# gevaertlab/RNA-GAN

Measured on AMD Instinct MI355X. Metric: training imgs/sec (G+D WGAN-GP step, 256x256), higher is better.
Workload: dtype bf16; 1 GPU; RNA-GAN lung (betaVAE-conditioned wganvae path) 256x256, DCGAN enc2048/step64, per-GPU batch 64, one iteration = G-loss + D-loss + GP steps; global_batch=64, parallelism=dp1, ranks=1, rna_features=19198, hip_graphs=True, dp_statistics=rank-local (DDP)

## Files before the change

include/rnagan_hip.h:

```cpp
#ifndef RNAGAN_HIP_H
#define RNAGAN_HIP_H

#include <stddef.h>
#include <stdint.h>

#ifdef __cplusplus
extern "C" {
#endif

#define RG_OK 0
#define RG_EINVAL (-1)
#define RG_EUNSUPPORTED (-2)
#define RG_EWORKSPACE (-3)
#define RG_EHIP (-4)

#define RG_F32 0
#define RG_BF16 1
#define RG_U8 3
#define RG_F16 2

#define RG_ALGO_AUTO 0
#define RG_ALGO_GENERIC 1
#define RG_ALGO_MFMA 2

int rg_version(void);
const char* rg_last_error(void);
int rg_set_option(const char* name, int value);


int rg_pack_conv_weight(const float* w, void* wdn, void* wup, int O, int I, int dtype, void* stream);
int rg_pack_conv_wup_from_bf16(const void* w_bf16, void* wup, int O, int I, void* stream);
int rg_pack_conv_wup_from_bf16_multi(int n, const void* const* w_bf16, void* const* wup, const int* O, const int* I, void* stream);
int rg_pack_g0_weight_from_bf16(const void* w_bf16, void* wp, int E, int C, void* stream);

int rg_conv_stats_rows(int up, int N, int Hlow, int Wlow, int O, int I, int dtype, int algo);
int rg_conv_down(const void* x, const float* w, const void* wdn, void* y, int N, int Hi, int Wi, int I,
                 int O, float* stats_partial, int dtype, int algo, void* ws, size_t ws_bytes, void* stream);
size_t rg_conv_workspace_bytes(int up, int N, int Hlow, int Wlow, int O, int I, int dtype, int algo);

int rg_conv_up(const void* x, const float* w, const void* wup, void* y, int N, int Ho, int Wo, int O, int I,
               const void* mask_act, float mask_slope, float* stats_partial, int dtype, int algo, void* ws,
               size_t ws_bytes, void* stream);

size_t rg_conv_wgrad_workspace_bytes(int N, int Ho, int Wo, int O, int I, int dtype, int algo);
int rg_conv_wgrad(const void* low, const void* high, float* dw, int N, int Ho, int Wo, int O, int I, int dtype,
                  int accumulate, int algo, void* ws, size_t ws_bytes, void* stream);
int rg_conv_wgrad2(const void* low0, const void* high0, const void* low1, const void* high1, float* dw, int N,
                   int Ho, int Wo, int O, int I, int dtype, int accumulate, int algo, void* ws, size_t ws_bytes,
                   void* stream);
int rg_conv_wgrad_slabs(const void* low0, const void* high0, const void* low1, const void* high1, float* dw, int N, int Ho,
                        int Wo, int O, int I, int dtype, int algo, void* slab, size_t slab_bytes, int* nsplit_out,
                        int* slab_dtype_out, void* stream);
int rg_conv_wgrad_adam_supported(int N, int Ho, int Wo, int O, int I, int two, int dtype, int algo);
int rg_conv_wgrad_adam(const void* low0, const void* high0, const void* low1, const void* high1, float* p, float* m, float* v,
                       const float* hyper, void* shadow_bf16, int N, int Ho, int Wo, int O, int I, int dtype, int algo,
                       void* stream);

int rg_first_down(const float* x_nchw, const float* w, const float* bias, void* y, int N, int H, int W, int I,
                  int O, float slope, int dtype, void* stream);
int rg_last_up(const void* x, const float* w, const float* bias, float* y_nchw, int N, int Ho, int Wo, int O,
               int I, int apply_tanh, int dtype, void* stream);
int rg_first_down_bits(const float* x_nchw, const float* w, const float* bias, void* y, void* bits, int N, int H, int W,
                       int I, int O, float slope, int dtype, void* stream);
int rg_sign_pack(const void* a, void* bits, long long npix, int C, int dtype, void* stream);
int rg_first_down_masked_supported(int H, int W, int I, int O, int dtype);
int rg_first_down_masked(const float* x_nchw, const float* w, void* y, const void* mask_bits, float mask_slope, int N,
                         int H, int W, int I, int O, int dtype, void* stream);
int rg_conv_up_maskbits_supported(int N, int Ho, int Wo, int O, int I, int dtype, int algo);
int rg_conv_up_maskbits(const void* x, const void* wup, void* y, int N, int Ho, int Wo, int O, int I,
                        const void* mask_bits, float mask_slope, int dtype, int algo, void* ws, size_t ws_bytes,
                        void* stream);
int rg_last_up_post_blocks(int N, int Ho, int Wo, int O, int I, int dtype);
int rg_last_up_post(const void* x, const float* w, float* y_nchw, int N, int Ho, int Wo, int O, int I, int dtype,
                    const float* tanh_img, float* part, void* stream);
int rg_last_up_part_chan_sum(const float* part, int nblocks, float* out3, int accumulate, void* stream);
int rg_gp_coef_parts(const float* part, int nblocks, float* sq, float* loss, float* coef, float lambd, void* stream);
int rg_gp_coef_parts_scaled(const float* part, int nblocks, float* sq, float* loss, float* coef, float lambd, float in_scale,
                            float out_scale, void* stream);
int rg_gp_coef_parts_scaled_dev(const float* part, int nblocks, float* sq, float* loss, float* coef, float lambd,
                                const int* amp_state, int slot, void* stream);
int rg_last_up_pre_supported(int Wo, int O, int I, int dtype);
int rg_last_up_pre(const void* z, const float* w, const float* bias, float* y_nchw, const float* mean, const float* invstd,
                   const float* gamma, const float* beta, float slope, int N, int Ho, int Wo, int O, int I, int apply_tanh,
                   int dtype, void* stream);
size_t rg_skinny_wgrad_workspace_bytes(int N, int Ho, int Wo, int O, int I);
int rg_skinny_wgrad(const void* low, const float* high_nchw, float* dw, int N, int Ho, int Wo, int O, int I,
                    int dtype, int accumulate, void* ws, size_t ws_bytes, void* stream);
int rg_skinny_wgrad_slabs(const void* low, const float* high_nchw, int N, int Ho, int Wo, int O, int I, int dtype, void* slab,
                          size_t slab_bytes, int* nslab_out, float* bias_slab, int* bias_done_out, void* stream);
int rg_skinny_wgrad_bias(const void* low, const float* high_nchw, float* dw, float* dbias, int N, int Ho, int Wo, int O, int I,
                         int dtype, int accumulate, int bias_accumulate, void* ws, size_t ws_bytes, int* bias_done_out,
                         void* stream);


int rg_pack_g0_weight(const float* w, void* wp, int E, int C, int dtype, void* stream);
int rg_g0_fwd(const float* z, const float* w, const void* wp, void* y, int N, int E, int C, int dtype, int algo,
              void* ws, size_t ws_bytes, void* stream);
size_t rg_g0_workspace_bytes(int N, int E, int C, int dtype, int algo);
int rg_g0_wgrad(const float* z, const void* gy, float* dw, int N, int E, int C, int dtype, int accumulate,
                int algo, void* ws, size_t ws_bytes, void* stream);

int rg_head_fwd(const void* a, const float* w, float* h, float* out, int N, int C, float slope, int dtype,
                void* stream);
int rg_head_fwd_bias(const void* a, const float* w, const float* bias, float* h, float* out, int N, int C, float slope,
                     int dtype, void* stream);
int rg_vec_sum(const float* x, int n, float* out, int accumulate, void* stream);
int rg_head_grad(const float* h, float* gh, int N, float coef, float slope, void* stream);
int rg_head_grad_dev(const float* h, float* gh, int N, float coef, const int* amp_state, int slot, int part, float slope,
                     void* stream);
int rg_head_bwd_data(const float* gh, const float* w, void* ga, int N, int C, int dtype, void* stream);
int rg_head_wgrad(const float* gh, const void* a, float* dw, int N, int C, int dtype, int accumulate,
                  void* stream);

int rg_pack_linear_weight(const float* w, void* wp, int Nout, int K, int Nout_pad, int K_pad, void* stream);
size_t rg_linear_workspace_bytes(int M, int K, int Nout, int algo);
int rg_linear_affine_act(const float* x, int ldx, const float* w, const void* wp, const float* scale,
                         const float* shift, float* y, int ldy, int M, int K, int Nout, float slope, int algo,
                         void* ws, size_t ws_bytes, void* stream);

size_t rg_colreduce_workspace_bytes(int M, int C, int nq);

int rg_bn_stats(const void* z, float* sum, float* sumsq, int M, int C, int dtype, void* ws, size_t ws_bytes,
                void* stream);
int rg_bn_finalize(const float* sum, const float* sumsq, int M, int C, float eps, float momentum, float* mean,
                   float* invstd, float* running_mean, float* running_var, int64_t* num_batches_tracked,
                   void* stream);
int rg_bn_forward(const void* z, int M, int C, float eps, float momentum, const float* gamma, const float* beta,
                  float slope, float* mean, float* invstd, float* running_mean, float* running_var,
                  int64_t* num_batches_tracked, void* a, int dtype, void* ws, size_t ws_bytes, void* stream);
int rg_bn_forward_partials(const float* partial, int G, const void* z, int M, int C, float eps, float momentum,
                           const float* gamma, const float* beta, float slope, float* mean, float* invstd,
                           float* running_mean, float* running_var, int64_t* num_batches_tracked, void* a, int dtype,
                           void* ws, size_t ws_bytes, void* stream);
int rg_bn_stats_finalize(const void* z, int M, int C, float eps, float momentum, float* mean, float* invstd,
                         float* running_mean, float* running_var, int64_t* num_batches_tracked, int dtype, void* ws,
                         size_t ws_bytes, void* stream);
int rg_bn_act(const void* z, const float* mean, const float* invstd, const float* gamma, const float* beta,
              void* a, int M, int C, float slope, int dtype, void* stream);
int rg_bn_act_bwd(const void* z, const void* ga, const float* mean, const float* invstd, const float* gamma,
                  const float* beta, void* gz, float* s_gy, float* s_gyxh, float* dgamma, float* dbeta,
                  int accumulate, int M, int C, float slope, int dtype, void* ws, size_t ws_bytes, void* stream);
int rg_bn_finalize_partials(const float* partial, int G, int M, int C, float eps, float momentum, float* mean,
                            float* invstd, float* running_mean, float* running_var, int64_t* num_batches_tracked, void* ws,
                            size_t ws_bytes, void* stream);
int rg_g0_wgrad_adam_supported(int N, int E, int C, int dtype);
int rg_g0_wgrad_adam(const float* z, const void* gz0, float* p, float* m, float* v, const float* hyper, void* shadow_bf16,
                     int N, int E, int C, int dtype, void* stream);

int rg_linear_wgrad_adam(const void* gT, const void* xT, int ldn, int N, float* p, float* m, float* v, const float* hyper, int O,
                         int I, void* wpack_bf16, int Kp, void* stream);

int rg_im2col_nhwc(const float* x, int ldx, float* cols, int N, int H, int W, int C, int kh, int kw, int sh, int sw, int ph,
                   int pw, void* stream);
int rg_pool2d_nhwc(const float* x, int ldx, float* y, int ldy, int N, int H, int W, int C, int k, int stride, int pad, int mode,
                   void* stream);
int rg_nchw_to_nhwc_affine(const float* x_nchw, float* y_nhwc, int N, int C, int H, int W, const float* scale, const float* shift,
                           void* stream);
int rg_spatial_mean_nhwc(const float* x, float* y, int N, int HW, int C, void* stream);

int rg_resize_bilinear01(const void* src, int src_dtype, int64_t sn, int64_t sc, int64_t sh, int64_t sw, float mul, float add,
                         float* dst_nchw, int N, int C, int H, int W, int Ho, int Wo, void* stream);
int rg_moments_update(const float* x, int ldx, int n, int F, double* s1, double* s2, void* stream);

int rg_conv_split(int up, int N, int Hlow, int Wlow, int O, int I, int dtype, int algo);
int rg_conv_slab_dtype(int up, int N, int Hlow, int Wlow, int O, int I, int dtype, int algo);
int rg_conv_down_partial(const void* x, const void* wdn, int N, int Hi, int Wi, int I, int O, int dtype, int algo,
                         void* ws, size_t ws_bytes, void* stream);
int rg_conv_up_partial(const void* x, const void* wup, int N, int Ho, int Wo, int O, int I, int dtype, int algo,
                       void* ws, size_t ws_bytes, void* stream);
int rg_slab_bn_supported(long long M, int C, int groups, int nsplit);
size_t rg_slab_bn_scratch_bytes(long long M, int C, int groups);
size_t rg_slab_bn_sync_words(void);
int rg_bn_forward_slabs(const void* slab, int nsplit, size_t slab_stride, int slab_dtype, void* z, void* a, long long M, int C, int groups,
                        float eps, float momentum, const float* gamma, const float* beta, float slope, float* mean,
                        float* invstd, float* running_mean, float* running_var, long long* num_batches_tracked,
                        void* scratch, size_t scratch_bytes, void* sync, void* stream);
int rg_bn_tangent_slabs(const void* slab, int nsplit, size_t slab_stride, int slab_dtype, const void* z, void* zt_out, void* at, long long M,
                        int C, const float* mean, const float* invstd, const float* gamma, const float* beta, float slope,
                        float* s_zt, float* s_xhzt, void* scratch, size_t scratch_bytes, void* sync, void* stream);
int rg_bn_act_bwd_slabs(const void* slab, int nsplit, size_t slab_stride, int slab_dtype, const void* z, void* ga_out, void* gz, long long M,
                        int C, int groups, const float* mean, const float* invstd, const float* gamma, const float* beta,
                        float slope, float* s_gy, float* s_gyxh, float* dgamma, float* dbeta, int accumulate, void* scratch,
                        size_t scratch_bytes, void* sync, void* stream);

int rg_bn_finalize_partials_g2(const float* partial, int G, int nblk, int M, int C, float eps, float momentum, float* mean,
                               float* invstd, float* running_mean, float* running_var, int64_t* num_batches_tracked,
                               void* ws, size_t ws_bytes, void* stream);
int rg_bn_forward_g2(const float* partial, int G, int nblk, const void* z, int M, int C, float eps, float momentum,
                     const float* gamma, const float* beta, float slope, float* mean, float* invstd, float* running_mean,
                     float* running_var, int64_t* num_batches_tracked, void* a, int dtype, void* ws, size_t ws_bytes,
                     void* stream);
int rg_bn_act_bwd_g2(const void* z, const void* ga, const float* mean, const float* invstd, const float* gamma,
                     const float* beta, void* gz, float* s_gy, float* s_gyxh, float* dgamma, float* dbeta, int accumulate,
                     int M, int C, float slope, int dtype, void* ws, size_t ws_bytes, void* stream);
int rg_bn_tangent(const void* z, const void* zt, const float* mean, const float* invstd, const float* gamma,
                  const float* beta, void* at, float* s_zt, float* s_xhzt, int M, int C, float slope, int dtype,
                  void* ws, size_t ws_bytes, void* stream);
int rg_bn_double_bwd(const void* z, const void* qa, const void* zt, const void* ga1, const float* mean,
                     const float* invstd, const float* gamma, const float* beta, const float* s_gy,
                     const float* s_gyxh, const float* s_zt, const float* s_xhzt, void* pz, float* dgamma,
                     float* dbeta, int accumulate, int M, int C, float slope, int dtype, void* ws,
                     size_t ws_bytes, void* stream);

int rg_slab_finish_rows(long long M, int C);
int rg_slab_bias_act(const void* slab, int nsplit, size_t stride, int slab_dtype, const float* bias, void* y, long long M, int C,
                     float slope, void* stream);
int rg_slab_mask(const void* slab, int nsplit, size_t stride, int slab_dtype, const void* mask_act, float mask_slope, void* y,
                 float* col_parts, long long M, int C, void* stream);
int rg_parts_col_sum(const float* parts, int rows, int C, float* out, int accumulate, void* stream);
int rg_bias_act(const void* z, const float* bias, void* y, long long M, int C, float slope, int dtype, void* stream);
int rg_conv_down_epi_supported(int N, int Hi, int Wi, int I, int O, int dtype, int algo);
int rg_conv_down_epi(const void* x, const void* wdn, void* y, int N, int Hi, int Wi, int I, int O, const float* shift, float slope,
                     const void* mask_act, float mask_slope, int dtype, int algo, void* ws, size_t ws_bytes, void* stream);

int rg_lrelu_bwd(const void* g, const void* a, void* out, size_t n, float slope, int dtype, void* stream);
int rg_col_sum(const void* g, float* out, int M, int C, int dtype, int accumulate, void* ws, size_t ws_bytes,
               void* stream);

int rg_tanh_bwd(const float* gy, const float* y, float* gz, size_t n, void* stream);
int rg_nchw_chan_sum(const float* g, float* out, int N, int C, int HW, int accumulate, void* ws, size_t ws_bytes,
                     void* stream);
int rg_interp(const float* real, const float* fake, float* out, size_t n, float eps, void* stream);
int rg_interp_dev(const float* real, const float* fake, float* out, size_t n, const float* eps, void* stream);
size_t rg_reduce_workspace_bytes(size_t n);
int rg_sqnorm(const float* x, float* out, size_t n, void* ws, size_t ws_bytes, void* stream);
int rg_gp_coef(const float* sq, float* loss, float* coef, float lambd, void* stream);
int rg_gp_coef_scaled(const float* sq, float* loss, float* coef, float lambd, float in_scale, float out_scale, void* stream);
int rg_gp_coef_scaled_dev(const float* sq, float* loss, float* coef, float lambd, const int* amp_state, int slot, void* stream);
int rg_scale_by(const float* x, const float* coef, float* out, size_t n, void* stream);
int rg_mean_diff(const float* a, const float* b, float* out, int n, float sign, void* stream);
// ... 130 lines not shown
```

rna_gan_amd/_abi.py:

```python
from __future__ import annotations

import ctypes as C
import os

_HERE = os.path.dirname(os.path.abspath(__file__))
LIB_PATH = os.path.join(_HERE, "librnagan_hip.so")

RG_F32, RG_BF16, RG_F16 = 0, 1, 2
RG_U8 = 3
ALGO_AUTO, ALGO_GENERIC, ALGO_MFMA = 0, 1, 2

_p = C.c_void_p
_i = C.c_int
_f = C.c_float
_d = C.c_double
_z = C.c_size_t
_l = C.c_int64

PROTOTYPES = {
    "rg_version": (_i, []),
    "rg_last_error": (C.c_char_p, []),
    "rg_set_option": (_i, [C.c_char_p, _i]),
    "rg_pack_conv_weight": (_i, [_p, _p, _p, _i, _i, _i, _p]),
    "rg_conv_stats_rows": (_i, [_i, _i, _i, _i, _i, _i, _i, _i]),
    "rg_conv_down": (_i, [_p, _p, _p, _p, _i, _i, _i, _i, _i, _p, _i, _i, _p, _z, _p]),
    "rg_conv_up": (_i, [_p, _p, _p, _p, _i, _i, _i, _i, _i, _p, _f, _p, _i, _i, _p, _z, _p]),
    "rg_conv_workspace_bytes": (_z, [_i, _i, _i, _i, _i, _i, _i, _i]),
    "rg_conv_wgrad_workspace_bytes": (_z, [_i, _i, _i, _i, _i, _i, _i]),
    "rg_conv_wgrad": (_i, [_p, _p, _p, _i, _i, _i, _i, _i, _i, _i, _i, _p, _z, _p]),
    "rg_conv_wgrad2": (_i, [_p, _p, _p, _p, _p, _i, _i, _i, _i, _i, _i, _i, _i, _p, _z, _p]),
    "rg_conv_wgrad_slabs": (_i, [_p, _p, _p, _p, _p, _i, _i, _i, _i, _i, _i, _i, _p, _z, _p, _p, _p]),
    "rg_grad_to_wire": (_i, [_p, _p, _z, _i, _p, _p, _p, _p, _p, _p]),
    "rg_conv_wgrad_wire": (_i, [_p, _p, _p, _p, _p, _i, _i, _i, _i, _i, _i, _i, _p]),
    "rg_conv_wgrad_adam_supported": (_i, [_i, _i, _i, _i, _i, _i, _i, _i]),
    "rg_conv_wgrad_adam": (_i, [_p, _p, _p, _p, _p, _p, _p, _p, _p, _i, _i, _i, _i, _i, _i, _i, _p]),
    "rg_first_down": (_i, [_p, _p, _p, _p, _i, _i, _i, _i, _i, _f, _i, _p]),
    "rg_first_down_bits": (_i, [_p, _p, _p, _p, _p, _i, _i, _i, _i, _i, _f, _i, _p]),
    "rg_sign_pack": (_i, [_p, _p, C.c_longlong, _i, _i, _p]),
    "rg_first_down_masked_supported": (_i, [_i, _i, _i, _i, _i]),
    "rg_first_down_masked": (_i, [_p, _p, _p, _p, _f, _i, _i, _i, _i, _i, _i, _p]),
    "rg_conv_up_maskbits_supported": (_i, [_i, _i, _i, _i, _i, _i, _i]),
    "rg_conv_up_maskbits": (_i, [_p, _p, _p, _i, _i, _i, _i, _i, _p, _f, _i, _i, _p, _z, _p]),
    "rg_last_up": (_i, [_p, _p, _p, _p, _i, _i, _i, _i, _i, _i, _i, _p]),
    "rg_skinny_wgrad_workspace_bytes": (_z, [_i, _i, _i, _i, _i]),
    "rg_skinny_wgrad": (_i, [_p, _p, _p, _i, _i, _i, _i, _i, _i, _i, _p, _z, _p]),
    "rg_skinny_wgrad_slabs": (_i, [_p, _p, _i, _i, _i, _i, _i, _i, _p, _z, _p, _p, _p, _p]),
    "rg_skinny_wgrad_bias": (_i, [_p, _p, _p, _p, _i, _i, _i, _i, _i, _i, _i, _i, _p, _z, _p, _p]),
    "rg_pack_g0_weight": (_i, [_p, _p, _i, _i, _i, _p]),
    "rg_pack_conv_wup_from_bf16": (_i, [_p, _p, _i, _i, _p]),
    "rg_pack_conv_wup_from_bf16_multi": (_i, [_i, _p, _p, _p, _p, _p]),
    "rg_pack_g0_weight_from_bf16": (_i, [_p, _p, _i, _i, _p]),
    "rg_g0_fwd": (_i, [_p, _p, _p, _p, _i, _i, _i, _i, _i, _p, _z, _p]),
    "rg_g0_workspace_bytes": (_z, [_i, _i, _i, _i, _i]),
    "rg_g0_wgrad": (_i, [_p, _p, _p, _i, _i, _i, _i, _i, _i, _p, _z, _p]),
    "rg_head_fwd": (_i, [_p, _p, _p, _p, _i, _i, _f, _i, _p]),
    "rg_head_grad": (_i, [_p, _p, _i, _f, _f, _p]),
    "rg_head_grad_dev": (_i, [_p, _p, _i, _f, _p, _i, _i, _f, _p]),
    "rg_adam_hyper_dev3": (_i, [_p, _d, _d, _d, _d, _d, _p, _i, _p, _p]),
    "rg_nonfinite_probe": (_i, [_i, _p, _p, _p, _p, _p]),
    "rg_amp_update": (_i, [_p, _i, _i, _i, _i, _p]),
    "rg_amp_latch": (_i, [_p, _i, _p]),
    "rg_gp_coef_scaled_dev": (_i, [_p, _p, _p, _f, _p, _i, _p]),
    "rg_gp_coef_parts_scaled_dev": (_i, [_p, _i, _p, _p, _p, _f, _p, _i, _p]),
    "rg_head_bwd_data": (_i, [_p, _p, _p, _i, _i, _i, _p]),
    "rg_head_wgrad": (_i, [_p, _p, _p, _i, _i, _i, _i, _p]),
    "rg_pack_linear_weight": (_i, [_p, _p, _i, _i, _i, _i, _p]),
    "rg_linear_workspace_bytes": (_z, [_i, _i, _i, _i]),
    "rg_linear_affine_act": (_i, [_p, _i, _p, _p, _p, _p, _p, _i, _i, _i, _i, _f, _i, _p, _z, _p]),
    "rg_colreduce_workspace_bytes": (_z, [_i, _i, _i]),
    "rg_bn_stats": (_i, [_p, _p, _p, _i, _i, _i, _p, _z, _p]),
    "rg_bn_finalize": (_i, [_p, _p, _i, _i, _f, _f, _p, _p, _p, _p, _p, _p]),
    "rg_bn_forward": (_i, [_p, _i, _i, _f, _f, _p, _p, _f, _p, _p, _p, _p, _p, _p, _i, _p, _z, _p]),
    "rg_bn_forward_partials": (_i, [_p, _i, _p, _i, _i, _f, _f, _p, _p, _f, _p, _p, _p, _p, _p, _p, _i, _p, _z, _p]),
    "rg_bn_stats_finalize": (_i, [_p, _i, _i, _f, _f, _p, _p, _p, _p, _p, _i, _p, _z, _p]),
    "rg_bn_act": (_i, [_p, _p, _p, _p, _p, _p, _i, _i, _f, _i, _p]),
    "rg_bn_act_bwd": (_i, [_p, _p, _p, _p, _p, _p, _p, _p, _p, _p, _p, _i, _i, _i, _f, _i, _p, _z, _p]),
    "rg_bn_act_bwd_g2": (_i, [_p, _p, _p, _p, _p, _p, _p, _p, _p, _p, _p, _i, _i, _i, _f, _i, _p, _z, _p]),
    "rg_bn_finalize_partials": (_i, [_p, _i, _i, _i, _f, _f, _p, _p, _p, _p, _p, _p, _z, _p]),
    "rg_linear_wgrad_adam": (_i, [_p, _p, _i, _i, _p, _p, _p, _p, _i, _i, _p, _i, _p]),
    "rg_last_up_post_blocks": (_i, [_i, _i, _i, _i, _i, _i]),
    "rg_last_up_post": (_i, [_p, _p, _p, _i, _i, _i, _i, _i, _i, _p, _p, _p]),
    "rg_last_up_part_chan_sum": (_i, [_p, _i, _p, _i, _p]),
    "rg_gp_coef_parts": (_i, [_p, _i, _p, _p, _p, _f, _p]),
    "rg_last_up_pre_supported": (_i, [_i, _i, _i, _i]),
    "rg_last_up_pre": (_i, [_p, _p, _p, _p, _p, _p, _p, _p, _f, _i, _i, _i, _i, _i, _i, _i, _p]),
    "rg_bn_forward_g2": (_i, [_p, _i, _i, _p, _i, _i, _f, _f, _p, _p, _f, _p, _p, _p, _p, _p, _p, _i, _p, _z, _p]),
    "rg_bn_finalize_partials_g2": (_i, [_p, _i, _i, _i, _i, _f, _f, _p, _p, _p, _p, _p, _p, _z, _p]),
    "rg_bn_tangent": (_i, [_p, _p, _p, _p, _p, _p, _p, _p, _p, _i, _i, _f, _i, _p, _z, _p]),
    "rg_bn_double_bwd": (_i, [_p, _p, _p, _p, _p, _p, _p, _p, _p, _p, _p, _p, _p, _p, _p, _i, _i, _i, _f, _i,
                              _p, _z, _p]),
    "rg_lrelu_bwd": (_i, [_p, _p, _p, _z, _f, _i, _p]),
    "rg_col_sum": (_i, [_p, _p, _i, _i, _i, _i, _p, _z, _p]),
    "rg_tanh_bwd": (_i, [_p, _p, _p, _z, _p]),
    "rg_nchw_chan_sum": (_i, [_p, _p, _i, _i, _i, _i, _p, _z, _p]),
    "rg_interp": (_i, [_p, _p, _p, _z, _f, _p]),
    "rg_reduce_workspace_bytes": (_z, [_z]),
    "rg_sqnorm": (_i, [_p, _p, _z, _p, _z, _p]),
    "rg_gp_coef": (_i, [_p, _p, _p, _f, _p]),
    "rg_scale_by": (_i, [_p, _p, _p, _z, _p]),
    "rg_mean_diff": (_i, [_p, _p, _p, _i, _f, _p]),
    "rg_latent_prep": (_i, [_p, _p, _p, _i, _i, _p]),
    "rg_adam_step": (_i, [_p, _p, _p, _p, _z, _i, _d, _d, _d, _d, _p]),
    "rg_clamp": (_i, [_p, _z, _f, _f, _p]),
    "rg_upconv3_workspace_bytes": (_z, [_i, _i, _i, _i, _i]),
    "rg_upconv3_fwd": (_i, [_p, _p, _p, _p, _i, _i, _i, _i, _i, _i, _i, _i, _p, _z, _p]),
    "rg_upconv3_bwd_data": (_i, [_p, _i, _p, _p, _i, _i, _i, _i, _i, _i, _i, _p, _z, _p]),
    "rg_upconv3_wgrad": (_i, [_p, _i, _p, _p, _i, _i, _i, _i, _i, _i, _i, _i, _p, _z, _p]),
    "rg_export_images_nhwc": (_i, [_p, _p, _i, _i, _i, _i, _p]),
    "rg_bn_bwd_sums": (_i, [_p, _p, _p, _p, _p, _p, _p, _p, _i, _i, _f, _i, _p, _z, _p]),
    "rg_bn_bwd_apply": (_i, [_p, _p, _p, _p, _p, _p, _p, _p, _p, _i, _i, _i, _f, _i, _p]),
    "rg_bn_tangent_sums": (_i, [_p, _p, _p, _p, _p, _p, _p, _p, _i, _i, _f, _i, _p, _z, _p]),
    "rg_bn_tangent_apply": (_i, [_p, _p, _p, _p, _p, _p, _p, _p, _p, _i, _i, _i, _f, _i, _p]),
    "rg_bn_dbl_sums": (_i, [_p, _p, _p, _p, _p, _p, _p, _p, _p, _i, _i, _f, _i, _p, _z, _p]),
    "rg_bn_dbl_apply": (_i, [_p] * 17 + [_i, _i, _i, _i, _f, _i, _p, _z, _p]),
    "rg_latent_stats": (_i, [_p, _p, _p, _p, _i, _i, _p]),
    "rg_latent_apply": (_i, [_p, _p, _p, _p, _p, _i, _i, _i, _p]),
    "rg_adam_step_dev": (_i, [_p, _p, _p, _p, _z, _p, _p, _p, _p]),
    "rg_adam_step_slabs": (_i, [_p, _p, _p, _p, _z, _p, _p, _i, _p, _p, _p, _p, _p, _p]),
    "rg_ema_update": (_i, [_p, _p, _z, _f, _p, _p, _p]),
    "rg_interp_dev": (_i, [_p, _p, _p, _z, _p, _p]),
    "rg_adam_hyper_dev": (_i, [_p, _d, _d, _d, _d, _d, _p, _p]),
    "rg_adam_hyper_dev2": (_i, [_p, _d, _d, _d, _d, _d, _d, _p, _p]),
    "rg_storage_dtype": (_i, []),
    "rg_gp_coef_scaled": (_i, [_p, _p, _p, _f, _f, _f, _p]),
    "rg_gp_coef_parts_scaled": (_i, [_p, _i, _p, _p, _p, _f, _f, _f, _p]),
    "rg_transpose_f32": (_i, [_p, _p, _i, _i, _p]),
    "rg_transpose_pack_bf16": (_i, [_p, _p, _i, _i, _i, _i, _p]),
    "rg_gemm_nt_bf16_workspace_bytes": (_z, [_i, _i, _i]),
    "rg_gemm_nt_bf16": (_i, [_p, _p, _p, _p, _p, _i, _i, _i, _i, _f, _p, _z, _p]),
    "rg_vae_dropout": (_i, [_p, _p, _p, _i, _i, _i, _f, _p]),
    "rg_vae_reparam": (_i, [_p, _p, _p, _p, _z, _p]),
    "rg_vae_reparam_bwd": (_i, [_p, _p, _p, _p, _p, _p, _p, _z, _p]),
    "rg_tanh_inplace": (_i, [_p, _z, _p]),
    "rg_add_inplace": (_i, [_p, _p, _z, _p]),
    "rg_vae_loss_workspace_bytes": (_z, []),
    "rg_vae_loss": (_i, [_p, _p, _i, _i, _i, _p, _p, _i, _f, _i, _p, _p, _p, _p, _p, _z, _p]),
    "rg_widen_bf16": (_i, [_p, _p, _z, _p]),
    "rg_cast_pad": (_i, [_p, _p, _i, _i, _i, _i, _p]),
    "rg_selftest_layouts": (_i, [_p, _p]),
    "rg_u8_to_norm": (_i, [_p, _p, _z, _f, _f, _p]),
    "rg_conv_up_fp8": (_i, [_p, _p, _p, _i, _i, _i, _i, _i, _p, _p, _f, _i, _p]),
    "rg_gemm_fp8": (_i, [_p, _p, _p, _i, _i, _i, _p, _p, _f, _i, _p]),
    "rg_fp8_supported": (_i, [_i, _i, _i, _i]),
    "rg_cast_fp8": (_i, [_p, _p, _z, _f, _p]),
    "rg_selftest_fp8": (_i, [_p, _p]),
    "rg_g0_wgrad_adam_supported": (_i, [_i, _i, _i, _i]),
    "rg_g0_wgrad_adam": (_i, [_p, _p, _p, _p, _p, _p, _p, _i, _i, _i, _i, _p]),
    "rg_im2col_nhwc": (_i, [_p, _i, _p, _i, _i, _i, _i, _i, _i, _i, _i, _i, _i, _p]),
    "rg_pool2d_nhwc": (_i, [_p, _i, _p, _i, _i, _i, _i, _i, _i, _i, _i, _i, _p]),
    "rg_nchw_to_nhwc_affine": (_i, [_p, _p, _i, _i, _i, _i, _p, _p, _p]),
    "rg_spatial_mean_nhwc": (_i, [_p, _p, _i, _i, _i, _p]),
    "rg_resize_bilinear01": (_i, [_p, _i, _l, _l, _l, _l, _f, _f, _p, _i, _i, _i, _i, _i, _i, _p]),
    "rg_moments_update": (_i, [_p, _i, _i, _i, _p, _p, _p]),
    "rg_conv_split": (_i, [_i, _i, _i, _i, _i, _i, _i, _i]),
    "rg_conv_slab_dtype": (_i, [_i, _i, _i, _i, _i, _i, _i, _i]),
    "rg_conv_down_partial": (_i, [_p, _p, _i, _i, _i, _i, _i, _i, _i, _p, _z, _p]),
    "rg_conv_up_partial": (_i, [_p, _p, _i, _i, _i, _i, _i, _i, _i, _p, _z, _p]),
    "rg_slab_bn_supported": (_i, [C.c_longlong, _i, _i, _i]),
    "rg_slab_bn_scratch_bytes": (_z, [C.c_longlong, _i, _i]),
    "rg_slab_bn_sync_words": (_z, []),
    "rg_bn_forward_slabs": (_i, [_p, _i, _z, _i, _p, _p, C.c_longlong, _i, _i, _f, _f, _p, _p, _f, _p, _p, _p, _p, _p, _p, _z, _p, _p]),
    "rg_bn_tangent_slabs": (_i, [_p, _i, _z, _i, _p, _p, _p, C.c_longlong, _i, _p, _p, _p, _p, _f, _p, _p, _p, _z, _p, _p]),
    "rg_bn_act_bwd_slabs": (_i, [_p, _i, _z, _i, _p, _p, _p, C.c_longlong, _i, _i, _p, _p, _p, _p, _f, _p, _p, _p, _p, _i, _p, _z,
                                 _p, _p]),
    "rg_conv_up_affine": (_i, [_p, _p, _p, _i, _i, _i, _i, _i, _p, _p, _f, _p, _z, _p]),
    "rg_g0_fwd_affine": (_i, [_p, _p, _p, _i, _i, _i, _p, _p, _f, _p, _z, _p]),
    "rg_split_planes": (_i, [_p, _p, _z, _p]),
    "rg_f32p_conv_supported": (_i, [_i, _i, _i, _i, _i, _i, _i]),
    "rg_f32p_conv_workspace_bytes": (_z, [_i, _i, _i, _i, _i, _i, _i]),
    "rg_f32p_conv_stats_rows": (_i, [_i, _i, _i, _i, _i, _i, _i]),
    "rg_f32p_conv": (_i, [_i, _p, _p, _p, _i, _i, _i, _i, _i, _i, _p, _p, _f, _p, _z, _p]),
    "rg_f32p_conv_mask_supported": (_i, [_i, _i, _i, _i, _i, _i, _i]),
    "rg_f32p_wgrad_supported": (_i, [_i, _i, _i, _i, _i, _i]),
    "rg_f32p_wgrad_workspace_bytes": (_z, [_i, _i, _i, _i, _i, _i, _i]),
    "rg_f32p_wgrad": (_i, [_p, _p, _p, _p, _p, _i, _i, _i, _i, _i, _i, _i, _p, _z, _p]),
    "rg_slab_finish_rows": (_i, [C.c_longlong, _i]),
    "rg_slab_bias_act": (_i, [_p, _i, _z, _i, _p, _p, C.c_longlong, _i, _f, _p]),
    "rg_slab_mask": (_i, [_p, _i, _z, _i, _p, _f, _p, _p, C.c_longlong, _i, _p]),
    "rg_parts_col_sum": (_i, [_p, _i, _i, _p, _i, _p]),
    "rg_bias_act": (_i, [_p, _p, _p, C.c_longlong, _i, _f, _i, _p]),
    "rg_vec_sum": (_i, [_p, _i, _p, _i, _p]),
    "rg_conv_down_epi_supported": (_i, [_i, _i, _i, _i, _i, _i, _i]),
    "rg_conv_down_epi": (_i, [_p, _p, _p, _i, _i, _i, _i, _i, _p, _f, _p, _f, _i, _i, _p, _z, _p]),
    "rg_head_fwd_bias": (_i, [_p, _p, _p, _p, _p, _i, _i, _f, _i, _p]),
    "rg_probe_mfma_bare": (_i, [_i, _i, _i, _i, _p, _p, _p]),
    "rg_probe_lds_mfma": (_i, [_i, _i, _i, _p, _p, _p, _p, _p]),
    "rg_probe_copy": (_i, [_p, _p, _z, _i, _i, _p]),
    "rg_probe_fill_bf16": (_i, [_p, _z, C.c_uint, _p]),
}

ABI_VERSION = 616

_libs = {}
LIB_PATH_F16 = os.path.join(_HERE, "librnagan_hip_f16.so")
BF16_ONLY_PREFIXES = ("rg_probe_", "rg_split_planes", "rg_f32p_")


def load(half: str = "bf16"):
    if half in _libs:
        return _libs[half]
    if half not in ("bf16", "f16"):
        raise ValueError("half must be 'bf16' or 'f16'")
    path = LIB_PATH if half == "bf16" else LIB_PATH_F16
    if not os.path.exists(path):
        raise RuntimeError(
            "rna_gan_amd: %s not found. Build it with `python -m rna_gan_amd.build` "
            "(hipcc --offload-arch=gfx950). There is no CPU / eager fallback." % path)
    try:
        lib = C.CDLL(path)
    except OSError as e:
        raise RuntimeError("rna_gan_amd: cannot load %s: %s" % (path, e))
    for name, (res, args) in PROTOTYPES.items():
        if half == "f16" and name.startswith(BF16_ONLY_PREFIXES):
            continue
        fn = getattr(lib, name, None)
        if fn is None:
            raise RuntimeError("rna_gan_amd: symbol %s missing from %s: the library is older than this package -- rebuild "
                               "it with `python -m rna_gan_amd.build`" % (name, path))
        fn.restype = res
        fn.argtypes = args
    got = lib.rg_version()
    if got != ABI_VERSION:
        raise RuntimeError("rna_gan_amd: %s reports ABI version %d, this package binds version %d (a stale or swapped "
                           "build): rebuild it with `python -m rna_gan_amd.build`" % (path, got, ABI_VERSION))
    want = RG_BF16 if half == "bf16" else RG_F16
    if lib.rg_storage_dtype() != want:
        raise RuntimeError("rna_gan_amd: %s stores dtype code %d, expected %d (a swapped build)" % (path, lib.rg_storage_dtype(), want))
    _libs[half] = lib
    return lib


_LAST_ERR_LIBS = ("bf16", "f16")


def check(rc: int, what: str):
    if rc != 0:
        msgs = []
        for h in _LAST_ERR_LIBS:
            if h in _libs:
                m = _libs[h].rg_last_error()
                if m:
                    msgs.append(m.decode() if len(_libs) == 1 else "[%s build] %s" % (h, m.decode()))
        raise RuntimeError("rna_gan_amd: %s failed (%d): %s" % (what, rc, " | ".join(msgs) if msgs else "?"))
```

rna_gan_amd/csrc/rg_api.hip:

```cpp
#include "rg_common.h"
#include "rg_internal.h"
#include <stdarg.h>
#include <stdio.h>
#include <stdlib.h>
#include <string.h>
#include <ctype.h>

static thread_local char g_err[512] = "";

void rg_set_error(const char* fmt, ...) {
  va_list ap;
  va_start(ap, fmt);
  vsnprintf(g_err, sizeof(g_err), fmt, ap);
  va_end(ap);
}

extern "C" int rg_version(void) { return 616; }
extern "C" const char* rg_last_error(void) { return g_err; }

static const char* const g_opt_names[] = {"conv8", "conv8_blocks", "conv_tile", "xcd", "class_fast", "wgrad_blocks",
                                          "wgrad8", "conv_v1", "stream_tile", "narrow8", "conv8_mfma", "conv8_epi", "wgrad8_blocks", "korder", "convp", "convp_blocks",
                                          "fp8_mx", "wgrad8n", "f32mma", "convd", "convd_blocks", "skinny128", "slab16", "wslab16", "bn_rev", "wgrad8_mfma", "narrow32", "upimg", "upimg_blocks"};
constexpr int G_NOPT = sizeof(g_opt_names) / sizeof(g_opt_names[0]);
static int g_opt_override[G_NOPT];
static int g_opt_env[G_NOPT];

int rg_option(const char* name, int dflt) {
  for (int i = 0; i < G_NOPT; ++i) {
    if (strcmp(name, g_opt_names[i]) != 0) continue;
    if (g_opt_override[i] > 0) return g_opt_override[i] - 1;
    if (g_opt_env[i] == 0) {
      char var[64] = "RNAGAN_";
      size_t n = strlen(var);
      for (const char* c = name; *c && n + 1 < sizeof(var); ++c) var[n++] = (char)toupper((unsigned char)*c);
      var[n] = 0;
      const char* e = getenv(var);
      g_opt_env[i] = e ? atoi(e) + 1 : -1;
      if (g_opt_env[i] == 0) g_opt_env[i] = -1;
    }
    return g_opt_env[i] > 0 ? g_opt_env[i] - 1 : dflt;
  }
  return dflt;
}

extern "C" int rg_set_option(const char* name, int value) {
  RG_REQUIRE(name, RG_EINVAL, "set_option: null name");
  for (int i = 0; i < G_NOPT; ++i)
    if (strcmp(name, g_opt_names[i]) == 0) { g_opt_override[i] = value < 0 ? 0 : value + 1; return RG_OK; }
  rg_set_error("set_option: unknown option '%s'", name);
  return RG_EINVAL;
}

static bool want_mfma(int algo, int dtype) { return algo != RG_ALGO_GENERIC && dtype == RG_H16; }

extern "C" int rg_pack_conv_weight(const float* w, void* wdn, void* wup, int O, int I, int dtype, void* stream) {
  RG_REQUIRE(w && O > 0 && I > 0, RG_EINVAL, "pack_conv_weight: bad args");
  RG_REQUIRE(dtype == RG_H16, RG_EUNSUPPORTED, "pack_conv_weight: only bf16 packs exist (fp32 kernels read w)");
  return rg_mfma_pack_conv_weight(w, wdn, wup, O, I, rg_stream(stream));
}

extern "C" size_t rg_conv_workspace_bytes(int up, int N, int Hlow, int Wlow, int O, int I, int dtype, int algo) {
  if (!want_mfma(algo, dtype)) return 0;
  if (!rg_mfma_conv_supported(N, Hlow, Wlow, up ? O : I, up ? I : O)) return 0;
  return rg_mfma_conv_ws_bytes(up, N, Hlow, Wlow, O, I);
}

extern "C" int rg_conv_stats_rows(int up, int N, int Hlow, int Wlow, int O, int I, int dtype, int algo) {
  if (N <= 0 || Hlow <= 0 || Wlow <= 0 || O <= 0 || I <= 0 || !want_mfma(algo, dtype)) return 0;
  if (!rg_mfma_conv_supported(N, Hlow, Wlow, up ? O : I, up ? I : O)) return 0;
  return rg_mfma_conv_stats_rows(up, N, Hlow, Wlow, O, I);
}

extern "C" int rg_conv_split(int up, int N, int Hlow, int Wlow, int O, int I, int dtype, int algo) {
  if (N <= 0 || Hlow <= 0 || Wlow <= 0 || O <= 0 || I <= 0 || !want_mfma(algo, dtype)) return 1;
  if (!rg_mfma_conv_supported(N, Hlow, Wlow, up ? O : I, up ? I : O)) return 1;
  return rg_mfma_conv_nsplit(up, N, Hlow, Wlow, O, I);
}

extern "C" int rg_conv_slab_dtype(int up, int N, int Hlow, int Wlow, int O, int I, int dtype, int algo) {
  if (rg_conv_split(up, N, Hlow, Wlow, O, I, dtype, algo) <= 1) return RG_F32;
  return rg_mfma_conv_slab16(up, N, Hlow, Wlow, O, I) ? RG_H16 : RG_F32;
}

extern "C" int rg_conv_down_partial(const void* x, const void* wdn, int N, int Hi, int Wi, int I, int O, int dtype, int algo,
                                    void* ws, size_t ws_bytes, void* stream) {
  RG_REQUIRE(x && wdn && ws && N > 0 && Hi > 0 && Wi > 0 && I > 0 && O > 0 && Hi % 2 == 0 && Wi % 2 == 0, RG_EINVAL,
             "conv_down_partial: bad args");
  RG_REQUIRE(rg_conv_split(0, N, Hi / 2, Wi / 2, O, I, dtype, algo) > 1, RG_EUNSUPPORTED,
             "conv_down_partial: this shape does not run split-K (rg_conv_split)");
  return rg_mfma_conv_down(x, wdn, nullptr, N, Hi, Wi, I, O, nullptr, ws, ws_bytes, rg_stream(stream), 1);
}

extern "C" int rg_conv_up_partial(const void* x, const void* wup, int N, int Ho, int Wo, int O, int I, int dtype, int algo,
                                  void* ws, size_t ws_bytes, void* stream) {
  RG_REQUIRE(x && wup && ws && N > 0 && Ho > 0 && Wo > 0 && I > 0 && O > 0, RG_EINVAL, "conv_up_partial: bad args");
  RG_REQUIRE(rg_conv_split(1, N, Ho, Wo, O, I, dtype, algo) > 1, RG_EUNSUPPORTED,
             "conv_up_partial: this shape does not run split-K (rg_conv_split)");
  return rg_mfma_conv_up(x, wup, nullptr, N, Ho, Wo, O, I, nullptr, 1.f, nullptr, ws, ws_bytes, rg_stream(stream), nullptr,
                         nullptr, 1.f, 0, 1);
}
// ... 159 lines not shown
                              const float* invstd, const float* gamma, const float* beta, float slope, int N, int Ho, int Wo,
                              int O, int I, int apply_tanh, int dtype, void* stream) {
  RG_REQUIRE(z && w && y_nchw && mean && invstd && gamma && beta && N > 0 && Ho > 0 && Wo > 0, RG_EINVAL,
             "last_up_pre: bad args");
  RG_REQUIRE(rg_last_up_pre_supported(Wo, O, I, dtype), RG_EUNSUPPORTED, "last_up_pre: shape");
  return rg_skinny_last_up(z, w, bias, y_nchw, N, Ho, Wo, O, I, apply_tanh, dtype, rg_stream(stream), mean, invstd, gamma,
                           beta, slope);
}

extern "C" int rg_last_up(const void* x, const float* w, const float* bias, float* y_nchw, int N, int Ho, int Wo,
                          int O, int I, int apply_tanh, int dtype, void* stream) {
  RG_REQUIRE(x && w && y_nchw && N > 0 && Ho > 0 && Wo > 0 && I > 0 && O > 0, RG_EINVAL, "last_up: bad args");
  if (rg_skinny_supported(I, O))
    return rg_skinny_last_up(x, w, bias, y_nchw, N, Ho, Wo, O, I, apply_tanh, dtype, rg_stream(stream));
  return rg_generic_last_up(x, w, bias, y_nchw, N, Ho, Wo, O, I, apply_tanh, dtype, rg_stream(stream));
}

extern "C" int rg_last_up_post_blocks(int N, int Ho, int Wo, int O, int I, int dtype) {
  return rg_skinny_supported(I, O) ? rg_skinny_last_up_post_blocks(N, Ho, Wo, O, dtype) : 0;
}
extern "C" int rg_last_up_post(const void* x, const float* w, float* y_nchw, int N, int Ho, int Wo, int O, int I, int dtype,
                               const float* tanh_img, float* part, void* stream) {
  RG_REQUIRE(x && w && y_nchw && N > 0 && Ho > 0 && Wo > 0 && (tanh_img || part), RG_EINVAL, "last_up_post: bad args");
  RG_REQUIRE(rg_last_up_post_blocks(N, Ho, Wo, O, I, dtype) > 0, RG_EUNSUPPORTED, "last_up_post: shape");
  RG_REQUIRE((((uintptr_t)tanh_img | (uintptr_t)part) & 15) == 0, RG_EINVAL, "last_up_post: 16-byte aligned buffers required");
  return rg_skinny_last_up(x, w, nullptr, y_nchw, N, Ho, Wo, O, I, 0, dtype, rg_stream(stream), nullptr, nullptr, nullptr,
                           nullptr, 1.f, tanh_img, part);
}
extern "C" int rg_last_up_part_chan_sum(const float* part, int nblocks, float* out3, int accumulate, void* stream) {
  RG_REQUIRE(part && out3 && nblocks > 0, RG_EINVAL, "last_up_part_chan_sum: bad args");
  return rg_skinny_lu_part_final(part, nblocks, out3, accumulate, 0, nullptr, nullptr, 0.f, rg_stream(stream));
}
extern "C" int rg_gp_coef_parts_scaled(const float* part, int nblocks, float* sq, float* loss, float* coef, float lambd,
                                       float in_scale, float out_scale, void* stream) {
  RG_REQUIRE(part && loss && coef && nblocks > 0 && in_scale > 0.f && out_scale > 0.f, RG_EINVAL, "gp_coef_parts: bad args");
  return rg_skinny_lu_part_final(part, nblocks, sq, 0, 1, loss, coef, lambd, rg_stream(stream), in_scale, out_scale);
}
extern "C" int rg_storage_dtype(void) { return RG_H16; }
extern "C" int rg_gp_coef_parts(const float* part, int nblocks, float* sq, float* loss, float* coef, float lambd,
                                void* stream) {
  RG_REQUIRE(part && loss && coef && nblocks > 0, RG_EINVAL, "gp_coef_parts: bad args");
  return rg_skinny_lu_part_final(part, nblocks, sq, 0, 1, loss, coef, lambd, rg_stream(stream));
}

extern "C" size_t rg_skinny_wgrad_workspace_bytes(int N, int Ho, int Wo, int O, int I) {
  size_t a = rg_generic_wgrad_ws_bytes(N, Ho, Wo, O, I);
  size_t b = rg_skinny_supported(I, O) ? rg_skinny_wgrad_ws_bytes(N, Ho, Wo, O, I) : 0;
  return a > b ? a : b;
}

extern "C" int rg_skinny_wgrad(const void* low, const float* high_nchw, float* dw, int N, int Ho, int Wo, int O, int I,
                               int dtype, int accumulate, void* ws, size_t ws_bytes, void* stream) {
  RG_REQUIRE(low && high_nchw && dw && N > 0 && Ho > 0 && Wo > 0 && I > 0 && O > 0, RG_EINVAL,
             "skinny_wgrad: bad args");
  if (rg_skinny_supported(I, O) && !(dtype == RG_F32 && rg_generic_f32_image_side(N, 2 * Ho, 2 * Wo, I, O)))
    return rg_skinny_wgrad_impl(low, high_nchw, dw, N, Ho, Wo, O, I, dtype, accumulate, ws, ws_bytes,
                                rg_stream(stream));
  return rg_generic_skinny_wgrad(low, high_nchw, dw, N, Ho, Wo, O, I, dtype, accumulate, ws, ws_bytes,
                                 rg_stream(stream));
}

extern "C" int rg_skinny_wgrad_bias(const void* low, const float* high_nchw, float* dw, float* dbias, int N, int Ho, int Wo, int O,
                                    int I, int dtype, int accumulate, int bias_accumulate, void* ws, size_t ws_bytes,
                                    int* bias_done_out, void* stream) {
  RG_REQUIRE(low && high_nchw && dw && bias_done_out && N > 0 && Ho > 0 && Wo > 0 && I > 0 && O > 0, RG_EINVAL,
             "skinny_wgrad_bias: bad args");
  *bias_done_out = 0;
  if (rg_skinny_supported(I, O) && !(dtype == RG_F32 && rg_generic_f32_image_side(N, 2 * Ho, 2 * Wo, I, O)))
    return rg_skinny_wgrad_impl(low, high_nchw, dw, N, Ho, Wo, O, I, dtype, accumulate, ws, ws_bytes, rg_stream(stream),
                                O == 64 ? dbias : nullptr, bias_accumulate, bias_done_out);
  return rg_generic_skinny_wgrad(low, high_nchw, dw, N, Ho, Wo, O, I, dtype, accumulate, ws, ws_bytes, rg_stream(stream));
}

extern "C" int rg_skinny_wgrad_slabs(const void* low, const float* high_nchw, int N, int Ho, int Wo, int O, int I, int dtype,
                                     void* slab, size_t slab_bytes, int* nslab_out, float* bias_slab, int* bias_done_out,
                                     void* stream) {
  RG_REQUIRE(low && high_nchw && slab && nslab_out && N > 0 && Ho > 0 && Wo > 0 && I > 0 && O > 0 &&
                 (bias_slab == nullptr || bias_done_out != nullptr), RG_EINVAL, "skinny_wgrad_slabs: bad args");
  *nslab_out = 0;
  if (bias_done_out) *bias_done_out = 0;
  if (!rg_skinny_supported(I, O)) return RG_OK;
  return rg_skinny_wgrad_slabs_impl(low, high_nchw, N, Ho, Wo, O, I, dtype, slab, slab_bytes, nslab_out, bias_slab, bias_done_out,
                                    rg_stream(stream));
}

extern "C" int rg_pack_conv_wup_from_bf16(const void* w_bf16, void* wup, int O, int I, void* stream) {
  RG_REQUIRE(w_bf16 && wup && O > 0 && I > 0, RG_EINVAL, "pack_conv_wup_from_bf16: bad args");
  return rg_mfma_transpose_bf16(w_bf16, wup, O, 16 * I, 0, rg_stream(stream));
}
extern "C" int rg_pack_conv_wup_from_bf16_multi(int n, const void* const* w_bf16, void* const* wup, const int* O, const int* I,
                                                void* stream) {
  RG_REQUIRE(n >= 1 && n <= 8 && w_bf16 && wup && O && I, RG_EINVAL, "pack_conv_wup_from_bf16_multi: bad args");
  int Cc[8];
  for (int i = 0; i < n; ++i) Cc[i] = 16 * I[i];
  return rg_mfma_transpose_bf16_multi(n, w_bf16, wup, O, Cc, rg_stream(stream));
}
extern "C" int rg_pack_g0_weight_from_bf16(const void* w_bf16, void* wp, int E, int C, void* stream) {
  RG_REQUIRE(w_bf16 && wp && E > 0 && C > 0, RG_EINVAL, "pack_g0_weight_from_bf16: bad args");
  return rg_mfma_transpose_bf16(w_bf16, wp, E, 16 * C, 1, rg_stream(stream));
}
extern "C" int rg_pack_g0_weight(const float* w, void* wp, int E, int C, int dtype, void* stream) {
  RG_REQUIRE(w && wp && E > 0 && C > 0, RG_EINVAL, "pack_g0_weight: bad args");
  RG_REQUIRE(dtype == RG_H16, RG_EUNSUPPORTED, "pack_g0_weight: only bf16 packs exist");
  return rg_mfma_pack_g0_weight(w, wp, E, C, rg_stream(stream));
}

extern "C" size_t rg_g0_workspace_bytes(int N, int E, int C, int dtype, int algo) {
  if (!want_mfma(algo, dtype)) return 0;
  size_t a = (size_t)N * E * 2;
  size_t b = rg_mfma_g0_wgrad_ws_bytes(N, E, C);
  return a > b ? a : b;
}

extern "C" int rg_g0_fwd(const float* z, const float* w, const void* wp, void* y, int N, int E, int C, int dtype,
                         int algo, void* ws, size_t ws_bytes, void* stream) {
  RG_REQUIRE(z && y && N > 0 && E > 0 && C > 0, RG_EINVAL, "g0_fwd: bad args");
  if (want_mfma(algo, dtype) && wp && rg_mfma_plain_supported(N, E, 16 * C)) {
    RG_REQUIRE(ws && ws_bytes >= (size_t)N * E * 2, RG_EWORKSPACE, "g0_fwd: workspace too small");
    int rc = rg_cast_pad(z, ws, N, E, E, RG_H16, stream);
    if (rc) return rc;
    return rg_mfma_gemm_plain(ws, wp, y, N, E, 16 * C, 16 * C, rg_stream(stream));
  }
  RG_REQUIRE(algo != RG_ALGO_MFMA, RG_EUNSUPPORTED, "g0_fwd: shape/dtype not supported by the MFMA kernel");
  RG_REQUIRE(w, RG_EINVAL, "g0_fwd: generic kernel needs the fp32 master weight");
  return rg_generic_g0_fwd(z, w, y, N, E, C, dtype, rg_stream(stream));
}

extern "C" int rg_g0_fwd_affine(const float* z, const void* wp, void* y, int N, int E, int C, const float* scale,
                                const float* shift, float slope, void* ws, size_t ws_bytes, void* stream) {
  RG_REQUIRE(z && wp && y && scale && shift && N > 0 && E > 0 && C > 0, RG_EINVAL, "g0_fwd_affine: bad args");
  RG_REQUIRE(rg_mfma_plain_supported(N, E, 16 * C), RG_EUNSUPPORTED, "g0_fwd_affine: shape not supported by the MFMA kernel");
  RG_REQUIRE(ws && ws_bytes >= (size_t)N * E * 2, RG_EWORKSPACE, "g0_fwd_affine: workspace too small");
  int rc = rg_cast_pad(z, ws, N, E, E, RG_H16, stream);
  if (rc) return rc;
  return rg_mfma_gemm_plain(ws, wp, y, N, E, 16 * C, 16 * C, rg_stream(stream), scale, shift, slope);
}

extern "C" int rg_conv_up_affine(const void* x, const void* wup, void* y, int N, int Ho, int Wo, int O, int I,
                                 const float* scale, const float* shift, float slope, void* ws, size_t ws_bytes,
                                 void* stream) {
  RG_REQUIRE(x && wup && y && scale && shift && N > 0 && Ho > 0 && Wo > 0 && I > 0 && O > 0, RG_EINVAL,
             "conv_up_affine: bad args");
  RG_REQUIRE(rg_mfma_conv_supported(N, Ho, Wo, O, I), RG_EUNSUPPORTED,
             "conv_up_affine: shape not supported by the MFMA kernel");
  return rg_mfma_conv_up(x, wup, y, N, Ho, Wo, O, I, nullptr, 1.f, nullptr, ws, ws_bytes, rg_stream(stream), scale, shift,
                         slope);
}

extern "C" int rg_conv_up_fp8(const void* x8, const void* wup8, void* y, int N, int Ho, int Wo, int O, int I,
                              const float* scale, const float* shift, float slope, int out_fp8, void* stream) {
  RG_REQUIRE(x8 && wup8 && y && scale && shift && N > 0 && Ho > 0 && Wo > 0 && I > 0 && O > 0, RG_EINVAL, "conv_up_fp8: bad args");
  RG_REQUIRE(rg_is_pow2(Ho) && rg_is_pow2(Wo) && rg_mfma_fp8_supported(N * Ho * Wo, 4 * O, I, 4), RG_EUNSUPPORTED,
             "conv_up_fp8: shape not supported (O, I multiples of 128, at least 256 / 512 low-resolution pixels)");
  return rg_mfma_conv_up_fp8(x8, wup8, y, N, Ho, Wo, O, I, scale, shift, slope, out_fp8, rg_stream(stream));
}
extern "C" int rg_gemm_fp8(const void* a8, const void* b8, void* y, int M, int K, int Ncols, const float* scale,
                           const float* shift, float slope, int out_fp8, void* stream) {
  RG_REQUIRE(a8 && b8 && y && scale && shift && M > 0 && K > 0 && Ncols > 0, RG_EINVAL, "gemm_fp8: bad args");
  RG_REQUIRE(rg_mfma_fp8_supported(M, K, Ncols, 1), RG_EUNSUPPORTED, "gemm_fp8: shape not supported");
  return rg_mfma_gemm_fp8(a8, b8, y, M, K, Ncols, scale, shift, slope, out_fp8, rg_stream(stream));
}
extern "C" int rg_fp8_supported(int M, int K, int Ncols, int taps) { return rg_mfma_fp8_supported(M, K, Ncols, taps) ? 1 : 0; }

extern "C" int rg_g0_wgrad(const float* z, const void* gy, float* dw, int N, int E, int C, int dtype, int accumulate,
                           int algo, void* ws, size_t ws_bytes, void* stream) {
  RG_REQUIRE(z && gy && dw && N > 0 && E > 0 && C > 0, RG_EINVAL, "g0_wgrad: bad args");
// ... 91 lines not shown
```

rna_gan_amd/csrc/rg_g0adam.hip:

```cpp
#include "rg_internal.h"
#include <stdlib.h>

namespace {

constexpr int GA_E = 64, GA_J = 256, GA_N = 64;

struct AdamC { float b1, b2, omb1, omb2, eps, step_size, inv_sqrt_bc2, wd, ginv; };
__device__ __forceinline__ void adam_upd(const AdamC& a, float& pp, float gg, float& mm, float& vv) {
  rg_adam_upd(pp, gg * a.ginv, mm, vv, a.b2, a.omb1, a.omb2, a.eps, a.step_size, a.inv_sqrt_bc2, a.wd);
}

typedef rg_h16x8 ga_bf16x8;
typedef __attribute__((ext_vector_type(16))) float ga_f32x16;
constexpr int GA_CP = GA_J + 4;
constexpr int GA_P = 72;

template <typename TG>
__global__ __launch_bounds__(256) void g0_wgrad_adam_kernel(const float* __restrict__ z, const TG* __restrict__ gz0,
                                                            float* __restrict__ p, float* __restrict__ m, float* __restrict__ v,
                                                            const float* __restrict__ hyper, uint16_t* __restrict__ shadow,
                                                            int N, int E, int C, int e_fastest) {
  constexpr int OPS = (GA_E + GA_J) * GA_P * 2;
  static_assert(32 * GA_CP * 4 <= OPS, "accumulator tile must fit into the operand area");
  __shared__ __attribute__((aligned(16))) unsigned char smem[OPS];
  if (hyper[9] != 0.f) return;
  uint16_t* zsT = reinterpret_cast<uint16_t*>(smem);
  uint16_t* gsT = zsT + GA_E * GA_P;
  float* ct = reinterpret_cast<float*>(smem);
  const int t = threadIdx.x, lane = t & 63, wave = t >> 6;
  const int fr = lane & 31, fh = lane >> 5;
  const int e0 = (e_fastest ? blockIdx.x : blockIdx.y) * GA_E, c0 = (e_fastest ? blockIdx.y : blockIdx.x) * 16;
  ga_f32x16 acc[2][2];
#pragma unroll
  for (int i = 0; i < 2; ++i)
#pragma unroll
    for (int j = 0; j < 2; ++j)
#pragma unroll
      for (int r = 0; r < 16; ++r) acc[i][j][r] = 0.f;

  const int ze = t & 63, zq = t >> 6;
  const int gnp = t & 31, gtap = (t >> 5) * 2;
  float zr[8][2];
  uint4 gr[2][2][2];
  auto load_chunk = [&](int n0) {
#pragma unroll
    for (int i = 0; i < 8; ++i) {
      const int n = n0 + 2 * (zq + 4 * i);
      zr[i][0] = n < N ? z[(size_t)n * E + e0 + ze] : 0.f;
      zr[i][1] = n + 1 < N ? z[(size_t)(n + 1) * E + e0 + ze] : 0.f;
    }
#pragma unroll
    for (int a = 0; a < 2; ++a)
#pragma unroll
      for (int k = 0; k < 2; ++k) {
        const int n = n0 + 2 * gnp + k;
        gr[a][k][0] = gr[a][k][1] = make_uint4(0, 0, 0, 0);
        if (n < N) {
          const TG* src = gz0 + ((size_t)n * 16 + gtap + a) * C + c0;
          if constexpr (sizeof(TG) == 2) {
            gr[a][k][0] = *reinterpret_cast<const uint4*>(src);
            gr[a][k][1] = *reinterpret_cast<const uint4*>(src + 8);
          } else {
            float x[16];
            Vec<TG, 8>::ld(src, x);
            Vec<TG, 8>::ld(src + 8, x + 8);
            uint32_t w[8];
#pragma unroll
            for (int c2 = 0; c2 < 8; ++c2) w[c2] = (uint32_t)f32_to_h16(x[2 * c2]) | ((uint32_t)f32_to_h16(x[2 * c2 + 1]) << 16);
            gr[a][k][0] = make_uint4(w[0], w[1], w[2], w[3]);
            gr[a][k][1] = make_uint4(w[4], w[5], w[6], w[7]);
          }
        }
      }
  };
  auto store_chunk = [&]() {
#pragma unroll
    for (int i = 0; i < 8; ++i)
      *reinterpret_cast<uint32_t*>(zsT + ze * GA_P + 2 * (zq + 4 * i)) =
          (uint32_t)f32_to_h16(zr[i][0]) | ((uint32_t)f32_to_h16(zr[i][1]) << 16);
#pragma unroll
    for (int a = 0; a < 2; ++a)
#pragma unroll
      for (int h = 0; h < 2; ++h) {
        const uint32_t lo[4] = {gr[a][0][h].x, gr[a][0][h].y, gr[a][0][h].z, gr[a][0][h].w};
        const uint32_t hi[4] = {gr[a][1][h].x, gr[a][1][h].y, gr[a][1][h].z, gr[a][1][h].w};
#pragma unroll
        for (int c2 = 0; c2 < 4; ++c2) {
          const int cl = 8 * h + 2 * c2;
          *reinterpret_cast<uint32_t*>(gsT + (cl * 16 + gtap + a) * GA_P + 2 * gnp) = (lo[c2] & 0xffffu) | (hi[c2] << 16);
          *reinterpret_cast<uint32_t*>(gsT + ((cl + 1) * 16 + gtap + a) * GA_P + 2 * gnp) = (lo[c2] >> 16) | (hi[c2] & 0xffff0000u);
        }
      }
  };
  load_chunk(0);
  for (int n0 = 0; n0 < N; n0 += GA_N) {
    if (n0) __syncthreads();
    store_chunk();
    __syncthreads();
    if (n0 + GA_N < N) load_chunk(n0 + GA_N);
#pragma unroll
    for (int ks = 0; ks < 4; ++ks) {
      ga_bf16x8 fa[2], fb[2];
#pragma unroll
      for (int i = 0; i < 2; ++i)
        fa[i] = __builtin_bit_cast(ga_bf16x8, *reinterpret_cast<const uint4*>(zsT + (32 * i + fr) * GA_P + 16 * ks + 8 * fh));
#pragma unroll
      for (int j = 0; j < 2; ++j)
        fb[j] = __builtin_bit_cast(ga_bf16x8,
                                   *reinterpret_cast<const uint4*>(gsT + (64 * wave + 32 * j + fr) * GA_P + 16 * ks + 8 * fh));
#pragma unroll
      for (int i = 0; i < 2; ++i)
#pragma unroll
        for (int j = 0; j < 2; ++j) acc[i][j] = rg_mfma_h16_32x32x16(fa[i], fb[j], acc[i][j], 0, 0, 0);
    }
  }

  const AdamC a{hyper[0], hyper[1], hyper[2], hyper[3], hyper[4], hyper[5], hyper[6], hyper[7], hyper[8]};
  const size_t ld = (size_t)C * 16;
  const int tj = t & 63, te = t >> 6;
  const size_t col = (size_t)c0 * 16 + 4 * tj;
#pragma unroll
  for (int i = 0; i < 2; ++i) {
    __syncthreads();
#pragma unroll
    for (int j = 0; j < 2; ++j)
#pragma unroll
      for (int r = 0; r < 16; ++r)
        ct[(8 * (r >> 2) + 4 * fh + (r & 3)) * GA_CP + 64 * wave + 32 * j + fr] = acc[i][j][r];
    __syncthreads();
#pragma unroll
    for (int k0 = 0; k0 < 8; k0 += 4) {
      float4 P[4], M[4], V[4];
#pragma unroll
      for (int k = 0; k < 4; ++k) {
        const size_t idx = (size_t)(e0 + 32 * i + 8 * te + k0 + k) * ld + col;
        P[k] = *reinterpret_cast<const float4*>(p + idx);
        M[k] = *reinterpret_cast<const float4*>(m + idx);
        V[k] = *reinterpret_cast<const float4*>(v + idx);
      }
#pragma unroll
      for (int k = 0; k < 4; ++k) {
        const size_t idx = (size_t)(e0 + 32 * i + 8 * te + k0 + k) * ld + col;
        const float4 g4 = *reinterpret_cast<const float4*>(ct + (8 * te + k0 + k) * GA_CP + 4 * tj);
        adam_upd(a, P[k].x, g4.x, M[k].x, V[k].x);
        adam_upd(a, P[k].y, g4.y, M[k].y, V[k].y);
        adam_upd(a, P[k].z, g4.z, M[k].z, V[k].z);
        adam_upd(a, P[k].w, g4.w, M[k].w, V[k].w);
        *reinterpret_cast<float4*>(p + idx) = P[k];
        *reinterpret_cast<float4*>(m + idx) = M[k];
        *reinterpret_cast<float4*>(v + idx) = V[k];
        if (shadow)
          *reinterpret_cast<uint2*>(shadow + idx) = make_uint2((uint32_t)f32_to_h16(P[k].x) | ((uint32_t)f32_to_h16(P[k].y) << 16),
                                                               (uint32_t)f32_to_h16(P[k].z) | ((uint32_t)f32_to_h16(P[k].w) << 16));
      }
    }
  }
}


template <int VEC>
__global__ __launch_bounds__(256) void lin_wgrad_adam_kernel(const uint16_t* __restrict__ gT, const uint16_t* __restrict__ xT,
                                                             int ldn, int N, float* __restrict__ p, float* __restrict__ m,
                                                             float* __restrict__ v, const float* __restrict__ hyper, int O,
                                                             int I, uint16_t* __restrict__ wpack, int Kp) {
  constexpr int OPS = (GA_E + GA_J) * GA_P * 2;
  __shared__ __attribute__((aligned(16))) unsigned char smem[OPS];
  if (hyper[9] != 0.f) return;
  uint16_t* zsT = reinterpret_cast<uint16_t*>(smem);
  uint16_t* gsT = zsT + GA_E * GA_P;
  float* ct = reinterpret_cast<float*>(smem);
  const int t = threadIdx.x, lane = t & 63, wave = t >> 6;
  const int fr = lane & 31, fh = lane >> 5;
  const int o0 = blockIdx.x * GA_E, i0 = blockIdx.y * GA_J;
  ga_f32x16 acc[2][2];
#pragma unroll
  for (int a = 0; a < 2; ++a)
#pragma unroll
    for (int b = 0; b < 2; ++b)
#pragma unroll
      for (int r = 0; r < 16; ++r) acc[a][b][r] = 0.f;

  for (int n0 = 0; n0 < N; n0 += GA_N) {
    if (n0) __syncthreads();
#pragma unroll
    for (int k = 0; k < 2; ++k) {
      const int idx = t + 256 * k, row = idx >> 3, pc = idx & 7;
      uint4 w = make_uint4(0, 0, 0, 0);
      if (o0 + row < O) w = *reinterpret_cast<const uint4*>(gT + (size_t)(o0 + row) * ldn + n0 + 8 * pc);
      *reinterpret_cast<uint4*>(zsT + row * GA_P + 8 * pc) = w;
    }
#pragma unroll
    for (int k = 0; k < 8; ++k) {
      const int idx = t + 256 * k, row = idx >> 3, pc = idx & 7;
      uint4 w = make_uint4(0, 0, 0, 0);
      if (i0 + row < I) w = *reinterpret_cast<const uint4*>(xT + (size_t)(i0 + row) * ldn + n0 + 8 * pc);
      *reinterpret_cast<uint4*>(gsT + row * GA_P + 8 * pc) = w;
    }
    __syncthreads();
#pragma unroll
    for (int ks = 0; ks < 4; ++ks) {
      ga_bf16x8 fa[2], fb[2];
#pragma unroll
      for (int a = 0; a < 2; ++a)
        fa[a] = __builtin_bit_cast(ga_bf16x8, *reinterpret_cast<const uint4*>(zsT + (32 * a + fr) * GA_P + 16 * ks + 8 * fh));
#pragma unroll
      for (int b = 0; b < 2; ++b)
        fb[b] = __builtin_bit_cast(ga_bf16x8,
                                   *reinterpret_cast<const uint4*>(gsT + (64 * wave + 32 * b + fr) * GA_P + 16 * ks + 8 * fh));
#pragma unroll
      for (int a = 0; a < 2; ++a)
#pragma unroll
        for (int b = 0; b < 2; ++b) acc[a][b] = rg_mfma_h16_32x32x16(fa[a], fb[b], acc[a][b], 0, 0, 0);
    }
  }

  const AdamC hy{hyper[0], hyper[1], hyper[2], hyper[3], hyper[4], hyper[5], hyper[6], hyper[7], hyper[8]};
  const int tj = t & 63, te = t >> 6;
  const int col = i0 + 4 * tj;
#pragma unroll
  for (int a = 0; a < 2; ++a) {
    __syncthreads();
#pragma unroll
    for (int b = 0; b < 2; ++b)
#pragma unroll
      for (int r = 0; r < 16; ++r)
        ct[(8 * (r >> 2) + 4 * fh + (r & 3)) * GA_CP + 64 * wave + 32 * b + fr] = acc[a][b][r];
    __syncthreads();
    constexpr int VPR = 4 / VEC;
#pragma unroll
    for (int k0 = 0; k0 < 8; k0 += 4) {
      float P[4][4], M[4][4], V[4][4];
      bool ok[4][VPR];
#pragma unroll
      for (int k = 0; k < 4; ++k) {
        const int row = o0 + 32 * a + 8 * te + k0 + k;
        const size_t base = (size_t)row * I + col;
#pragma unroll
        for (int q = 0; q < VPR; ++q) {
          ok[k][q] = row < O && col + q * VEC < I;
          if (!ok[k][q]) continue;
          if constexpr (VEC == 4) {
            const float4 a4 = *reinterpret_cast<const float4*>(p + base), b4 = *reinterpret_cast<const float4*>(m + base),
                         c4 = *reinterpret_cast<const float4*>(v + base);
            P[k][0] = a4.x; P[k][1] = a4.y; P[k][2] = a4.z; P[k][3] = a4.w;
            M[k][0] = b4.x; M[k][1] = b4.y; M[k][2] = b4.z; M[k][3] = b4.w;
            V[k][0] = c4.x; V[k][1] = c4.y; V[k][2] = c4.z; V[k][3] = c4.w;
          } else if constexpr (VEC == 2) {
            const float2 a2 = *reinterpret_cast<const float2*>(p + base + 2 * q), b2 = *reinterpret_cast<const float2*>(m + base + 2 * q),
                         c2 = *reinterpret_cast<const float2*>(v + base + 2 * q);
            P[k][2 * q] = a2.x; P[k][2 * q + 1] = a2.y; M[k][2 * q] = b2.x; M[k][2 * q + 1] = b2.y;
            V[k][2 * q] = c2.x; V[k][2 * q + 1] = c2.y;
          } else {
            P[k][q] = p[base + q]; M[k][q] = m[base + q]; V[k][q] = v[base + q];
          }
        }
      }
#pragma unroll
      for (int k = 0; k < 4; ++k) {
        const int row = o0 + 32 * a + 8 * te + k0 + k;
        const size_t base = (size_t)row * I + col;
        const float* gsrc = ct + (8 * te + k0 + k) * GA_CP + 4 * tj;
#pragma unroll
        for (int q = 0; q < VPR; ++q) {
          if (!ok[k][q]) continue;
#pragma unroll
          for (int e = 0; e < VEC; ++e) adam_upd(hy, P[k][q * VEC + e], gsrc[q * VEC + e], M[k][q * VEC + e], V[k][q * VEC + e]);
          if constexpr (VEC == 4) {
            *reinterpret_cast<float4*>(p + base) = make_float4(P[k][0], P[k][1], P[k][2], P[k][3]);
            *reinterpret_cast<float4*>(m + base) = make_float4(M[k][0], M[k][1], M[k][2], M[k][3]);
            *reinterpret_cast<float4*>(v + base) = make_float4(V[k][0], V[k][1], V[k][2], V[k][3]);
            if (wpack)
              *reinterpret_cast<uint2*>(wpack + (size_t)row * Kp + col) =
                  make_uint2((uint32_t)f32_to_h16(P[k][0]) | ((uint32_t)f32_to_h16(P[k][1]) << 16),
                             (uint32_t)f32_to_h16(P[k][2]) | ((uint32_t)f32_to_h16(P[k][3]) << 16));
          } else if constexpr (VEC == 2) {
            *reinterpret_cast<float2*>(p + base + 2 * q) = make_float2(P[k][2 * q], P[k][2 * q + 1]);
            *reinterpret_cast<float2*>(m + base + 2 * q) = make_float2(M[k][2 * q], M[k][2 * q + 1]);
            *reinterpret_cast<float2*>(v + base + 2 * q) = make_float2(V[k][2 * q], V[k][2 * q + 1]);
            if (wpack)
              *reinterpret_cast<uint32_t*>(wpack + (size_t)row * Kp + col + 2 * q) =
                  (uint32_t)f32_to_h16(P[k][2 * q]) | ((uint32_t)f32_to_h16(P[k][2 * q + 1]) << 16);
          } else {
            p[base + q] = P[k][q]; m[base + q] = M[k][q]; v[base + q] = V[k][q];
            if (wpack) wpack[(size_t)row * Kp + col + q] = f32_to_h16(P[k][q]);
          }
        }
      }
    }
  }
}

}

extern "C" int rg_g0_wgrad_adam_supported(int N, int E, int C, int dtype) {
  return N > 0 && E % GA_E == 0 && C % 16 == 0 && (dtype == RG_H16 || dtype == RG_F32) ? 1 : 0;
}

extern "C" int rg_g0_wgrad_adam(const float* z, const void* gz0, float* p, float* m, float* v, const float* hyper,
                                void* shadow_bf16, int N, int E, int C, int dtype, void* stream) {
  RG_REQUIRE(z && gz0 && p && m && v && hyper, RG_EINVAL, "g0_wgrad_adam: null");
  RG_REQUIRE(rg_g0_wgrad_adam_supported(N, E, C, dtype), RG_EUNSUPPORTED, "g0_wgrad_adam: E %% 64 == 0 and C %% 16 == 0 required");
  RG_REQUIRE((((uintptr_t)p | (uintptr_t)m | (uintptr_t)v | (uintptr_t)z | (uintptr_t)gz0) & 15) == 0 &&
                 (((uintptr_t)shadow_bf16) & 7) == 0, RG_EINVAL, "g0_wgrad_adam: 16-byte aligned buffers required");
  static int order = -1;
  if (order < 0) { const char* e = getenv("RNAGAN_G0ADAM_ORDER"); order = e ? atoi(e) : 1; }
  const int e_fastest = order != 0;
  const dim3 grid(e_fastest ? (unsigned)(E / GA_E) : (unsigned)(C / 16), e_fastest ? (unsigned)(C / 16) : (unsigned)(E / GA_E));
  hipStream_t st = rg_stream(stream);
  if (dtype == RG_H16)
    hipLaunchKernelGGL(g0_wgrad_adam_kernel<h16_t>, grid, dim3(256), 0, st, z, (const h16_t*)gz0, p, m, v, hyper,
                       (uint16_t*)shadow_bf16, N, E, C, e_fastest);
  else
    hipLaunchKernelGGL(g0_wgrad_adam_kernel<float>, grid, dim3(256), 0, st, z, (const float*)gz0, p, m, v, hyper,
                       (uint16_t*)shadow_bf16, N, E, C, e_fastest);
  RG_LAUNCH_CHECK("g0_wgrad_adam");
  return RG_OK;
}

extern "C" int rg_linear_wgrad_adam(const void* gT, const void* xT, int ldn, int N, float* p, float* m, float* v,
                                    const float* hyper, int O, int I, void* wpack_bf16, int Kp, void* stream) {
  RG_REQUIRE(gT && xT && p && m && v && hyper && N > 0 && O > 0 && I > 0, RG_EINVAL, "linear_wgrad_adam: bad args");
  RG_REQUIRE(ldn % 64 == 0 && ldn >= N && (((uintptr_t)gT | (uintptr_t)xT) & 15) == 0, RG_EINVAL,
             "linear_wgrad_adam: operands must be sample-contiguous, zero padded to a multiple of 64 samples, 16-byte aligned");
  RG_REQUIRE(!wpack_bf16 || (Kp >= I && Kp % 8 == 0 && ((uintptr_t)wpack_bf16 & 15) == 0), RG_EINVAL,
             "linear_wgrad_adam: packed image needs Kp >= I, Kp %% 8 == 0, 16-byte alignment");
  uint16_t* wpk = (uint16_t*)wpack_bf16;
  const dim3 grid((unsigned)((O + GA_E - 1) / GA_E), (unsigned)((I + GA_J - 1) / GA_J));
  hipStream_t st = rg_stream(stream);
  const uintptr_t al = (uintptr_t)p | (uintptr_t)m | (uintptr_t)v;
  const uint16_t* a = (const uint16_t*)gT;
  const uint16_t* b = (const uint16_t*)xT;
  if (I % 4 == 0 && (al & 15) == 0)
    hipLaunchKernelGGL(lin_wgrad_adam_kernel<4>, grid, dim3(256), 0, st, a, b, ldn, N, p, m, v, hyper, O, I, wpk, Kp);
  else if (I % 2 == 0 && (al & 7) == 0)
    hipLaunchKernelGGL(lin_wgrad_adam_kernel<2>, grid, dim3(256), 0, st, a, b, ldn, N, p, m, v, hyper, O, I, wpk, Kp);
  else
    hipLaunchKernelGGL(lin_wgrad_adam_kernel<1>, grid, dim3(256), 0, st, a, b, ldn, N, p, m, v, hyper, O, I, wpk, Kp);
  RG_LAUNCH_CHECK("linear_wgrad_adam");
  return RG_OK;
}
```

rna_gan_amd/csrc/rg_internal.h:

```cpp
#pragma once
#include "rg_common.h"

int rg_option(const char* name, int dflt);

int rg_reduce_slabs(const float* slab, float* dst, size_t n, int nsplit, int accumulate, int perm_mode, int Q,
                    hipStream_t st);
int rg_generic_conv_down(const void* x, const float* w, void* y, int N, int Hi, int Wi, int I, int O, int dtype,
                         hipStream_t st);
int rg_generic_conv_up(const void* x, const float* w, void* y, int N, int Ho, int Wo, int O, int I, const void* mask,
                       float mslope, int dtype, hipStream_t st);
bool rg_generic_f32_image_side(int N, int H, int W, int I, int O);
int rg_generic_first_down(const float* x, const float* w, const float* bias, void* y, int N, int H, int W, int I,
                          int O, float slope, int dtype, hipStream_t st);
int rg_generic_last_up(const void* x, const float* w, const float* bias, float* y, int N, int Ho, int Wo, int O,
                       int I, int apply_tanh, int dtype, hipStream_t st);
size_t rg_generic_wgrad_ws_bytes(int N, int Ho, int Wo, int O, int I);
int rg_generic_conv_wgrad(const void* low, const void* high, float* dw, int N, int Ho, int Wo, int O, int I,
                          int dtype, int accumulate, void* ws, size_t ws_bytes, hipStream_t st);
int rg_generic_skinny_wgrad(const void* low, const float* high_nchw, float* dw, int N, int Ho, int Wo, int O, int I,
                            int dtype, int accumulate, void* ws, size_t ws_bytes, hipStream_t st);
int rg_generic_g0_fwd(const float* z, const float* w, void* y, int N, int E, int C, int dtype, hipStream_t st);
int rg_generic_g0_wgrad(const float* z, const void* gy, float* dw, int N, int E, int C, int dtype, int accumulate,
                        hipStream_t st);
int rg_generic_linear(const float* x, int ldx, const float* w, const float* scale, const float* shift, float* y,
// ... 63 lines not shown
                           int Cout, int out_nchw, int dtype, hipStream_t st);
int rg_generic_upconv3_bwd_data(const void* gy, int gy_nchw, const float* w, void* gx, int N, int H, int W, int Cin,
                                int Cout, int dtype, void* ws, size_t ws_bytes, hipStream_t st);
int rg_generic_upconv3_wgrad(const void* gy, int gy_nchw, const void* x, float* dw, int N, int H, int W, int Cin,
                             int Cout, int dtype, int accumulate, void* ws, size_t ws_bytes, hipStream_t st);
int rg_mfma_transpose_bf16(const void* src, void* dst, int R, int Cc, int permute, hipStream_t st);
int rg_mfma_transpose_bf16_multi(int n, const void* const* src, void* const* dst, const int* R, const int* Cc, hipStream_t st);
size_t rg_mfma_g0_wgrad_ws_bytes(int N, int E, int C);
bool rg_mfma_g0_wgrad_supported(int N, int E, int C);
int rg_mfma_g0_wgrad(const float* z, const void* gy, float* dw, int N, int E, int C, void* ws, size_t ws_bytes,
                     hipStream_t st);
int rg_mfma_gemm_plain(const void* a, const void* bt, void* c, int M, int K, int Ncols, int ldc, hipStream_t st,
                       const float* scale = nullptr, const float* shift = nullptr, float slope = 1.f);
int rg_mfma_linear(const void* a, const void* bt, const float* scale, const float* shift, float* y, int ldy, int M,
                   int Kpad, int Nout, float slope, void* ws, size_t ws_bytes, hipStream_t st);
size_t rg_mfma_linear_ws_bytes(int M, int Kpad, int Nout);
int rg_mfma_conv_wgrad(const void* low, const void* high, float* dw, int N, int Ho, int Wo, int O, int I,
                       int accumulate, void* ws, size_t ws_bytes, hipStream_t st);

int rg_mfma_conv_wgrad2(const void* low0, const void* high0, const void* low1, const void* high1, float* dw, int N,
                        int Ho, int Wo, int O, int I, int accumulate, void* ws, size_t ws_bytes, hipStream_t st,
                        int* nsplit_out = nullptr, int* slab_dtype_out = nullptr);
size_t rg_mfma_wgrad2_ws_bytes(int N, int Ho, int Wo, int O, int I);

bool rg_mfma_conv_up_planes64_supported(int N, int Ho, int Wo, int O, int I, int products);
int rg_mfma_conv_up_planes64(const void* xp, const void* wp, float* y, int N, int Ho, int Wo, int O, int I, int products,
                             hipStream_t st, const float* maskf = nullptr, float mslope = 1.f);
bool rg_mfma_fp8_supported(int M, int K, int Ncols, int taps);
int rg_mfma_conv_up_fp8(const void* x8, const void* wup8, void* y, int N, int Ho, int Wo, int O, int I, const float* scale,
                        const float* shift, float slope, int out_fp8, hipStream_t st);
int rg_mfma_gemm_fp8(const void* a8, const void* b8, void* y, int M, int K, int Ncols, const float* scale, const float* shift,
                     float slope, int out_fp8, hipStream_t st);

int rg_conv8_launch(int mode, const void* args, int bm, unsigned gx, unsigned gy, unsigned gz, hipStream_t st);
int rg_conv8n_launch(const void* args, unsigned tiles_m, hipStream_t st);
bool rg_convp_supported(int M, int Ncols, int Cin, int Hs, int Ws);
constexpr int RG_CONVP_DEFAULT = 1;
bool rg_convd_supported(int M, int Ncols, int Cin, int Hs, int Ws);
int rg_convd_stats_rows(int M);
int rg_convd_launch(const void* args, hipStream_t st);
int rg_convp_tiles(int M);
int rg_convp_launch(const void* args, hipStream_t st);

bool rg_wgrad8_supported(int K, int O, int I);
int rg_wgrad8_split(int K, int O, int I, int* kt_per_split);
bool rg_wgrad8n_supported(int K, int O, int I);
int rg_wgrad8n_split(int K, int O, int I, int* kt_per_split);
int rg_wgrad8n_launch(const void* low0, const void* high0, const void* low1, const void* high1, float* out, int Kseg,
                      int two, int O, int I, int Ho, int Wo, int nsplit, int kt_per_split, int accumulate, hipStream_t st,
                      int slab16 = 0);
int rg_wgrad8_launch(const void* low0, const void* high0, const void* low1, const void* high1, float* out, int Kseg,
                     int two, int O, int I, int Ho, int Wo, int nsplit, int kt_per_split, int accumulate, hipStream_t st,
                     int slab16 = 0);
int rg_wgrad8_wire_launch(const void* low0, const void* high0, const void* low1, const void* high1, uint16_t* out16, int Kseg,
                          int two, int O, int I, int Ho, int Wo, int kt_per_split, hipStream_t st);
int rg_mfma_conv_wgrad_wire(const void* low0, const void* high0, const void* low1, const void* high1, int N, int Ho, int Wo,
                            int O, int I, uint16_t* out16, hipStream_t st);
int rg_wgrad8_adam_launch(const void* low0, const void* high0, const void* low1, const void* high1, int Kseg, int two, int O,
                          int I, int Ho, int Wo, int kt_per_split, float* p, float* m, float* v, uint16_t* shadow,
                          const float* hyper, hipStream_t st);
bool rg_mfma_conv_wgrad_adam_supported(int N, int Ho, int Wo, int O, int I, bool two);
int rg_mfma_conv_wgrad_adam(const void* low0, const void* high0, const void* low1, const void* high1, int N, int Ho, int Wo,
                            int O, int I, float* p, float* m, float* v, uint16_t* shadow, const float* hyper, hipStream_t st);

bool rg_skinny_supported(int I, int O);
int rg_skinny_first_down(const float* x, const float* w, const float* bias, void* y, void* bits, int N, int H, int W, int I,
                         int O, float slope, int dtype, hipStream_t st);
int rg_skinny_sign_pack(const void* a, void* bits, long long npix, int C, int dtype, hipStream_t st);
bool rg_skinny_first_down_masked_supported(int H, int W, int I, int O, int dtype);
int rg_skinny_first_down_masked(const float* x, const float* w, void* y, const void* mask_bits, float mslope, int N, int H,
                                int W, int I, int O, int dtype, hipStream_t st);
int rg_skinny_last_up(const void* x, const float* w, const float* bias, float* y, int N, int Ho, int Wo, int O, int I,
                      int apply_tanh, int dtype, hipStream_t st, const float* pre_mean = nullptr,
                      const float* pre_invstd = nullptr, const float* pre_gamma = nullptr, const float* pre_beta = nullptr,
                      float pre_slope = 1.f, const float* post_tb_img = nullptr, float* post_part = nullptr);
bool rg_skinny_last_up_pre_supported(int Wo, int O, int dtype);
int rg_skinny_last_up_post_blocks(int N, int Ho, int Wo, int O, int dtype);
int rg_skinny_lu_part_final(const float* part, int nb, float* out, int accumulate, int mode, float* loss, float* coef,
                            float lambd, hipStream_t st, float in_scale = 1.f, float out_scale = 1.f,
                            const int* scale_exp = nullptr);
size_t rg_skinny_wgrad_ws_bytes(int N, int Ho, int Wo, int O, int I);
int rg_skinny_wgrad_slabs_impl(const void* low, const float* high_nchw, int N, int Ho, int Wo, int O, int I, int dtype,
                               void* slab, size_t slab_bytes, int* nslab_out, float* bias_slab, int* bias_done_out,
                               hipStream_t st);
int rg_skinny_wgrad_impl(const void* low, const float* high_nchw, float* dw, int N, int Ho, int Wo, int O, int I,
                         int dtype, int accumulate, void* ws, size_t ws_bytes, hipStream_t st, float* dbias = nullptr,
                         int bias_accumulate = 0, int* bias_done_out = nullptr);
```

rna_gan_amd/csrc/rg_skinny.hip:

```cpp
#include "rg_internal.h"
#include <stdlib.h>

namespace {

constexpr int SK_I = 3;
constexpr int SK_K = SK_I * 16;


template <typename T, int OC>
__global__ __launch_bounds__(256) void first_down_kernel(const float* __restrict__ x, const float* __restrict__ wq,
                                                         const float* __restrict__ bias, T* __restrict__ y, int N,
                                                         int H, int W, int O, float slope) {
  const int Ho = H >> 1, Wo = W >> 1;
  const long long npix = (long long)N * Ho * Wo;
  const long long p = (long long)blockIdx.x * 256 + threadIdx.x;
  if (p >= npix) return;
  const int wo = (int)(p % Wo);
  const long long tq = p / Wo;
  const int ho = (int)(tq % Ho), n = (int)(tq / Ho);
  float patch[SK_K];
#pragma unroll
  for (int ci = 0; ci < SK_I; ++ci)
#pragma unroll
    for (int kh = 0; kh < 4; ++kh)
// ... 907 lines not shown
        const uint16_t* s1 = ring + ((k - 1) % 3) * SLOT;
        const uint16_t* s2 = slot;
#pragma unroll
        for (int sj = 0; sj < 2; ++sj) {
          const int st = wave + 4 * sj;
          sk_f32x4 acc = {0.f, 0.f, 0.f, 0.f};
          const int aoff = (16 * st + lp) * LU_PXS + 8 * lq;
#pragma unroll
          for (int dw = 0; dw < 3; ++dw)
#pragma unroll
            for (int c = 0; c < 2; ++c) {
              const int o = aoff + dw * LU_PXS + 32 * c;
              sk_bf16x8 a0 = __builtin_bit_cast(sk_bf16x8, *reinterpret_cast<const uint4*>(s0 + o));
              sk_bf16x8 a1 = __builtin_bit_cast(sk_bf16x8, *reinterpret_cast<const uint4*>(s1 + o));
              sk_bf16x8 a2 = __builtin_bit_cast(sk_bf16x8, *reinterpret_cast<const uint4*>(s2 + o));
              acc = rg_mfma_h16_16x16x32(a0, wf[0][dw][c], acc, 0, 0, 0);
              acc = rg_mfma_h16_16x16x32(a1, wf[1][dw][c], acc, 0, 0, 0);
              acc = rg_mfma_h16_16x16x32(a2, wf[2][dw][c], acc, 0, 0, 0);
            }
          if (ni < SK_I) {
            float* orow = outt + (ni * 2 + nph) * LU_OS + 2 * (16 * st + 4 * lq) + npw;
#pragma unroll
            for (int r = 0; r < 4; ++r) {
              float v = acc[r] + bv;
              if (apply_tanh) v = sk_fast_tanh(v);
              orow[2 * r] = v;
            }
          }
        }
        __syncthreads();
        float4 v4 = *reinterpret_cast<const float4*>(outt + rid4 * LU_OS + 4 * m4);
        float2 v2 = *reinterpret_cast<const float2*>(outt + rid2 * LU_OS + 2 * m2);
        if (TB) {
          v4 = make_float4(v4.x * (1.f - im4.x * im4.x), v4.y * (1.f - im4.y * im4.y), v4.z * (1.f - im4.z * im4.z),
                           v4.w * (1.f - im4.w * im4.w));
          v2 = make_float2(v2.x * (1.f - im2.x * im2.x), v2.y * (1.f - im2.y * im2.y));
        }
        *reinterpret_cast<float4*>(y + oi4) = v4;
        *reinterpret_cast<float2*>(y + oi2) = v2;
        if (PART) {
          const float s4 = (v4.x + v4.y) + (v4.z + v4.w), s2 = v2.x + v2.y;
          const int i4 = rid4 >> 1;
          pc0 += i4 == 0 ? s4 : 0.f; pc1 += i4 == 1 ? s4 : 0.f; pc2 += s2;
          pq += ((v4.x * v4.x + v4.y * v4.y) + (v4.z * v4.z + v4.w * v4.w)) + (v2.x * v2.x + v2.y * v2.y);
        }
      }
    };
    step(0, ra, false);
    step(1, rb, false);
    step(2, ra, true);
    step(3, rb, true);
#pragma unroll 1
    for (int k = 4; k < STRIP + 2; k += 2) {
      step(k, ra, true);
      step(k + 1, rb, true);
    }
  }
  if (PART) {
    float vals[4] = {pc0, pc1, pc2, pq};
#pragma unroll
    for (int k = 0; k < 4; ++k)
#pragma unroll
      for (int o = 32; o > 0; o >>= 1) vals[k] += __shfl_xor(vals[k], o, 64);
    __syncthreads();
    if (lane == 0) {
#pragma unroll
      for (int k = 0; k < 4; ++k) outt[wave * 4 + k] = vals[k];
    }
    __syncthreads();
    if (t < 4) post.part[(size_t)blockIdx.x * 4 + t] = (outt[t] + outt[4 + t]) + (outt[8 + t] + outt[12 + t]);
  }
}

typedef __attribute__((ext_vector_type(4))) unsigned sk_u32x4;
struct Sw128Low { sk_u32x4 v0, v1, v2, v3; };
__device__ __forceinline__ void sw128_load_low(Sw128Low& r, const uint16_t* __restrict__ low, int u, int t) {
  const uint16_t* src = low + (size_t)u * R128_WO * 64 + (size_t)t * 8;
  r.v0 = *reinterpret_cast<const sk_u32x4*>(src);
  r.v1 = *reinterpret_cast<const sk_u32x4*>(src + 2048);
  r.v2 = *reinterpret_cast<const sk_u32x4*>(src + 4096);
  r.v3 = *reinterpret_cast<const sk_u32x4*>(src + 6144);
}

__global__ __launch_bounds__(256, 2) void skinny_wgrad_rows128_kernel(const uint16_t* __restrict__ low,
                                                                      const float* __restrict__ x, float* __restrict__ slab,
                                                                      int nunits, float* __restrict__ bias_slab) {
  __shared__ __attribute__((aligned(16))) uint16_t pt2[2][(SK_K + 1) * SW_PTS];
  __shared__ __attribute__((aligned(16))) uint16_t lt2[2][128 * 64];
  uint16_t* const lt = lt2[0];
  const int t = threadIdx.x, lane = t & 63, wave = t >> 6;
  const int r = lane & 31, h = lane >> 5;
  sk_f32x16 acc[2][2];
#pragma unroll
  for (int i = 0; i < 2; ++i)
#pragma unroll
    for (int j = 0; j < 2; ++j)
#pragma unroll
      for (int e = 0; e < 16; ++e) acc[i][j][e] = 0.f;
  const int grp16 = lane >> 4, idx = lane & 15, q4 = idx >> 2, p4 = idx & 3, fh = grp16 >> 1, cb = grp16 & 1;
  const int per = (nunits + gridDim.x - 1) / gridDim.x;
  const int u0 = blockIdx.x * per, u1 = min(nunits, u0 + per);
  if (u0 < u1) {
    fd128_zero_edges<SW_PTS>(pt2[0], t);
    fd128_zero_edges<SW_PTS>(pt2[1], t);
    if (t < SW_PTS) { pt2[0][SK_K * SW_PTS + t] = RG_H16_ONE; pt2[1][SK_K * SW_PTS + t] = RG_H16_ONE; }
    Fd128Rows ra, rb;
    Sw128Low la, lb;
    fd128_load(ra, x, u0, wave, lane);
    sw128_load_low(la, low, u0, t);
    fd128_load(rb, x, min(u0 + 1, u1 - 1), wave, lane);
    sw128_load_low(lb, low, min(u0 + 1, u1 - 1), t);
    auto step = [&](int u, Fd128Rows& cur, Sw128Low& lcur, uint16_t* ptu, uint16_t* ltu) __attribute__((always_inline)) {
      fd128_scatter<SW_PTS>(ptu, cur, fd128_row_ok(u, wave), wave, lane);
      {
        const int px = t >> 3, c = t & 7;
        uint16_t* d = ltu + px * 64 + ((c ^ (((px >> 1) & 1) << 2)) << 3);
        *reinterpret_cast<sk_u32x4*>(d) = lcur.v0;
        *reinterpret_cast<sk_u32x4*>(d + 32 * 64) = lcur.v1;
        *reinterpret_cast<sk_u32x4*>(d + 64 * 64) = lcur.v2;
        *reinterpret_cast<sk_u32x4*>(d + 96 * 64) = lcur.v3;
      }
      __syncthreads();
      fd128_load(cur, x, min(u + 2, u1 - 1), wave, lane);
      sw128_load_low(lcur, low, min(u + 2, u1 - 1), t);
#pragma unroll
      for (int ks = 0; ks < 2; ++ks) {
        const int prow = wave * 32 + ks * 16 + 8 * fh + q4;
        const int sw = ((prow >> 1) & 1) << 2;
        sk_bf16x8 fa[2], fb[2];
#pragma unroll
        for (int i = 0; i < 2; ++i) {
          const int c = 4 * i + 2 * cb + (p4 >> 1);
          const uint16_t* ap = ltu + prow * 64 + ((c ^ sw) << 3) + (p4 & 1) * 4;
          sk_s16x4 lo = sk_tr_read(ap), hi = sk_tr_read(ap + 4 * 64);
          fa[i] = __builtin_bit_cast(sk_bf16x8, __builtin_shufflevector(lo, hi, 0, 1, 2, 3, 4, 5, 6, 7));
          const int k = 32 * i + r;
          fb[i] = __builtin_bit_cast(sk_bf16x8, *reinterpret_cast<const uint4*>(ptu + (k <= SK_K ? k : 0) * SW_PTS +
                                                                                wave * 32 + ks * 16 + 8 * h));
        }
#pragma unroll
        for (int i = 0; i < 2; ++i)
#pragma unroll
          for (int j = 0; j < 2; ++j) acc[i][j] = rg_mfma_h16_32x32x16(fa[i], fb[j], acc[i][j], 0, 0, 0);
      }
    };
    int u = u0;
    if (u + 1 < u1) {
      step(u, ra, la, pt2[0], lt2[0]);
      step(u + 1, rb, lb, pt2[1], lt2[1]);
      u += 2;
#pragma unroll 1
      for (; u + 1 < u1; u += 2) {
        step(u, ra, la, pt2[0], lt2[0]);
        step(u + 1, rb, lb, pt2[1], lt2[1]);
      }
    }
    if (u < u1) step(u, ra, la, pt2[0], lt2[0]);
  }
  __syncthreads();
  float* red = reinterpret_cast<float*>(lt);
  for (int i = t; i < 64 * SK_K + 64; i += 256) red[i] = 0.f;
  __syncthreads();
  for (int wv = 0; wv < 4; ++wv) {
    if (wave == wv) {
#pragma unroll
      for (int i = 0; i < 2; ++i)
#pragma unroll
        for (int j = 0; j < 2; ++j) {
          const int k = 32 * j + r;
          if (k < SK_K) {
#pragma unroll
            for (int e = 0; e < 16; ++e) red[(32 * i + (e & 3) + 8 * (e >> 2) + 4 * h) * SK_K + k] += acc[i][j][e];
          } else if (k == SK_K) {
#pragma unroll
            for (int e = 0; e < 16; ++e) red[64 * SK_K + 32 * i + (e & 3) + 8 * (e >> 2) + 4 * h] += acc[i][j][e];
          }
        }
    }
    __syncthreads();
  }
  float* sl = slab + (size_t)blockIdx.x * 64 * SK_K;
  for (int i = t; i < 64 * SK_K; i += 256) sl[i] = red[i];
  if (bias_slab && t < 64) bias_slab[(size_t)blockIdx.x * 64 + t] = red[64 * SK_K + t];
}

constexpr int SK_ROWS_BLOCKS = 768;
bool sk_rows128(int H, int W) { return H == R128_H && W == R128_W && rg_option("skinny128", 1) != 0; }
bool sk_rows_chunk(int Wo, int* chunk) {
  if (Wo >= 128 && Wo % 128 == 0) { *chunk = 128; return true; }
  if (Wo == 32 || Wo == 64) { *chunk = Wo; return true; }
  return false;
}

int skinny_wgrad_blocks(long long npix, int* ppb) {
  long long want = 512;
  long long per = (npix + want - 1) / want;
  per = (per + 63) / 64 * 64;
  if (per < 64) per = 64;
  *ppb = (int)per;
  return (int)((npix + per - 1) / per);
}

}
// ... 112 lines not shown
                            float lambd, hipStream_t st, float in_scale, float out_scale, const int* scale_exp) {
  hipLaunchKernelGGL(lu_part_final_kernel, dim3(1), dim3(256), 0, st, part, nb, out, accumulate, mode, loss, coef, lambd,
                     1.f / in_scale, out_scale, scale_exp);
  RG_LAUNCH_CHECK("last_up_post_final");
  return RG_OK;
}
int rg_skinny_last_up(const void* x, const float* w, const float* bias, float* y, int N, int Ho, int Wo, int O, int I,
                      int apply_tanh, int dtype, hipStream_t st, const float* pre_mean, const float* pre_invstd,
                      const float* pre_gamma, const float* pre_beta, float pre_slope, const float* post_tb_img,
                      float* post_part) {
  const LuPre pre{pre_mean, pre_invstd, pre_gamma, pre_beta, pre_slope};
  const LuPost post{post_tb_img, post_part};
  RG_REQUIRE(!(post_tb_img || post_part) || rg_skinny_last_up_post_blocks(N, Ho, Wo, O, dtype) > 0, RG_EUNSUPPORTED,
             "last_up: fused output epilogue");
  RG_REQUIRE(!pre_mean || rg_skinny_last_up_pre_supported(Wo, O, dtype), RG_EUNSUPPORTED, "last_up: fused BatchNorm input");
  (void)I;
  static int lu_valu = -1;
  if (lu_valu < 0) { const char* e = getenv("RNAGAN_SKINNY_VALU"); lu_valu = (e && e[0] == '1') ? 1 : 0; }
  int chunk;
  if (dtype == RG_H16 && O == 64 && sk_rows_chunk(Wo, &chunk) && !lu_valu) {
    int strip = Ho < 16 ? Ho : 16;
    while (Ho % strip) --strip;
    long long nstrips = (long long)N * (Ho / strip) * (Wo / chunk);
    int blocks = nstrips < 512 ? (int)nstrips : 512;
    if (sk_rows128(2 * Ho, 2 * Wo)) {
#define LU128(PRE_, TB_, PART_)                                                                                          \
  hipLaunchKernelGGL((last_up_rows128_kernel<PRE_, TB_, PART_>), dim3(blocks), dim3(256), 0, st, (const uint16_t*)x, w, bias, \
                     y, apply_tanh, (int)nstrips, pre, post)
      if (pre_mean) {
        RG_REQUIRE(!post_tb_img && !post_part, RG_EUNSUPPORTED, "last_up: fused input and output passes together");
        LU128(true, false, false);
      } else if (post_tb_img) {
        if (post_part) LU128(false, true, true); else LU128(false, true, false);
      } else {
        if (post_part) LU128(false, false, true); else LU128(false, false, false);
      }
#undef LU128
      RG_LAUNCH_CHECK("last_up(128)");
      return RG_OK;
    }
    hipLaunchKernelGGL(last_up_rows_kernel, dim3(blocks), dim3(256), 0, st, (const uint16_t*)x, w, bias, y, N, Ho, Wo,
                       apply_tanh, chunk, strip, (int)nstrips, pre, post);
    RG_LAUNCH_CHECK("last_up(mfma)");
    return RG_OK;
  }
  if (dtype == RG_H16) {
    constexpr int TH = 8;
    int tiles = ((Wo + LU_TW - 1) / LU_TW) * ((Ho + TH - 1) / TH);
    size_t sh = (size_t)(TH + 2) * (LU_TW + 2) * (O * 2 + 8);
    hipLaunchKernelGGL((last_up_kernel<h16_t, TH>), dim3((unsigned)((long long)N * tiles)), dim3(TH * 32), sh, st,
                       (const h16_t*)x, w, bias, y, N, Ho, Wo, O, apply_tanh);
  } else if (dtype == RG_F32) {
    if (O % 16 == 0 && !getenv("RNAGAN_LASTUP_WHOLE")) {
      constexpr int TH = 4, CCH = 16;
      int tiles = ((Wo + LU_TW - 1) / LU_TW) * ((Ho + TH - 1) / TH);
      size_t sh = (size_t)(TH + 2) * (LU_TW + 2) * (CCH * 4 + 8);
      hipLaunchKernelGGL((last_up_kernel<float, TH, CCH>), dim3((unsigned)((long long)N * tiles)), dim3(TH * 32), sh, st,
                         (const float*)x, w, bias, y, N, Ho, Wo, O, apply_tanh);
    } else {
      constexpr int TH = 2;
      int tiles = ((Wo + LU_TW - 1) / LU_TW) * ((Ho + TH - 1) / TH);
      size_t sh = (size_t)(TH + 2) * (LU_TW + 2) * (O * 4 + 8);
      hipLaunchKernelGGL((last_up_kernel<float, TH>), dim3((unsigned)((long long)N * tiles)), dim3(TH * 32), sh, st,
                         (const float*)x, w, bias, y, N, Ho, Wo, O, apply_tanh);
    }
  } else {
    rg_set_error("bad dtype %d", dtype);
    return RG_EINVAL;
  }
  RG_LAUNCH_CHECK("last_up");
  return RG_OK;
}

constexpr int SKW_BLOCKS = SK_ROWS_BLOCKS;

size_t rg_skinny_wgrad_ws_bytes(int N, int Ho, int Wo, int O, int I) {
  (void)I;
  int ppb;
  int nb = skinny_wgrad_blocks((long long)N * Ho * Wo, &ppb);
  if (nb < SKW_BLOCKS) nb = SKW_BLOCKS;
  return (size_t)nb * (O * SK_K + 64) * sizeof(float);
}

int rg_skinny_wgrad_slabs_impl(const void* low, const float* high_nchw, int N, int Ho, int Wo, int O, int I, int dtype,
                               void* slab, size_t slab_bytes, int* nslab_out, float* bias_slab, int* bias_done_out,
                               hipStream_t st) {
  (void)I;
  *nslab_out = 0;
  if (bias_done_out) *bias_done_out = 0;
  const size_t elems = (size_t)O * SK_K;
  const long long npix = (long long)N * Ho * Wo;
  int chunk;
  if (!(dtype == RG_H16 && O == 64 && sk_rows_chunk(Wo, &chunk) && npix / chunk < 0x7fffffff)) return RG_OK;
  const int nunits = (int)(npix / chunk);
  int nbm = nunits < SK_ROWS_BLOCKS ? nunits : SK_ROWS_BLOCKS;
  if (sk_rows128(2 * Ho, 2 * Wo)) {
    if (nbm > 512) nbm = 512;
    RG_REQUIRE(slab && slab_bytes >= (size_t)nbm * elems * sizeof(float), RG_EWORKSPACE, "skinny_wgrad_slabs: buffer too small");
    hipLaunchKernelGGL(skinny_wgrad_rows128_kernel, dim3(nbm), dim3(256), 0, st, (const uint16_t*)low, high_nchw, (float*)slab,
                       nunits, bias_slab);
    if (bias_done_out) *bias_done_out = bias_slab ? 1 : 0;
  } else {
    RG_REQUIRE(slab && slab_bytes >= (size_t)nbm * elems * sizeof(float), RG_EWORKSPACE, "skinny_wgrad_slabs: buffer too small");
    hipLaunchKernelGGL(skinny_wgrad_rows_kernel, dim3(nbm), dim3(256), 0, st, (const uint16_t*)low, high_nchw, (float*)slab, N,
                       2 * Ho, 2 * Wo, chunk, nunits);
  }
  RG_LAUNCH_CHECK("skinny_wgrad_slabs");
  *nslab_out = nbm;
  return RG_OK;
}

int rg_skinny_wgrad_impl(const void* low, const float* high_nchw, float* dw, int N, int Ho, int Wo, int O, int I,
                         int dtype, int accumulate, void* ws, size_t ws_bytes, hipStream_t st, float* dbias, int bias_accumulate,
                         int* bias_done_out) {
  (void)I;
  int bias_done_local = 0;
  if (!bias_done_out) bias_done_out = &bias_done_local;
  *bias_done_out = 0;
  size_t elems = (size_t)O * SK_K;
  long long npix = (long long)N * Ho * Wo;
  static int no_mfma = -1;
  if (no_mfma < 0) { const char* e = getenv("RNAGAN_SKINNY_VALU"); no_mfma = (e && e[0] == '1') ? 1 : 0; }
  int chunk;
  if (dtype == RG_H16 && O == 64 && sk_rows_chunk(Wo, &chunk) && npix / chunk < 0x7fffffff && !no_mfma) {
    int nunits = (int)(npix / chunk);
    int nbm = nunits < SK_ROWS_BLOCKS ? nunits : SK_ROWS_BLOCKS;
    RG_REQUIRE(ws && ws_bytes >= (size_t)nbm * elems * sizeof(float), RG_EWORKSPACE, "skinny_wgrad: workspace too small");
    if (sk_rows128(2 * Ho, 2 * Wo)) {
      if (nbm > 512) nbm = 512;
      float* bpart = (dbias && ws_bytes >= (size_t)nbm * (elems + 64) * sizeof(float)) ? (float*)ws + (size_t)nbm * elems : nullptr;
      hipLaunchKernelGGL(skinny_wgrad_rows128_kernel, dim3(nbm), dim3(256), 0, st, (const uint16_t*)low, high_nchw, (float*)ws,
                         nunits, bpart);
      RG_LAUNCH_CHECK("skinny_wgrad(128)");
      int rc = rg_reduce_slabs((const float*)ws, dw, elems, nbm, accumulate, 0, 0, st);
      if (rc || !bpart) return rc;
      *bias_done_out = 1;
      return rg_reduce_slabs(bpart, dbias, 64, nbm, bias_accumulate, 0, 0, st);
    }
    hipLaunchKernelGGL(skinny_wgrad_rows_kernel, dim3(nbm), dim3(256), 0, st, (const uint16_t*)low, high_nchw, (float*)ws,
                       N, 2 * Ho, 2 * Wo, chunk, nunits);
    RG_LAUNCH_CHECK("skinny_wgrad(mfma)");
    return rg_reduce_slabs((const float*)ws, dw, elems, nbm, accumulate, 0, 0, st);
  }
  int ppb;
  int nb = skinny_wgrad_blocks(npix, &ppb);
  RG_REQUIRE(ws && ws_bytes >= (size_t)nb * elems * sizeof(float), RG_EWORKSPACE, "skinny_wgrad: workspace too small");
  RG_DISPATCH_DTYPE(dtype, T, {
    hipLaunchKernelGGL((skinny_wgrad_kernel<T>), dim3(nb), dim3(256), 0, st, (const T*)low, high_nchw, (float*)ws, N,
                       Ho, Wo, O, ppb);
    RG_LAUNCH_CHECK("skinny_wgrad");
  })
  return rg_reduce_slabs((const float*)ws, dw, elems, nb, accumulate, 0, 0, st);
}
```

rna_gan_amd/engine.py:

```python
from __future__ import annotations

from typing import List, NamedTuple, Optional

import torch


class ConvW:

    __slots__ = ("w", "bias", "dw", "dbias", "packs", "packs_version", "version", "layout", "shadow",
                 "shadow_version", "_fp8", "fuse_step", "pending_wgrad", "factor_stage", "owner", "defer_slabs",
                 "pending_slabs", "_slab_ws", "wire_slot", "pending_bias", "_bias_ws")

    def __init__(self, w, bias=None, dw=None, dbias=None, layout="OIHW"):
        self.w = w
        self.bias = bias
        self.dw = dw
        self.dbias = dbias
        self.packs = None
        self.packs_version = -1
        self.version = 0
        self.layout = layout
        self.shadow = None
        self.shadow_version = -1
        self._fp8 = None
# ... 372 lines not shown
                    ops.col_sum(p, D.conv0.dbias, True)
    gx = None
    if need_input_grad and input_post is not None:
        fused = ops.last_up_post(gz0, D.conv0, input_post.get("tanh_img"))
        if fused is not None:
            gx, ctx.gx_parts = fused
    if need_input_grad and gx is None:
        gx = ops.last_up(gz0, D.conv0, None, False)
    return gx


def _plain_backward_pair(ops, D: PlainDiscNet, ctx_a, coef_a, ctx_b, coef_b):
    _plain_backward(ops, D, ctx_a, coef_a, "defer", False, False)
    _plain_backward(ops, D, ctx_b, coef_b, True, True, False, partner=ctx_a)


def _plain_loss_grads_batched(ops, G, D: PlainDiscNet, real, noise, grad_scale=1.0, next_noise=None):
    n = real.shape[0]
    fake_next = None
    if next_noise is not None and isinstance(G, GenNet):
        img2 = gen_forward_pair(ops, G, torch.cat([noise, next_noise]))
        img, fake_next = img2[:n], img2[n:]
    else:
        img, _ = _gen_fwd(ops, G, noise, keep=False)
        if next_noise is not None:
            fake_next, _ = _gen_fwd(ops, G, next_noise, keep=False)
    xs = (real, img)
    _refresh(ops, [(cw,) for cw in D.blocks])
    H, W = real.shape[2], real.shape[3]
    C0 = D.conv0.w.shape[0]
    a = torch.empty((2 * n, H // 2, W // 2, C0), dtype=ops.act_dtype, device=real.device)
    bits = ops.sign_bits_for(2 * n, H // 2, W // 2, C0, D.blocks[0].O) if D.blocks else None
    for h in range(2):
        ops.first_down(xs[h], D.conv0, D.conv0.bias, D.slope,
                       out=(a[h * n:(h + 1) * n], None if bits is None else bits[h * n:(h + 1) * n]))
    if bits is not None:
        a._rg_sign_bits = bits
    ctx = _Ctx()
    ctx.x, ctx.a = xs, [a]
    for cw in D.blocks:
        a = ops.conv_down_bias_act(a, cw, cw.bias, D.slope)
        ctx.a.append(a)
    ctx.h, out = ops.head_fwd_bias(a, D.head, D.head.bias, D.last_slope)
    loss = ops.mean_diff(out[n:], out[:n], 1.0)
    gh = torch.cat([ops.head_grad(ctx.h[:n], -grad_scale / n, D.last_slope), ops.head_grad(ctx.h[n:], grad_scale / n, D.last_slope)])
    _plain_backward(ops, D, ctx, None, True, False, False, gh=gh)
    return loss if next_noise is None else (loss, fake_next)


def _plain_gp_second(ops, D: PlainDiscNet, ctx, st, accumulate, need_input_grad):
    R = len(D.blocks)
    g, v = st
    at = ops.first_down_tangent(v, D.conv0, ctx.a[0], D.slope)
    ats = [at]
    for l in range(1, R + 1):
        at = ops.conv_down_mask(at, D.blocks[l - 1], ctx.a[l], D.slope)
        ats.append(at)
    ops.head_wgrad(ctx.gh, ats[R], D.head.dw, accumulate)
    for l in range(R, 0, -1):
        ops.conv_wgrad(ctx.gz1[l], ats[l - 1], D.blocks[l - 1], accumulate)
    ops.skinny_wgrad(ctx.gz1[0], v, D.conv0.dw, accumulate)
    if not accumulate:
        for cw in D.convs():
            ops.zero_(cw.dbias)
    gx = ops.zero_(torch.empty_like(ctx.x)) if need_input_grad else None
    return gx


def gen_forward(ops, G: GenNet, noise, update_running=True, keep=True):
    ctx = _Ctx()
    ctx.noise = noise
    _refresh(ops, G.blocks)
    z = ops.g0_fwd(noise, G.g0)
    a, mean, invstd = _bn_forward(ops, z, G.bn0, G.slope, update_running)
    ctx.z, ctx.mean, ctx.invstd, ctx.a = [z], [mean], [invstd], [a]
    for l, (cw, bn) in enumerate(G.blocks):
        fused_last = not keep and l == len(G.blocks) - 1
        z, st = ops.conv_up(a, cw, want_stats=True, defer=0 if fused_last else 1)
        if not keep and l == len(G.blocks) - 1:
            img = ops.last_up_bn(z, st, bn, G.slope, G.last, G.last.bias, True, update_running)
            if img is not None:
                ctx.img = img
                return img, ctx
        a, mean, invstd = _bn_forward(ops, z, bn, G.slope, update_running, st)
        if keep:
            ctx.z.append(z); ctx.mean.append(mean); ctx.invstd.append(invstd); ctx.a.append(a)
    img = ops.last_up(a, G.last, G.last.bias, True)
    ctx.img = img
    return img, ctx


def _class_partials(st, m_half: int):
    if st is None:
        return None
    rows = st.shape[0]
    if rows % 8:
        return None
    per_class = rows // 4
    if (2 * m_half) % per_class or m_half % ((2 * m_half) // per_class):
        return None
    return st


def gen_forward_pair(ops, G: GenNet, noise2, update_running=True):
    def run(bn):
        return (bn.running_mean, bn.running_var, bn.nbt) if update_running else (None, None, None)
    _refresh(ops, G.blocks)
    z = ops.g0_fwd(noise2, G.g0)
    a, _, _ = ops.bn_forward2(z, G.bn0.gamma, G.bn0.beta, G.slope, G.bn0.eps, G.bn0.momentum, *run(G.bn0))
    for l, (cw, bn) in enumerate(G.blocks):
        z, st = ops.conv_up(a, cw, want_stats=True, defer=0 if l == len(G.blocks) - 1 else 2)
        st = _class_partials(st, a.numel() // a.shape[-1] // 2)
        if l == len(G.blocks) - 1:
            img = ops.last_up_bn2(z, st, bn, G.slope, G.last, G.last.bias, True, update_running)
            if img is not None:
                return img
        a, _, _ = ops.bn_forward2(z, bn.gamma, bn.beta, G.slope, bn.eps, bn.momentum, *run(bn), partials=st, nblk=4)
    return ops.last_up(a, G.last, G.last.bias, True)


def upgen_forward(ops, G: UpGenNet, noise, update_running=True, keep=True):
    ctx = _Ctx()
    ctx.noise = noise
    z = ops.g0_fwd(noise, G.g0)
    a, mean, invstd = _bn_forward(ops, z, G.bn0, G.slope, update_running)
    ctx.z, ctx.mean, ctx.invstd, ctx.a = [z], [mean], [invstd], [a]
    for cw, bn in G.blocks:
        z = ops.upconv3(a, cw, cw.bias)
        a, mean, invstd = _bn_forward(ops, z, bn, G.slope, update_running)
        if keep:
            ctx.z.append(z); ctx.mean.append(mean); ctx.invstd.append(invstd); ctx.a.append(a)
    ctx.a_last = a
    img = ops.upconv3(a, G.last, G.last.bias, out_nchw=True)
    ctx.img = img
    return img, ctx


def upgen_backward(ops, G: UpGenNet, ctx, gimg, accumulate: bool, need_input_grad: bool = False):
    R = len(G.blocks)
    ops.upconv3_wgrad(gimg, ctx.a[R], G.last, accumulate, gy_nchw=True)
    ops.nchw_chan_sum(gimg, G.last.dbias, accumulate)
    ga = ops.upconv3_bwd_data(gimg, G.last, gy_nchw=True)
    for l in range(R, 0, -1):
        cw, bn = G.blocks[l - 1]
        gz, _, _ = ops.bn_act_bwd(ctx.z[l], ga, ctx.mean[l], ctx.invstd[l], bn.gamma, bn.beta,
                                  G.slope, bn.dgamma, bn.dbeta, accumulate)
        ops.upconv3_wgrad(gz, ctx.a[l - 1], cw, accumulate)
        ops.col_sum(gz, cw.dbias, accumulate)
        ga = ops.upconv3_bwd_data(gz, cw)
    gz0, _, _ = ops.bn_act_bwd(ctx.z[0], ga, ctx.mean[0], ctx.invstd[0], G.bn0.gamma, G.bn0.beta,
                               G.slope, G.bn0.dgamma, G.bn0.dbeta, accumulate)
    ops.g0_wgrad(ctx.noise, gz0, G.g0.dw, accumulate)
    return ops.g0_bwd_data(gz0, G.g0) if need_input_grad else None


def _gen_fwd(ops, G, noise, **kw):
    return upgen_forward(ops, G, noise, **kw) if isinstance(G, UpGenNet) else gen_forward(ops, G, noise, **kw)


def _gen_bwd(ops, G, ctx, gimg, accumulate, need_input_grad=False):
    if isinstance(G, UpGenNet):
        return upgen_backward(ops, G, ctx, gimg, accumulate, need_input_grad)
    return gen_backward(ops, G, ctx, gimg, accumulate, need_input_grad)


def gen_backward(ops, G: GenNet, ctx, gimg, accumulate: bool, need_input_grad: bool = False, gzl=None, gzl_parts=None):
    R = len(G.blocks)
    if gzl is None:
        gzl = ops.tanh_bwd(gimg, ctx.img)
    ops.skinny_wgrad(ctx.a[R], gzl, G.last.dw, accumulate)
    if gzl_parts is not None:
        ops.parts_chan_sum(gzl_parts, G.last.dbias, accumulate)
    else:
        ops.nchw_chan_sum(gzl, G.last.dbias, accumulate)
    ga = ops.first_down(gzl, G.last, None, 1.0)
    for l in range(R, 0, -1):
        cw, bn = G.blocks[l - 1]
        gz, _, _ = ops.bn_act_bwd(ctx.z[l], ga, ctx.mean[l], ctx.invstd[l], bn.gamma, bn.beta,
                                  G.slope, bn.dgamma, bn.dbeta, accumulate, keep_ga=False)
        ops.conv_wgrad(ctx.a[l - 1], gz, cw, accumulate)
        ga = ops.conv_down(gz, cw, defer=1)
    gz0, _, _ = ops.bn_act_bwd(ctx.z[0], ga, ctx.mean[0], ctx.invstd[0], G.bn0.gamma, G.bn0.beta,
                               G.slope, G.bn0.dgamma, G.bn0.dbeta, accumulate, keep_ga=False)
    if not ops.g0_wgrad_deferred(ctx.noise, gz0, G.g0, accumulate):
        ops.g0_wgrad(ctx.noise, gz0, G.g0.dw, accumulate)
    gin = ops.g0_bwd_data(gz0, G.g0) if need_input_grad else None
    return gin


def gen_loss_prefix(ops, G, noise):
    return _gen_fwd(ops, G, noise)


def gen_loss_rest(ops, G, D: DiscNet, pre, grad_scale: float = 1.0):
    img, gctx = pre
    n = img.shape[0]
    out, dctx = disc_forward(ops, D, img)
    loss = ops.mean_diff(out, None, -1.0)
    fuse = {"tanh_img": gctx.img} if isinstance(G, GenNet) else None
    gimg = disc_backward(ops, D, dctx, -grad_scale / n, wgrad=False, accumulate=False, need_input_grad=True, input_post=fuse)
    if dctx.gx_parts is not None:
        gen_backward(ops, G, gctx, None, accumulate=False, gzl=gimg, gzl_parts=dctx.gx_parts)
    else:
        _gen_bwd(ops, G, gctx, gimg, accumulate=False)
    return loss


def gen_loss_grads(ops, G: GenNet, D: DiscNet, noise, grad_scale: float = 1.0):
    return gen_loss_rest(ops, G, D, gen_loss_prefix(ops, G, noise), grad_scale)


class DiscPrefix(NamedTuple):
    out_r: object
    ctx_r: object
    backward: object


def disc_loss_prefix(ops, D: DiscNet, real, backward=None, grad_scale: float = 1.0):
    out_r, ctx_r = disc_forward(ops, D, real)
    if backward is not None:
        n = out_r.shape[0]
        disc_backward(ops, D, ctx_r, -grad_scale / n, wgrad=True if backward == "all" else "defer", accumulate=False,
                      need_input_grad=False)
    return DiscPrefix(out_r, None if backward == "all" else ctx_r, backward)


def disc_loss_rest(ops, G, D: DiscNet, pre: DiscPrefix, noise, grad_scale: float = 1.0):
    out_r, ctx_r, backward = pre
    n = out_r.shape[0]
    img, _ = _gen_fwd(ops, G, noise, keep=False)
    out_f, ctx_f = disc_forward(ops, D, img)
    loss = ops.mean_diff(out_f, out_r, 1.0)
    if backward is None:
        disc_backward_pair(ops, D, ctx_r, -grad_scale / n, ctx_f, grad_scale / n)
    else:
        disc_backward(ops, D, ctx_f, grad_scale / n, wgrad=True, accumulate=True, need_input_grad=False,
                      partner=ctx_r if backward == "dgrad" else None)
    return loss


def _half_partials(st, m_half: int, m_total: int, h: int):
    if st is None:
        return None
    rows = st.shape[0]
    if rows % 2 or m_total % rows or m_half % (m_total // rows):
        return None
    return st[h * (rows // 2):(h + 1) * (rows // 2)]


def disc_loss_grads_batched(ops, G, D: DiscNet, real, noise, grad_scale: float = 1.0, next_noise=None):
    if isinstance(D, PlainDiscNet):
        return _plain_loss_grads_batched(ops, G, D, real, noise, grad_scale, next_noise)
    n = real.shape[0]
# ... 240 lines not shown
```

rna_gan_amd/graphed.py:

```python
from __future__ import annotations

import math
import os

import torch

ENABLED = os.environ.get("RNAGAN_GRAPHS", "1") != "0"
WARMUP_CALLS = 2
_captured = []
_POOL = None


def _pool():
    global _POOL
    if os.environ.get("RNAGAN_GRAPH_POOL", "1") == "0":
        return None
    if _POOL is None:
        _POOL = torch.cuda.graph_pool_handle()
    return _POOL


def mark_static(t):
    t._rg_static = True
    return t


class StepGraph:

    def __init__(self, fn, example_inputs, modules, optimizers, stepped=()):
        self.fn = fn
        self.static_in = [t if getattr(t, "_rg_static", False) else t.detach().clone() for t in example_inputs]
        self.modules = modules
        self.optimizers = optimizers
        self.stepped = list(stepped)
        self.graph = None
        self.static_out = None
        self.calls = 0
        self.failed = False
        self._out_spec = None
        self.wire_cell = None
        self._rebuilt = {}

    STABLE_NUMEL = 4096

    @staticmethod
    def _flat(out):
        return list(out) if isinstance(out, (tuple, list)) else [out]

    def _note_outputs(self, out):
        self._out_spec = [(tuple(t.shape), t.dtype, t.device) if torch.is_tensor(t) else None for t in self._flat(out)]
        return out

    def _stable(self, out, bufs):
        res = []
        for t, b in zip(self._flat(out), bufs):
            if b is not None:
                b.copy_(t)
                res.append(b)
            else:
                res.append(t)
        return type(out)(res) if isinstance(out, (tuple, list)) else res[0]

    def _run(self):
        return self.fn(*self.static_in)

    def __call__(self, *inputs, allow_capture=True):
        for i, (s, t) in enumerate(zip(self.static_in, inputs)):
            if s.shape != t.shape:
                raise RuntimeError("StepGraph: input shape changed")
            if s is not t:
                if self.graph is None and getattr(t, "_rg_static", False) and t.dtype == s.dtype:
                    self.static_in[i] = t
                else:
                    s.copy_(t, non_blocking=True)
        self.calls += 1
        if self.failed or self.calls <= WARMUP_CALLS or (self.graph is None and not allow_capture):
            return self._note_outputs(self._run())
        if self.graph is None:
            try:
                torch.cuda.synchronize()
                bufs = [torch.empty(sp[0], dtype=sp[1], device=sp[2])
                        if sp is not None and math.prod(sp[0]) <= self.STABLE_NUMEL else None
                        for sp in (self._out_spec or [])]
                before = {id(m): m.pack_versions() for m in self.modules if getattr(m, "precision", None) == "fp32"}
                g = torch.cuda.CUDAGraph()
                with torch.cuda.graph(g, pool=_pool(), capture_error_mode="thread_local"):
                    out = self._run()
                    self.static_out = self._stable(out, bufs) if len(bufs) == len(self._flat(out)) else out
                self.graph = g
                self._rebuilt = {mid: [cw for cw, pv in snap.items() if cw.packs_version != pv] for mid, snap in before.items()}
                if os.environ.get("RNAGAN_GRAPH_DEBUG"):
                    print("rna_gan_amd: captured graph #%d for %s" % (len(_captured), getattr(self.fn, "__name__", "?")),
                          flush=True)
                _captured.append(self)
            except Exception as e:
                self.failed = True
                print("rna_gan_amd: HIP graph capture failed (%s); continuing without graphs" % str(e)[:200])
                torch.cuda.synchronize()
                return self._run()
        self.graph.replay()
        for t in (self.static_out if isinstance(self.static_out, (tuple, list)) else (self.static_out,)):
            if torch.is_tensor(t):
                t._rg_static = True
        for o in self.optimizers:
            o.note_replayed()
        for m in self.modules:
            m.mark_packs_fresh(only=self._rebuilt.get(id(m)))
        for m in self.stepped:
            m.weights_changed(by_optimizer=True)
        return self.static_out
```

rna_gan_amd/models.py:

```python
from __future__ import annotations

from math import ceil, log2
from typing import List

import torch
import torch.nn as nn

from . import dist as D_
from . import engine as E


def _num_repeats(size: int, what: str) -> int:
    if size < 16 or ceil(log2(size)) != log2(size):
        raise Exception("%s must be at least 16*16 and an exact power of 2" % what)
    return size.bit_length() - 4


def _flat_view(buf, off, n, p):
    if E.is_tap_major(p.data):
        O, I = p.shape[0], p.shape[1]
        return buf[off:off + n].view(O, 4, 4, I).permute(0, 3, 1, 2)
    return buf[off:off + n].view(p.shape)


# ... 44 lines not shown
            if p.grad is None or p.grad.data_ptr() != gbase + self.esize * off:
                p.grad = _flat_view(self.grad, off, n, p)
        return True


class _HipModule(nn.Module):

    def __init__(self):
        super().__init__()
        self._rt_ops = None
        self._rt_net = None
        self._rt_flat = None
        self.precision = "bf16"

    def set_precision(self, precision: str):
        if precision not in ("bf16", "fp32", "fp16"):
            raise ValueError("precision must be 'bf16', 'fp32' or 'fp16'")
        if precision != self.precision:
            self.precision = precision
            self._rt_ops = None
            self._rt_net = None
        return self

    def _build_net(self):
        raise NotImplementedError

    def runtime(self):
        p0 = next(self.parameters())
        if p0.device.type != "cuda":
            raise RuntimeError("%s runs on the HIP kernels only: move it to a ROCm GPU (.to('cuda')); "
                               "there is no CPU fallback" % type(self).__name__)
        if self._rt_flat is None or not self._rt_flat.owns(self):
            E.tap_major_(self)
            self._rt_flat = FlatParams(self)
            self._rt_net = None
        if self._rt_ops is None or self._rt_net is None:
            from .ops_hip import HipOps
            dt = {"bf16": torch.bfloat16, "fp16": torch.float16, "fp32": torch.float32}[self.precision]
            self._rt_ops = D_.attach_sync(HipOps(dt, p0.device))
            if getattr(self, "_amp_scaler", None) is not None:
                self._amp_scaler.attach_ops(self._rt_ops)
            self._rt_net = self._build_net()
            for cw in self._rt_net.convs():
                cw.owner = "D" if hasattr(self, "disc") else "G"
            if self.precision in ("bf16", "fp16") and p0.dtype == torch.float32:
                self._attach_shadows()
        return self._rt_ops, self._rt_net

    def _attach_shadows(self):
        flat = self._rt_flat
        shadow = flat.ensure_shadow(self._rt_ops.h16)
        base = flat.data.data_ptr()
        g0 = getattr(self._rt_net, "g0", None)
        for cw in self._rt_net.convs():
            if cw.layout != "OHWI" and cw is not g0:
                continue
            off = (cw.w.data_ptr() - base) // flat.esize
            n = cw.w.numel()
            cw.shadow = shadow[off:off + n].view(cw.O, 16, cw.I) if cw.layout == "OHWI" else shadow[off:off + n]
            cw.shadow_version = -1

    @property
    def flat(self) -> "FlatParams":
        self.runtime()
        return self._rt_flat

    def weights_changed(self, by_optimizer=False):
        if self._rt_net is not None:
            self._rt_net.bump()
            if by_optimizer and self._rt_flat is not None and self._rt_flat.shadow is not None:
                for cw in self._rt_net.convs():
                    if cw.shadow is not None:
                        cw.shadow_version = cw.version

    def packs_stale(self) -> int:
        if self._rt_net is None:
            return 2
        st = 0
        for cw in self._rt_net.convs():
            if cw.packs is None and self.precision == "fp32":
                continue
            if cw.packs_version != cw.version:
                st = max(st, 2 if (cw.shadow is not None and cw.shadow_version != cw.version) else 1)
        return st

    def mark_packs_fresh(self, only=None):
        if self._rt_net is not None:
            for cw in (self._rt_net.convs() if only is None else only):
                cw.packs_version = cw.version
                if cw.shadow is not None:
                    cw.shadow_version = cw.version

    def pack_versions(self):
        return {} if self._rt_net is None else {cw: cw.packs_version for cw in self._rt_net.convs()}

    def load_state_dict(self, *a, **k):
        D_.flush()
        r = super().load_state_dict(*a, **k)
        self.weights_changed()
        return r

    def state_dict(self, *a, **k):
        D_.flush()
        return super().state_dict(*a, **k)

    def _apply(self, fn, *a, **k):
        r = super()._apply(fn, *a, **k)
        flat = self._rt_flat
        if flat is not None and next(self.parameters()).device == flat.data.device and \
                next(self.parameters()).dtype == flat.data.dtype and flat.owns(self):
            return r
        self._rt_ops = None
        self._rt_net = None
        self._rt_flat = None
        return r


class Generator(_HipModule):

    def __init__(self, encoding_dims, label_type="none"):
        super().__init__()
        self.encoding_dims = encoding_dims
        self.label_type = label_type

    def _weight_initializer(self):
        for m in self.modules():
            if isinstance(m, (nn.ConvTranspose2d, nn.Conv2d, nn.Linear)):
                nn.init.kaiming_normal_(m.weight)
                if m.bias is not None:
                    nn.init.constant_(m.bias, 0.0)
            elif isinstance(m, nn.BatchNorm2d):
                nn.init.constant_(m.weight, 1.0)
                nn.init.constant_(m.bias, 0.0)

    def sampler(self, sample_size, device):
        return [torch.randn(sample_size, self.encoding_dims, device=device)]


class Discriminator(_HipModule):

    def __init__(self, input_dims, label_type="none"):
        super().__init__()
        self.input_dims = input_dims
        self.label_type = label_type

    _weight_initializer = Generator._weight_initializer


class _GenForwardFn(torch.autograd.Function):

    @staticmethod
    def forward(ctx, module, x, *params):
        ops, net = module.runtime()
        img, gctx = E._gen_fwd(ops, net, x, update_running=True)
        ctx.module, ctx.gctx = module, gctx
        return img

    @staticmethod
    def backward(ctx, gimg):
        ops, net = ctx.module.runtime()
        gin = E._gen_bwd(ops, net, ctx.gctx, gimg.contiguous().float(), accumulate=True,
                         need_input_grad=ctx.needs_input_grad[1])
        return (None, gin) + (None,) * len(ctx.module._rt_flat.params)


class _DiscForwardFn(torch.autograd.Function):
# ... 150 lines not shown
```

rna_gan_amd/ops_hip.py:

```python
from __future__ import annotations

import ctypes
import os
import weakref

import torch

from . import _abi
from ._abi import RG_BF16, RG_F16, RG_F32, check
from .engine import ConvW


def _ptr(t):
    return 0 if t is None else t.data_ptr()


class SlabRef:

    __slots__ = ("ws", "nsplit", "stride", "groups", "dtype")

    def __init__(self, ws, nsplit, stride, groups, dtype=RG_F32):
        self.ws, self.nsplit, self.stride, self.groups, self.dtype = ws, nsplit, stride, groups, dtype


# ... 20 lines not shown
_HANDOFF_MSG = ("rna_gan_amd: a fused split-K BatchNorm launch timed out waiting for its workgroups%s: the results of that "
                "launch are invalid.  The kernels need all their <= 256 workgroups co-resident; another kernel (a "
                "collective?) held CUs.  Set RNAGAN_SPLIT_BN_DP=0 / RNAGAN_SPLIT_BN=0 to use the separate launches.")


def check_handoffs():
    from . import dist as D_
    flag = _handoff_flag()
    if D_.active():
        if flag is None:
            dev = torch.device("cuda", torch.cuda.current_device()) if torch.cuda.is_available() else torch.device("cpu")
            flag = torch.zeros(1, dtype=torch.int32, device=dev)
        torch.distributed.all_reduce(flag, op=torch.distributed.ReduceOp.MAX)
    if flag is not None and int(flag.item()) != 0:
        _rearm()
        raise RuntimeError(_HANDOFF_MSG % (" on at least one rank" if D_.active() else ""))


def handoffs_poll_start():
    from . import dist as D_
    flag = _handoff_flag()
    if flag is None:
        if not D_.active() or not torch.cuda.is_available():
            return None
        flag = torch.zeros(1, dtype=torch.int32, device=torch.device("cuda", torch.cuda.current_device()))
    if D_.active():
        torch.distributed.all_reduce(flag, op=torch.distributed.ReduceOp.MAX)
    slot = torch.empty(1, dtype=torch.int32, pin_memory=flag.is_cuda)
    slot.copy_(flag, non_blocking=True)
    ev = None
    if flag.is_cuda:
        ev = torch.cuda.Event()
        ev.record(torch.cuda.current_stream(flag.device))
    return slot, ev, flag


def handoffs_poll_finish(handle):
    if handle is None:
        return
    from . import dist as D_
    slot, ev, _flag = handle
    if ev is not None:
        ev.synchronize()
    if int(slot.item()) != 0:
        _rearm()
        raise RuntimeError(_HANDOFF_MSG % (" on at least one rank" if D_.active() else ""))


class HipOps:
    name = "hip"

    def __init__(self, act_dtype=torch.bfloat16, device="cuda:0", algo=_abi.ALGO_AUTO):
        if not torch.cuda.is_available():
            raise RuntimeError("rna_gan_amd.HipOps needs a ROCm GPU (no CPU fallback exists)")
        if act_dtype not in (torch.float32, torch.bfloat16, torch.float16):
            raise ValueError("act_dtype must be torch.float32, torch.bfloat16 or torch.float16")
        self.half = "f16" if act_dtype == torch.float16 else "bf16"
        self.lib = _abi.load(self.half)
        self.device = torch.device(device)
        self.act_dtype = act_dtype
        self.h16 = torch.float16 if self.half == "f16" else torch.bfloat16
        self.H16 = RG_F16 if self.half == "f16" else RG_BF16
        self.dt = RG_F32 if act_dtype == torch.float32 else self.H16
        self.loss_scale = 1.0
        self.gp_seed_scale = 1.0
        self.gp_tangent_scale = 1.0
        self.amp = None
        self.amp_slot = 0
        if self.half == "f16" and os.environ.get("RNAGAN_F16_LOSS_SCALE", "").strip().lower() == "dynamic":
            from .amp import default_scaler
            self.amp = default_scaler(self.device)
        elif self.half == "f16":
            ls = float(os.environ.get("RNAGAN_F16_LOSS_SCALE", "4096"))
            rt = ls ** 0.5
            if ls < 1.0 or rt != int(rt) or (int(rt) & (int(rt) - 1)) != 0:
                raise ValueError("RNAGAN_F16_LOSS_SCALE must be the square of a power of two (1, 4, 16, ..., 4096, 16384, ...)")
            self.loss_scale, self.gp_seed_scale, self.gp_tangent_scale = ls, rt, rt
        self.algo = algo
        self._wsbuf = None
        self.timing = None
        self._ws_retired = []
        self.fuse_input_post = os.environ.get("RNAGAN_INPUT_POST", "1") != "0"
        self.pack_from_shadow = os.environ.get("RNAGAN_PACK_FROM_SHADOW", "1") != "0"
        self.wgrad_in_step = os.environ.get("RNAGAN_WGRAD_ADAM", "1") != "0"
        self._skinny_defer = None
        self.skinny_bias = os.environ.get("RNAGAN_SKINNY_BIAS", "1") != "0"
        self.epilogue_stats = os.environ.get("RNAGAN_EPILOGUE_STATS", "1") != "0"
        self.stat_reduce = None
        self.stat_world = 1
        self.split_bn = os.environ.get("RNAGAN_SPLIT_BN", "1") != "0"
        self._split_bn_dp = None
        self.f32_planes = int(os.environ.get("RNAGAN_F32_PLANES", "6")) if self.dt == RG_F32 else 0
        if self.f32_planes not in (0, 3, 6):
            raise ValueError("RNAGAN_F32_PLANES must be 0, 3 or 6")
        self.plain_paths = {}
        self._slabs_pending = None
        self._sb_sync = None
        self._sb_scratch = None
        self._sb_retired = []
        _LIVE_OPS.add(self)

    @property
    def stream(self):
        return torch.cuda.current_stream(self.device).cuda_stream

    def _ws(self, nbytes: int):
        nbytes = max(int(nbytes), 256)
        if self._slabs_pending is not None:
            raise RuntimeError("rna_gan_amd: a conv launched with defer= left its split-K slabs in the workspace and another "
                               "op asked for the workspace before the BatchNorm op consumed them")
        if self._wsbuf is None or self._wsbuf.numel() < nbytes:
            if self._wsbuf is not None:
                self._ws_retired.append(self._wsbuf)
            self._wsbuf = torch.empty(int(nbytes * 1.25) + 4096, dtype=torch.uint8, device=self.device)
        return self._wsbuf

    def _sb_bufs(self, M, C, groups):
        if self._sb_sync is None:
            self._sb_sync = torch.zeros(int(self.lib.rg_slab_bn_sync_words()), dtype=torch.int32, device=self.device)
        need = int(self.lib.rg_slab_bn_scratch_bytes(int(M), int(C), int(groups)))
        if self._sb_scratch is None or self._sb_scratch.numel() < need:
            if self._sb_scratch is not None:
                self._sb_retired.append(self._sb_scratch)
            self._sb_scratch = torch.empty(max(need, 1 << 20), dtype=torch.uint8, device=self.device)
        return self._sb_scratch, self._sb_sync

    def _defer_split(self, up, N, Hl, Wl, O, I, rows_out, C, groups):
        if not groups or not self.split_bn or self.dt == RG_F32 or self.stat_reduce is not None or rows_out % groups:
            return 0
        if self._split_bn_dp is None:
            from . import dist as D_
            dflt = "1" if D_.world_size() <= 1 else "0"
            self._split_bn_dp = (not D_.active()) or os.environ.get("RNAGAN_SPLIT_BN_DP", dflt) != "0"
        if not self._split_bn_dp:
            return 0
        ns = int(self.lib.rg_conv_split(up, N, Hl, Wl, O, I, self.dt, self.algo))
        if ns <= 1 or not self.lib.rg_slab_bn_supported(rows_out // groups, C, groups, ns):
            return 0
        return ns

    def _timed(self, key, flops, thunk, cw=None):
        if self.timing is None:
            return thunk()
        e0, e1 = torch.cuda.Event(enable_timing=True), torch.cuda.Event(enable_timing=True)
        e0.record(torch.cuda.current_stream(self.device))
        r = thunk()
        e1.record(torch.cuda.current_stream(self.device))
        self.timing.append((key, float(flops), e0, e1, getattr(cw, "owner", None)))
        return r

    def _act(self, *shape):
        return torch.empty(shape, dtype=self.act_dtype, device=self.device)

    def _f32(self, *shape):
        return torch.empty(shape, dtype=torch.float32, device=self.device)

    def _planes(self, t):
        c = getattr(t, "_rg_planes", None)
        if c is None or c[0] != t._version:
            assert t.dtype == torch.float32 and t.is_contiguous() and t.numel() % 8 == 0
            p = c[1] if c is not None else torch.empty((3, t.numel()), dtype=torch.bfloat16, device=self.device)
            check(self.lib.rg_split_planes(_ptr(t), _ptr(p), t.numel(), self.stream), "rg_split_planes")
            c = t._rg_planes = (t._version, p)
        return c[1]

    def _plane_packs(self, cw: ConvW):
# ... 458 lines not shown
        assert img_nchw.dtype == torch.float32 and img_nchw.is_contiguous()
        y = self._f32(N, H, W, C)
        check(self.lib.rg_export_images_nhwc(_ptr(img_nchw), _ptr(y), N, C, H, W, self.stream), "rg_export_images_nhwc")
        return y

    def upconv3(self, x, cw: ConvW, bias, out_nchw=False):
        N, H, W, Cin = x.shape
        Cout = cw.w.shape[0]
        assert tuple(cw.w.shape) == (Cout, Cin, 3, 3) and cw.w.is_contiguous() and x.is_contiguous()
        y = self._f32(N, Cout, 2 * H, 2 * W) if out_nchw else self._act(N, 2 * H, 2 * W, Cout)
        ws = self._ws(self.lib.rg_upconv3_workspace_bytes(N, H, W, Cin, Cout))
        check(self.lib.rg_upconv3_fwd(_ptr(x), _ptr(cw.w), _ptr(bias), _ptr(y), N, H, W, Cin, Cout, int(out_nchw),
                                      self.dt, self.algo, _ptr(ws), ws.numel(), self.stream), "rg_upconv3_fwd")
        return y

    def _up_dims(self, gy, cw, gy_nchw):
        Cout, Cin = cw.w.shape[0], cw.w.shape[1]
        if gy_nchw:
            N, C, H2, W2 = gy.shape
            assert gy.dtype == torch.float32
        else:
            N, H2, W2, C = gy.shape
        assert C == Cout and gy.is_contiguous()
        return N, H2 // 2, W2 // 2, Cin, Cout

    def upconv3_bwd_data(self, gy, cw: ConvW, gy_nchw=False):
        N, H, W, Cin, Cout = self._up_dims(gy, cw, gy_nchw)
        gx = self._act(N, H, W, Cin)
        ws = self._ws(self.lib.rg_upconv3_workspace_bytes(N, H, W, Cin, Cout))
        check(self.lib.rg_upconv3_bwd_data(_ptr(gy), int(gy_nchw), _ptr(cw.w), _ptr(gx), N, H, W, Cin, Cout, self.dt,
                                           self.algo, _ptr(ws), ws.numel(), self.stream), "rg_upconv3_bwd_data")
        return gx

    def upconv3_wgrad(self, gy, x, cw: ConvW, accumulate: bool, gy_nchw=False):
        N, H, W, Cin, Cout = self._up_dims(gy, cw, gy_nchw)
        assert tuple(x.shape) == (N, H, W, Cin) and x.is_contiguous() and cw.dw.is_contiguous()
        ws = self._ws(self.lib.rg_upconv3_workspace_bytes(N, H, W, Cin, Cout))
        check(self.lib.rg_upconv3_wgrad(_ptr(gy), int(gy_nchw), _ptr(x), _ptr(cw.dw), N, H, W, Cin, Cout, self.dt,
                                        self.algo, int(accumulate), _ptr(ws), ws.numel(), self.stream), "rg_upconv3_wgrad")

    def first_down(self, x_nchw, cw: ConvW, bias, slope: float, out=None):
        N, I, H, W = x_nchw.shape
        O = cw.w.shape[0]
        assert x_nchw.dtype == torch.float32 and x_nchw.is_contiguous() and cw.w.shape[1] == I
        if out is not None:
            y, bits = out
            assert y.shape == (N, H // 2, W // 2, O) and y.is_contiguous() and y.dtype == self.act_dtype
            if bits is not None:
                check(self.lib.rg_first_down_bits(_ptr(x_nchw), _ptr(cw.w), _ptr(bias), _ptr(y), _ptr(bits), N, H, W, I, O,
                                                  float(slope), self.dt, self.stream), "rg_first_down_bits")
            else:
                check(self.lib.rg_first_down(_ptr(x_nchw), _ptr(cw.w), _ptr(bias), _ptr(y), N, H, W, I, O, float(slope),
                                             self.dt, self.stream), "rg_first_down")
            return y
        y = self._act(N, H // 2, W // 2, O)
        if (self.dt != RG_F32 and O == 64 and slope != 1.0 and H % 4 == 0 and W % 4 == 0 and
                self.lib.rg_conv_up_maskbits_supported(N, H // 4, W // 4, 128, 64, self.dt, self.algo)):
            bits = torch.empty((N, H // 2, W // 2), dtype=torch.int64, device=self.device)
            check(self.lib.rg_first_down_bits(_ptr(x_nchw), _ptr(cw.w), _ptr(bias), _ptr(y), _ptr(bits), N, H, W, I, O,
                                              float(slope), self.dt, self.stream), "rg_first_down_bits")
            y._rg_sign_bits = bits
            return y
        check(self.lib.rg_first_down(_ptr(x_nchw), _ptr(cw.w), _ptr(bias), _ptr(y), N, H, W, I, O, float(slope),
                                     self.dt, self.stream), "rg_first_down")
        return y

    def first_down_tangent(self, v_nchw, cw: ConvW, a0, slope: float):
        N, I, H, W = v_nchw.shape
        O = cw.w.shape[0]
        bits = getattr(a0, "_rg_sign_bits", None)
        if bits is not None and self.lib.rg_first_down_masked_supported(H, W, I, O, self.dt):
            y = self._act(N, H // 2, W // 2, O)
            check(self.lib.rg_first_down_masked(_ptr(v_nchw), _ptr(cw.w), _ptr(y), _ptr(bits), float(slope), N, H, W, I, O,
                                                self.dt, self.stream), "rg_first_down_masked")
            return y
        return self.lrelu_bwd(self.first_down(v_nchw, cw, None, 1.0), a0, slope)

    def sign_pack(self, a):
        assert a.dtype == self.h16 and a.shape[-1] == 64 and a.is_contiguous()
        bits = torch.empty(a.shape[:-1], dtype=torch.int64, device=a.device)
        check(self.lib.rg_sign_pack(_ptr(a), _ptr(bits), a.numel() // 64, 64, self.dt, self.stream), "rg_sign_pack")
        return bits

    def last_up_bn(self, z, partials, bn, slope: float, cw: ConvW, bias, tanh: bool, update_running=True):
        N, Ho, Wo, O = z.shape
        I = cw.w.shape[1]
        if self.stat_reduce is not None or not self.lib.rg_last_up_pre_supported(Wo, O, I, self.dt):
            return None
        M, C = self._mc(z)
        rm, rv, nbt = (bn.running_mean, bn.running_var, bn.nbt) if update_running else (None, None, None)
        if partials is not None:
            mean, invstd = self._f32(C), self._f32(C)
            ws = self._ws(32 * 2 * C * 4)
            check(self.lib.rg_bn_finalize_partials(_ptr(partials), partials.shape[0], M, C, float(bn.eps), float(bn.momentum),
                                                   _ptr(mean), _ptr(invstd), _ptr(rm), _ptr(rv), _ptr(nbt), _ptr(ws),
                                                   ws.numel(), self.stream), "rg_bn_finalize_partials")
        else:
            mean, invstd = self.bn_stats_finalize(z, bn.eps, bn.momentum, rm, rv, nbt)
        y = self._f32(N, I, 2 * Ho, 2 * Wo)
        check(self.lib.rg_last_up_pre(_ptr(z), _ptr(cw.w), _ptr(bias), _ptr(y), _ptr(mean), _ptr(invstd), _ptr(bn.gamma),
                                      _ptr(bn.beta), float(slope), N, Ho, Wo, O, I, int(tanh), self.dt, self.stream),
              "rg_last_up_pre")
        return y

    def last_up_bn2(self, z, partials, bn, slope: float, cw: ConvW, bias, tanh: bool, update_running=True):
        N2, Ho, Wo, O = z.shape
        I = cw.w.shape[1]
        n = N2 // 2
        if self.stat_reduce is not None or N2 % 2 or not self.lib.rg_last_up_pre_supported(Wo, O, I, self.dt):
            return None
        M2, C = self._mc(z)
        M = M2 // 2
        rm, rv, nbt = (bn.running_mean, bn.running_var, bn.nbt) if update_running else (None, None, None)
        if partials is not None:
            mean, invstd = self._f32(2, C), self._f32(2, C)
            ws = self._ws(2 * 32 * 2 * C * 4)
            check(self.lib.rg_bn_finalize_partials_g2(_ptr(partials), partials.shape[0] // 2, 4, M, C, float(bn.eps),
                                                      float(bn.momentum), _ptr(mean), _ptr(invstd), _ptr(rm), _ptr(rv),
                                                      _ptr(nbt), _ptr(ws), ws.numel(), self.stream),
                  "rg_bn_finalize_partials_g2")
        else:
            st = [self.bn_stats_finalize(z[h * n:(h + 1) * n], bn.eps, bn.momentum, rm, rv, nbt) for h in range(2)]
            mean, invstd = torch.stack([st[0][0], st[1][0]]), torch.stack([st[0][1], st[1][1]])
        y = self._f32(N2, I, 2 * Ho, 2 * Wo)
        for h in range(2):
            check(self.lib.rg_last_up_pre(_ptr(z[h * n:(h + 1) * n]), _ptr(cw.w), _ptr(bias), _ptr(y[h * n:(h + 1) * n]),
                                          _ptr(mean[h]), _ptr(invstd[h]), _ptr(bn.gamma), _ptr(bn.beta), float(slope), n, Ho, Wo,
                                          O, I, int(tanh), self.dt, self.stream), "rg_last_up_pre")
        return y

    def last_up(self, x, cw: ConvW, bias, tanh: bool):
        N, Ho, Wo, O = x.shape
        I = cw.w.shape[1]
        assert cw.w.shape[0] == O and x.is_contiguous()
        y = self._f32(N, I, 2 * Ho, 2 * Wo)
        check(self.lib.rg_last_up(_ptr(x), _ptr(cw.w), _ptr(bias), _ptr(y), N, Ho, Wo, O, I, int(tanh), self.dt,
                                  self.stream), "rg_last_up")
        return y

    def last_up_post(self, x, cw: ConvW, tanh_img=None):
        N, Ho, Wo, O = x.shape
        I = cw.w.shape[1]
        if not self.fuse_input_post:
            return None
        nb = self.lib.rg_last_up_post_blocks(N, Ho, Wo, O, I, self.dt)
        if nb <= 0:
            return None
        assert cw.w.shape[0] == O and x.is_contiguous()
        assert tanh_img is None or (tanh_img.shape == (N, I, 2 * Ho, 2 * Wo) and tanh_img.is_contiguous()
                                    and tanh_img.dtype == torch.float32)
        y = self._f32(N, I, 2 * Ho, 2 * Wo)
        parts = self._f32(nb, 4)
        check(self.lib.rg_last_up_post(_ptr(x), _ptr(cw.w), _ptr(y), N, Ho, Wo, O, I, self.dt, _ptr(tanh_img), _ptr(parts),
                                       self.stream), "rg_last_up_post")
        return y, parts

    def parts_chan_sum(self, parts, out, accumulate: bool):
        check(self.lib.rg_last_up_part_chan_sum(_ptr(parts), parts.shape[0], _ptr(out), int(accumulate), self.stream),
              "rg_last_up_part_chan_sum")

    def gp_coef_parts(self, parts, lambd: float):
        loss, coef = self._f32(1), self._f32(1)
        if self.amp is not None:
            check(self.lib.rg_gp_coef_parts_scaled_dev(_ptr(parts), parts.shape[0], None, _ptr(loss), _ptr(coef), float(lambd),
                                                       _ptr(self.amp.state), self.amp_slot, self.stream),
                  "rg_gp_coef_parts_scaled_dev")
            return loss, coef
        check(self.lib.rg_gp_coef_parts_scaled(_ptr(parts), parts.shape[0], None, _ptr(loss), _ptr(coef), float(lambd),
                                               float(self.gp_seed_scale), float(self.gp_tangent_scale), self.stream),
              "rg_gp_coef_parts_scaled")
        return loss, coef

    def skinny_wgrad(self, low, high_nchw, dw, accumulate: bool, dbias=None, dbias_accumulate=False):
        N, Ho, Wo, O = low.shape
        I = high_nchw.shape[1]
        assert high_nchw.dtype == torch.float32 and high_nchw.is_contiguous() and low.is_contiguous()
        if not self.skinny_bias:
            dbias = None
        nb = self.lib.rg_skinny_wgrad_workspace_bytes(N, Ho, Wo, O, I)
        cw = self._skinny_defer.get(dw.data_ptr()) if self._skinny_defer else None
        if cw is not None and cw.pending_slabs is None and accumulate:
            cw = None
        if cw is not None and self.dt != RG_F32 and self.stat_reduce is None:
            prev = cw.pending_slabs
            if (prev is None) == bool(accumulate):
                raise RuntimeError("rna_gan_amd: deferred image-side weight gradient: contributions out of order")
            have = 0 if prev is None else prev[1]
            if cw._slab_ws is None or cw._slab_ws.numel() < 2 * nb + 4096:
                if prev is not None:
                    raise RuntimeError("rna_gan_amd: deferred image-side weight gradient: the slab buffer grew between two contributions")
                self._ws_retired.extend(b for b in (cw._slab_ws, cw._bias_ws) if b is not None)
                cw._slab_ws = torch.empty(2 * nb + 4096, dtype=torch.uint8, device=self.device)
                cw._bias_ws = torch.empty(2 * 1024 * O, dtype=torch.float32, device=self.device)
            want_bias = (dbias is not None and cw.bias is not None and cw.dbias is not None and
                         dbias.data_ptr() == cw.dbias.data_ptr() and O == 64)
            bprev = cw.pending_bias
            if want_bias and (bprev is None) == bool(dbias_accumulate):
                want_bias = False
            bhave = 0 if bprev is None else bprev[1]
            off = have * O * 48 * 4
            ns, bdone = ctypes.c_int(0), ctypes.c_int(0)
            check(self.lib.rg_skinny_wgrad_slabs(_ptr(low), _ptr(high_nchw), N, Ho, Wo, O, I, self.dt, cw._slab_ws.data_ptr() + off,
                                                 cw._slab_ws.numel() - off, ctypes.addressof(ns),
                                                 cw._bias_ws.data_ptr() + bhave * O * 4 if want_bias else 0,
                                                 ctypes.addressof(bdone), self.stream), "rg_skinny_wgrad_slabs")
            if ns.value > 0:
                cw.pending_slabs = (cw._slab_ws, have + int(ns.value), RG_F32)
                if want_bias and bdone.value:
                    if bhave + ns.value > 2 * 1024:
                        raise RuntimeError("rna_gan_amd: deferred bias-gradient partials exceed their buffer")
                    cw.pending_bias = (cw._bias_ws, bhave + int(ns.value))
                    return True
                return False
            if prev is not None:
                raise RuntimeError("rna_gan_amd: deferred image-side weight gradient: the second contribution has no slab form")
        ws = self._ws(nb)
        bdone = ctypes.c_int(0)
        check(self.lib.rg_skinny_wgrad_bias(_ptr(low), _ptr(high_nchw), _ptr(dw), _ptr(dbias), N, Ho, Wo, O, I, self.dt,
                                            int(accumulate), int(dbias_accumulate), _ptr(ws), ws.numel(), ctypes.addressof(bdone),
                                            self.stream), "rg_skinny_wgrad_bias")
        return bool(bdone.value)

    def g0_pack(self, cw: ConvW):
        E, C = cw.w.shape[0], cw.w.shape[1]
        if True:
            if cw.packs is None or cw.packs_version != cw.version:
                if cw.packs is None:
                    cw.packs = (torch.empty((16 * C, E), dtype=self.h16, device=self.device),)
                if cw.shadow is not None and cw.shadow_version == cw.version and self.pack_from_shadow:
                    check(self.lib.rg_pack_g0_weight_from_bf16(_ptr(cw.shadow), _ptr(cw.packs[0]), E, C, self.stream),
                          "rg_pack_g0_weight_from_bf16")
                else:
                    check(self.lib.rg_pack_g0_weight(_ptr(cw.w), _ptr(cw.packs[0]), E, C, self.H16, self.stream),
                          "rg_pack_g0_weight")
                cw.packs_version = cw.version
                if cw.shadow is not None:
                    cw.shadow_version = cw.version

    def g0_fwd(self, z, cw: ConvW):
        N, E = z.shape
        C = cw.w.shape[1]
        assert z.dtype == torch.float32 and z.is_contiguous() and cw.w.shape[0] == E
        wp = None
        if self.dt != RG_F32:
            self.g0_pack(cw)
            wp = cw.packs[0]
        y = self._act(N, 4, 4, C)
        ws = self._ws(self.lib.rg_g0_workspace_bytes(N, E, C, self.dt, self.algo))
        check(self.lib.rg_g0_fwd(_ptr(z), _ptr(cw.w), _ptr(wp), _ptr(y), N, E, C, self.dt, self.algo, _ptr(ws),
                                 ws.numel(), self.stream), "rg_g0_fwd")
        return y

    def g0_wgrad_deferred(self, z, gy, cw: ConvW, accumulate: bool):
        if not cw.fuse_step or accumulate or self.stat_reduce is not None:
            return False
        N, E = z.shape
        C = gy.shape[3]
        if not self.lib.rg_g0_wgrad_adam_supported(N, E, C, self.dt) or not z.is_contiguous() or not gy.is_contiguous():
            if cw.factor_stage is not None:
                raise RuntimeError("g0_wgrad_deferred: the data-parallel runner announced gathered factors for a shape the "
                                   "fused kernel does not take")
            return False
        if cw.factor_stage is not None:
            zs, gs = cw.factor_stage
            zs.copy_(z)
            gs.copy_(gy.reshape(gs.shape))
            cw.pending_wgrad = "staged"
            return True
        cw.pending_wgrad = (z, gy, self.dt)
        return True

    def g0_wgrad(self, z, gy, dw, accumulate: bool):
        N, E = z.shape
        C = gy.shape[3]
        ws = self._ws(self.lib.rg_g0_workspace_bytes(N, E, C, self.dt, self.algo))
        check(self.lib.rg_g0_wgrad(_ptr(z), _ptr(gy), _ptr(dw), N, E, C, self.dt, int(accumulate), self.algo,
                                   _ptr(ws), ws.numel(), self.stream), "rg_g0_wgrad")

    def g0_bwd_data(self, gz0, cw: ConvW):
        N, C = gz0.shape[0], gz0.shape[3]
        E = cw.w.shape[0]
        assert tuple(cw.w.shape) == (E, C, 4, 4) and cw.w.is_contiguous()
        x = gz0.float().reshape(N, 16, C).permute(0, 2, 1).contiguous().reshape(N, C * 16)
        return self.linear_affine_act(x, cw.w.reshape(E, C * 16), None, None, 1.0)

    def head_fwd(self, a, cw: ConvW, slope: float):
        N, C = a.shape[0], a.shape[3]
        assert a.shape[1] == 4 and a.shape[2] == 4 and a.is_contiguous()
        h, out = self._f32(N), self._f32(N)
        check(self.lib.rg_head_fwd(_ptr(a), _ptr(cw.w), _ptr(h), _ptr(out), N, C, float(slope), self.dt,
                                   self.stream), "rg_head_fwd")
        return h, out

    def head_grad(self, h, coef: float, slope: float, part: int = 0):
        gh = torch.empty_like(h)
        if self.amp is not None:
            check(self.lib.rg_head_grad_dev(_ptr(h), _ptr(gh), h.numel(), float(coef), _ptr(self.amp.state), self.amp_slot,
                                            int(part), float(slope), self.stream), "rg_head_grad_dev")
            return gh
        check(self.lib.rg_head_grad(_ptr(h), _ptr(gh), h.numel(), float(coef), float(slope), self.stream),
# ... 358 lines not shown
```

rna_gan_amd/optim.py:

```python
from __future__ import annotations

import torch

from .models import _flat_view

from . import _abi
from ._abi import check


class Adam(torch.optim.Adam):
    def __init__(self, params, lr=1e-3, betas=(0.9, 0.999), eps=1e-8, weight_decay=0, amsgrad=False, **kw):
        if amsgrad:
            raise NotImplementedError("rna_gan_amd.optim.Adam: amsgrad is not on the RNA-GAN path")
        super().__init__(params, lr=lr, betas=betas, eps=eps, weight_decay=weight_decay, amsgrad=False,
                         foreach=False, fused=False)
        self._module = None
        self._m = None
        self._v = None
        self._flat_id = None
        self._step_dev = None
        self._hyper = None
        self._host_steps = 0
        self.buf_gen = 0
        self.grad_wire = None
        self._ema = None

    def bind(self, module, fuse_linear_wgrad=False):
        mine = {id(p) for g in self.param_groups for p in g["params"]}
        theirs = list(module.parameters())
        if len(self.param_groups) != 1 or mine != {id(p) for p in theirs}:
            raise ValueError("rna_gan_amd.optim.Adam: one param group holding exactly module.parameters() is required "
                             "(the fused kernel steps the module's whole flat buffer)")
        if not all(p.requires_grad for p in theirs):
            raise ValueError("rna_gan_amd.optim.Adam: frozen parameters (requires_grad=False) are not supported")
        self._module = module
        if fuse_linear_wgrad:
            module._fuse_linear_wgrad = True
            if hasattr(module, "_trt"):
                module._trt = None
        return self

    def attach_ema(self, ema):
        if self._module is None or ema.source is not self._module:
            raise ValueError("rna_gan_amd.optim.Adam: attach_ema needs an optimizer bound to the module the ParamEMA averages")
        if self._ema is not None and self._ema is not ema:
            raise RuntimeError("rna_gan_amd.optim.Adam: another ParamEMA is attached (detach_ema() first)")
        from . import dist as D_
        D_.flush()
        ema._attach(self)
        self._ema = ema
        self.buf_gen += 1
        return ema

    def detach_ema(self):
        ema, self._ema = self._ema, None
        if ema is not None:
            from . import dist as D_
            D_.flush()
            ema._detach()
            self.buf_gen += 1
        return ema

    def _ensure(self):
        if self._module is None:
            raise RuntimeError("rna_gan_amd.optim.Adam must be bound to its module (Adam(...).bind(module))")
        flat = self._module.flat
        if self._flat_id is not flat:
            old = {p: self.state.get(p) for p in flat.params}
            self._m = torch.zeros_like(flat.data)
            self._v = torch.zeros_like(flat.data)
            step0 = 0
            for p, (off, n) in zip(flat.params, flat.offsets):
                st = old.get(p) or {}
                m = _flat_view(self._m, off, n, p)
                v = _flat_view(self._v, off, n, p)
                if "exp_avg" in st:
                    m.copy_(st["exp_avg"]); v.copy_(st["exp_avg_sq"])
                step0 = max(step0, int(float(st.get("step", 0))))
                self.state[p] = {"step": torch.tensor(float(step0)), "exp_avg": m, "exp_avg_sq": v}
            self._host_steps = step0
            self._step_dev = torch.tensor([step0], dtype=torch.int32, device=flat.data.device)
            self._hyper = torch.zeros(12, dtype=torch.float32, device=flat.data.device)
            self._flat_id = flat
            self.buf_gen += 1
        if self._ema is not None and not torch.cuda.is_current_stream_capturing() and self._ema._rehomed():
            self.buf_gen += 1
        return flat

    def _sync_step_state(self):
        for p in (self._flat_id.params if self._flat_id is not None else []):
            self.state[p]["step"] = torch.tensor(float(self._host_steps))

    def _amp(self):
        return getattr(getattr(self._module, "_rt_ops", None), "amp", None) if self._module is not None else None

    def state_dict(self):
        from . import dist as D_
        D_.flush()
        if self._amp() is not None and self._step_dev is not None:
            self._host_steps = int(self._step_dev.item())
        self._sync_step_state()
        return super().state_dict()

    def load_state_dict(self, state_dict):
        from . import dist as D_
        D_.flush()
        super().load_state_dict(state_dict)
        flat = self._flat_id
        if flat is None or self._module is None or self._module._rt_flat is not flat:
            self._flat_id = None
            return
        step0 = 0
        with torch.no_grad():
            for p, (off, n) in zip(flat.params, flat.offsets):
                st = self.state.get(p) or {}
                m, v = _flat_view(self._m, off, n, p), _flat_view(self._v, off, n, p)
                if "exp_avg" in st:
                    m.copy_(st["exp_avg"]); v.copy_(st["exp_avg_sq"])
                else:
                    m.zero_(); v.zero_()
                step0 = max(step0, int(float(st.get("step", 0))))
                self.state[p] = {"step": torch.tensor(float(step0)), "exp_avg": m, "exp_avg_sq": v}
            self._step_dev.fill_(step0)
        self._host_steps = step0

    def zero_grad(self, set_to_none: bool = False):
        if self._module is not None and not set_to_none:
            from . import dist as D_
            D_.flush()
            self._module.flat.grad.zero_()

    def note_replayed(self):
        self._host_steps += 1
        if self._ema is not None:
            self._ema.module.weights_changed()

    @torch.no_grad()
    def step(self, closure=None):
        flat = self._ensure()
        g = self.param_groups[0]
        mops = getattr(self._module, "_rt_ops", None)
        lib = mops.lib if mops is not None else _abi.load()
        ginv = 1.0 / float(getattr(mops, "loss_scale", 1.0)) if mops is not None else 1.0
        stream = torch.cuda.current_stream(flat.data.device).cuda_stream
        amp = getattr(mops, "amp", None) if mops is not None else None
        launches, probes = [], []
        if amp is None:
            check(lib.rg_adam_hyper_dev2(self._step_dev.data_ptr(), float(g["lr"]), float(g["betas"][0]),
                                         float(g["betas"][1]), float(g["eps"]), float(g.get("weight_decay", 0.0)), ginv,
                                         self._hyper.data_ptr(), stream),
                  "rg_adam_hyper_dev2")
        H16 = getattr(mops, "H16", _abi.RG_BF16)

        def seg(t, n=None, dt=None):
            if torch.is_tensor(t):
                return (t.data_ptr(), t.numel() if n is None else n, _abi.RG_F32 if t.dtype == torch.float32 else H16)
            return (t, n, dt)
        shadow = flat.shadow
        lo = 0
        g0 = getattr(getattr(self._module, "_rt_net", None), "g0", None)
        pend = None if g0 is None else g0.pending_wgrad
        if pend is not None:
            g0.pending_wgrad = None
            z, gy, dt = pend
            off = (g0.w.data_ptr() - flat.data.data_ptr()) // 4
            n0 = g0.w.numel()
            if off != 0:
                raise RuntimeError("rna_gan_amd.optim.Adam: the deferred G.0 weight gradient expects that tensor at the head "
                                   "of the flat buffer")
            E, C = g0.w.shape[0], g0.w.shape[1]
            launches.append(lambda z=z, gy=gy, E=E, C=C, dt=dt: check(lib.rg_g0_wgrad_adam(
                z.data_ptr(), gy.data_ptr(), flat.data.data_ptr(), self._m.data_ptr(), self._v.data_ptr(),
                self._hyper.data_ptr(), 0 if shadow is None else shadow.data_ptr(), z.shape[0], E, C, dt, stream),
                "rg_g0_wgrad_adam"))
            probes += [seg(z), seg(gy)]
            lo = n0
        segs = []
        pend_lin = getattr(self._module, "_rg_pending_linear", None)
        if pend_lin:
            self._module._rg_pending_linear = []
            if shadow is not None or self.grad_wire is not None:
                raise RuntimeError("rna_gan_amd.optim.Adam: fused linear weight gradients expect an fp32-only, single-process step")
            for w, gT, xT, nsamp, pack in pend_lin:
                off = (w.data_ptr() - flat.data.data_ptr()) // 4
                O_, I_ = w.shape
                if not w.is_contiguous() or off < 0 or off + O_ * I_ > flat.data.numel():
                    raise RuntimeError("rna_gan_amd.optim.Adam: a pending linear weight is not a dense view of the flat buffer")
                img = None if pack is None else pack["image"]
                launches.append(lambda gT=gT, xT=xT, nsamp=nsamp, off=off, O_=O_, I_=I_, img=img: check(lib.rg_linear_wgrad_adam(
                    gT.data_ptr(), xT.data_ptr(), gT.shape[1], nsamp, flat.data.data_ptr() + 4 * off,
                    self._m.data_ptr() + 4 * off, self._v.data_ptr() + 4 * off, self._hyper.data_ptr(), O_, I_,
                    0 if img is None else img.data_ptr(), 0 if img is None else img.shape[1], stream), "rg_linear_wgrad_adam"))
                probes += [seg(gT), seg(xT)]
                if pack is not None:
                    pack["version"] = w._version
                segs.append((off, off + O_ * I_))
            segs.sort()
        slab_segs = []
        net = getattr(self._module, "_rt_net", None)
        for cw in (net.convs() if net is not None and hasattr(net, "convs") else []):
            ps = getattr(cw, "pending_slabs", None)
            if ps is not None:
                cw.pending_slabs = None
                slab_segs.append(((cw.w.data_ptr() - flat.data.data_ptr()) // 4, cw.w.numel(), ps[0], ps[1], ps[2]))
            pb = getattr(cw, "pending_bias", None)
            if pb is not None:
                cw.pending_bias = None
                slab_segs.append(((cw.bias.data_ptr() - flat.data.data_ptr()) // 4, cw.bias.numel(), pb[0], pb[1], 0))
            pw = getattr(cw, "pending_wgrad", None)
            if isinstance(pw, tuple) and isinstance(pw[0], str) and pw[0] == "conv":
                cw.pending_wgrad = None
                _, low0, high0, low1, high1, (N_, Ho_, Wo_, O_, I_), dt, algo, flops = pw
                off = (cw.w.data_ptr() - flat.data.data_ptr()) // 4
                if shadow is None or off % 4 or off < lo:
                    raise RuntimeError("rna_gan_amd.optim.Adam: a deferred single-launch weight gradient expects a bf16 step and "
                                       "a 16-byte aligned tensor inside the flat buffer")
                ops = getattr(self._module, "_rt_ops", None)
                call = lambda low0=low0, high0=high0, low1=low1, high1=high1, off=off, N_=N_, Ho_=Ho_, Wo_=Wo_, O_=O_, I_=I_, \
                    dt=dt, algo=algo: check(lib.rg_conv_wgrad_adam(
                    low0.data_ptr(), high0.data_ptr(), 0 if low1 is None else low1.data_ptr(),
                    0 if high1 is None else high1.data_ptr(), flat.data.data_ptr() + 4 * off, self._m.data_ptr() + 4 * off,
                    self._v.data_ptr() + 4 * off, self._hyper.data_ptr(), shadow.data_ptr() + 2 * off, N_, Ho_, Wo_, O_, I_, dt,
                    algo, stream), "rg_conv_wgrad_adam")
                if ops is not None and hasattr(ops, "_timed"):
                    launches.append(lambda call=call, flops=flops, cw=cw, ops=ops: ops._timed("conv_wgrad_adam", flops, call, cw=cw))
                else:
                    launches.append(call)
                probes += [seg(t) for t in (low0, high0, low1, high1) if t is not None]
                slab_segs.append((off, cw.w.numel(), None, -1, 0))
        if slab_segs:
            if segs or self.grad_wire is not None:
                raise RuntimeError("rna_gan_amd.optim.Adam: deferred split-K slabs expect a single-process step without fused "
                                   "linear weight gradients")
            import ctypes as C
            slab_segs.sort(key=lambda t: t[0])
            total = flat.data.numel()
            table, pos = [], lo
            for off, n, buf, ns, sdt in slab_segs:
                if off < pos or off % 4 or n % 4 or off + n > total:
                    raise RuntimeError("rna_gan_amd.optim.Adam: a deferred weight gradient does not sit 16-byte aligned inside "
                                       "the part of the flat buffer this launch steps")
                if off > pos:
                    table.append((pos - lo, off - pos, 0, 0, 0))
                table.append((off - lo, n, 0 if buf is None else buf.data_ptr(), ns, sdt))
                pos = off + n
            if total > pos:
                table.append((pos - lo, total - pos, 0, 0, 0))
            k = len(table)
            offs = (C.c_ulonglong * k)(*[t[0] for t in table])
            lens = (C.c_ulonglong * k)(*[t[1] for t in table])
            slabs = (C.c_void_p * k)(*[t[2] or None for t in table])
            nsp = (C.c_int * k)(*[t[3] for t in table])
            sdts = (C.c_int * k)(*[t[4] for t in table])
            launches.append(lambda k=k, offs=offs, lens=lens, slabs=slabs, nsp=nsp, sdts=sdts: check(lib.rg_adam_step_slabs(
                flat.data.data_ptr() + 4 * lo, flat.grad.data_ptr() + 4 * lo, self._m.data_ptr() + 4 * lo,
                self._v.data_ptr() + 4 * lo, total - lo, self._hyper.data_ptr(),
                0 if shadow is None else shadow.data_ptr() + 2 * lo, k, C.addressof(offs), C.addressof(lens),
                C.addressof(slabs), C.addressof(nsp), C.addressof(sdts), stream), "rg_adam_step_slabs"))
            for off, n, sp, ns, sdt in table:
                if sp:
                    probes.append(seg(sp, ns * n, _abi.RG_F32 if sdt == _abi.RG_F32 else H16))
                elif ns == 0:
                    probes.append(seg(flat.grad.data_ptr() + 4 * (lo + off), n, _abi.RG_F32))
            segs = [(lo, total)]
        pos = lo
        wire = self.grad_wire
        for a, b in segs + [(flat.data.numel(), flat.data.numel())]:
            if a > pos:
                launches.append(lambda pos=pos, a=a: check(lib.rg_adam_step_dev(
                    flat.data.data_ptr() + 4 * pos, flat.grad.data_ptr() + 4 * pos, self._m.data_ptr() + 4 * pos,
                    self._v.data_ptr() + 4 * pos, a - pos, self._hyper.data_ptr(),
                    0 if shadow is None else shadow.data_ptr() + 2 * pos, 0 if wire is None else wire.data_ptr() + 2 * pos,
                    stream), "rg_adam_step_dev"))
                probes.append(seg(flat.grad.data_ptr() + 4 * pos, a - pos, _abi.RG_F32) if wire is None else
                              seg(wire.data_ptr() + 2 * pos, a - pos, H16))
            pos = max(pos, b)
        if amp is not None:
            amp.probe(lib, self._module, probes, stream)
            amp.hyper(lib, self._module, self._step_dev, g, self._hyper, stream)
        for fn in launches:
            fn()
        if self._ema is not None:
            self._ema._launch(lib, self._hyper, self._step_dev, stream)
        if amp is not None:
            amp.update(lib, self._module, stream)
        if not torch.cuda.is_current_stream_capturing():
            self._host_steps += 1
        self._module.weights_changed(by_optimizer=True)
        return None
```

Before: 6020 imgs/sec.

## Fuse G0 weight packing into Adam step and BN-activation into skinny wgrad

The G0 weight-gradient Adam kernel gains a PACK variant. It restages the updated 16-bit weights through shared memory and writes the packed forward-weight layout directly, so a separate pack pass after the optimizer is no longer needed. Separately, the skinny wgrad kernels gain a PRE mode that applies BN normalization and leaky-ReLU to the stored pre-activation z on the fly. This lets the last up-block skip materializing its activation. Both add template variants and extra register and shared-memory work inside already heavy kernels.

```diff
diff --git a/include/rnagan_hip.h b/include/rnagan_hip.h
--- a/include/rnagan_hip.h
+++ b/include/rnagan_hip.h
@@ -83,6 +83,14 @@
 int rg_last_up_pre(const void* z, const float* w, const float* bias, float* y_nchw, const float* mean, const float* invstd,
                    const float* gamma, const float* beta, float slope, int N, int Ho, int Wo, int O, int I, int apply_tanh,
                    int dtype, void* stream);
+int rg_skinny_wgrad_pre_supported(int N, int Ho, int Wo, int O, int I, int dtype);
+int rg_skinny_wgrad_bias_pre(const void* z, const float* high_nchw, float* dw, float* dbias, const float* mean,
+                             const float* invstd, const float* gamma, const float* beta, float slope, int N, int Ho, int Wo,
+                             int O, int I, int dtype, int accumulate, int bias_accumulate, void* ws, size_t ws_bytes,
+                             int* bias_done_out, void* stream);
+int rg_skinny_wgrad_slabs_pre(const void* z, const float* high_nchw, const float* mean, const float* invstd, const float* gamma,
+                              const float* beta, float slope, int N, int Ho, int Wo, int O, int I, int dtype, void* slab,
+                              size_t slab_bytes, int* nslab_out, float* bias_slab, int* bias_done_out, void* stream);
 size_t rg_skinny_wgrad_workspace_bytes(int N, int Ho, int Wo, int O, int I);
 int rg_skinny_wgrad(const void* low, const float* high_nchw, float* dw, int N, int Ho, int Wo, int O, int I,
                     int dtype, int accumulate, void* ws, size_t ws_bytes, void* stream);
@@ -146,6 +154,8 @@
 int rg_g0_wgrad_adam_supported(int N, int E, int C, int dtype);
 int rg_g0_wgrad_adam(const float* z, const void* gz0, float* p, float* m, float* v, const float* hyper, void* shadow_bf16,
                      int N, int E, int C, int dtype, void* stream);
+int rg_g0_wgrad_adam_pack(const float* z, const void* gz0, float* p, float* m, float* v, const float* hyper, void* shadow_bf16,
+                          void* wp, int N, int E, int C, int dtype, void* stream);
 
 int rg_linear_wgrad_adam(const void* gT, const void* xT, int ldn, int N, float* p, float* m, float* v, const float* hyper, int O,
                          int I, void* wpack_bf16, int Kp, void* stream);
diff --git a/rna_gan_amd/_abi.py b/rna_gan_amd/_abi.py
--- a/rna_gan_amd/_abi.py
+++ b/rna_gan_amd/_abi.py
@@ -46,6 +46,9 @@
     "rg_skinny_wgrad": (_i, [_p, _p, _p, _i, _i, _i, _i, _i, _i, _i, _p, _z, _p]),
     "rg_skinny_wgrad_slabs": (_i, [_p, _p, _i, _i, _i, _i, _i, _i, _p, _z, _p, _p, _p, _p]),
     "rg_skinny_wgrad_bias": (_i, [_p, _p, _p, _p, _i, _i, _i, _i, _i, _i, _i, _i, _p, _z, _p, _p]),
+    "rg_skinny_wgrad_pre_supported": (_i, [_i, _i, _i, _i, _i, _i]),
+    "rg_skinny_wgrad_bias_pre": (_i, [_p, _p, _p, _p, _p, _p, _p, _p, _f, _i, _i, _i, _i, _i, _i, _i, _i, _p, _z, _p, _p]),
+    "rg_skinny_wgrad_slabs_pre": (_i, [_p, _p, _p, _p, _p, _p, _f, _i, _i, _i, _i, _i, _i, _p, _z, _p, _p, _p, _p]),
     "rg_pack_g0_weight": (_i, [_p, _p, _i, _i, _i, _p]),
     "rg_pack_conv_wup_from_bf16": (_i, [_p, _p, _i, _i, _p]),
     "rg_pack_conv_wup_from_bf16_multi": (_i, [_i, _p, _p, _p, _p, _p]),
@@ -146,6 +149,7 @@
     "rg_selftest_fp8": (_i, [_p, _p]),
     "rg_g0_wgrad_adam_supported": (_i, [_i, _i, _i, _i]),
     "rg_g0_wgrad_adam": (_i, [_p, _p, _p, _p, _p, _p, _p, _i, _i, _i, _i, _p]),
+    "rg_g0_wgrad_adam_pack": (_i, [_p, _p, _p, _p, _p, _p, _p, _p, _i, _i, _i, _i, _p]),
     "rg_im2col_nhwc": (_i, [_p, _i, _p, _i, _i, _i, _i, _i, _i, _i, _i, _i, _i, _p]),
     "rg_pool2d_nhwc": (_i, [_p, _i, _p, _i, _i, _i, _i, _i, _i, _i, _i, _i, _p]),
     "rg_nchw_to_nhwc_affine": (_i, [_p, _p, _i, _i, _i, _i, _p, _p, _p]),
@@ -189,7 +193,7 @@
     "rg_probe_fill_bf16": (_i, [_p, _z, C.c_uint, _p]),
 }
 
-ABI_VERSION = 616
+ABI_VERSION = 617
 
 _libs = {}
 LIB_PATH_F16 = os.path.join(_HERE, "librnagan_hip_f16.so")
diff --git a/rna_gan_amd/csrc/rg_api.hip b/rna_gan_amd/csrc/rg_api.hip
--- a/rna_gan_amd/csrc/rg_api.hip
+++ b/rna_gan_amd/csrc/rg_api.hip
@@ -15,7 +15,7 @@
   va_end(ap);
 }
 
-extern "C" int rg_version(void) { return 616; }
+extern "C" int rg_version(void) { return 617; }
 extern "C" const char* rg_last_error(void) { return g_err; }
 
 static const char* const g_opt_names[] = {"conv8", "conv8_blocks", "conv_tile", "xcd", "class_fast", "wgrad_blocks",
@@ -341,6 +341,32 @@
   if (!rg_skinny_supported(I, O)) return RG_OK;
   return rg_skinny_wgrad_slabs_impl(low, high_nchw, N, Ho, Wo, O, I, dtype, slab, slab_bytes, nslab_out, bias_slab, bias_done_out,
                                     rg_stream(stream));
+}
+
+extern "C" int rg_skinny_wgrad_pre_supported(int N, int Ho, int Wo, int O, int I, int dtype) {
+  return rg_skinny_supported(I, O) && rg_skinny_wgrad_pre_ok(N, Ho, Wo, O, dtype) ? 1 : 0;
+}
+extern "C" int rg_skinny_wgrad_bias_pre(const void* z, const float* high_nchw, float* dw, float* dbias, const float* mean,
+                                        const float* invstd, const float* gamma, const float* beta, float slope, int N, int Ho,
+                                        int Wo, int O, int I, int dtype, int accumulate, int bias_accumulate, void* ws,
+                                        size_t ws_bytes, int* bias_done_out, void* stream) {
+  RG_REQUIRE(z && high_nchw && dw && bias_done_out && mean && invstd && gamma && beta, RG_EINVAL, "skinny_wgrad_bias_pre: bad args");
+  *bias_done_out = 0;
+  RG_REQUIRE(rg_skinny_wgrad_pre_supported(N, Ho, Wo, O, I, dtype), RG_EUNSUPPORTED, "skinny_wgrad_bias_pre: shape");
+  return rg_skinny_wgrad_impl(z, high_nchw, dw, N, Ho, Wo, O, I, dtype, accumulate, ws, ws_bytes, rg_stream(stream), dbias,
+                              bias_accumulate, bias_done_out, mean, invstd, gamma, beta, slope);
+}
+extern "C" int rg_skinny_wgrad_slabs_pre(const void* z, const float* high_nchw, const float* mean, const float* invstd,
+                                         const float* gamma, const float* beta, float slope, int N, int Ho, int Wo, int O, int I,
+                                         int dtype, void* slab, size_t slab_bytes, int* nslab_out, float* bias_slab,
+                                         int* bias_done_out, void* stream) {
+  RG_REQUIRE(z && high_nchw && slab && nslab_out && mean && invstd && gamma && beta &&
+                 (bias_slab == nullptr || bias_done_out != nullptr), RG_EINVAL, "skinny_wgrad_slabs_pre: bad args");
+  *nslab_out = 0;
+  if (bias_done_out) *bias_done_out = 0;
+  RG_REQUIRE(rg_skinny_wgrad_pre_supported(N, Ho, Wo, O, I, dtype), RG_EUNSUPPORTED, "skinny_wgrad_slabs_pre: shape");
+  return rg_skinny_wgrad_slabs_impl(z, high_nchw, N, Ho, Wo, O, I, dtype, slab, slab_bytes, nslab_out, bias_slab, bias_done_out,
+                                    rg_stream(stream), mean, invstd, gamma, beta, slope);
 }
 
 extern "C" int rg_pack_conv_wup_from_bf16(const void* w_bf16, void* wup, int O, int I, void* stream) {
diff --git a/rna_gan_amd/csrc/rg_g0adam.hip b/rna_gan_amd/csrc/rg_g0adam.hip
--- a/rna_gan_amd/csrc/rg_g0adam.hip
+++ b/rna_gan_amd/csrc/rg_g0adam.hip
@@ -15,13 +15,15 @@
 constexpr int GA_CP = GA_J + 4;
 constexpr int GA_P = 72;
 
-template <typename TG>
+constexpr int GA_TP = 33;
+template <typename TG, bool PACK>
 __global__ __launch_bounds__(256) void g0_wgrad_adam_kernel(const float* __restrict__ z, const TG* __restrict__ gz0,
                                                             float* __restrict__ p, float* __restrict__ m, float* __restrict__ v,
                                                             const float* __restrict__ hyper, uint16_t* __restrict__ shadow,
-                                                            int N, int E, int C, int e_fastest) {
+                                                            uint16_t* __restrict__ pack, int N, int E, int C, int e_fastest) {
   constexpr int OPS = (GA_E + GA_J) * GA_P * 2;
   static_assert(32 * GA_CP * 4 <= OPS, "accumulator tile must fit into the operand area");
+  static_assert(GA_J * GA_TP * 4 <= OPS, "restaged 16-bit tile must fit into the operand area");
   __shared__ __attribute__((aligned(16))) unsigned char smem[OPS];
   if (hyper[9] != 0.f) return;
   uint16_t* zsT = reinterpret_cast<uint16_t*>(smem);
@@ -119,6 +121,7 @@
   const size_t ld = (size_t)C * 16;
   const int tj = t & 63, te = t >> 6;
   const size_t col = (size_t)c0 * 16 + 4 * tj;
+  uint32_t hw[2][2][2][4];
 #pragma unroll
   for (int i = 0; i < 2; ++i) {
     __syncthreads();
@@ -149,10 +152,36 @@
         *reinterpret_cast<float4*>(p + idx) = P[k];
         *reinterpret_cast<float4*>(m + idx) = M[k];
         *reinterpret_cast<float4*>(v + idx) = V[k];
-        if (shadow)
-          *reinterpret_cast<uint2*>(shadow + idx) = make_uint2((uint32_t)f32_to_h16(P[k].x) | ((uint32_t)f32_to_h16(P[k].y) << 16),
-                                                               (uint32_t)f32_to_h16(P[k].z) | ((uint32_t)f32_to_h16(P[k].w) << 16));
-      }
+        const uint32_t h[4] = {f32_to_h16(P[k].x), f32_to_h16(P[k].y), f32_to_h16(P[k].z), f32_to_h16(P[k].w)};
+        if (shadow) *reinterpret_cast<uint2*>(shadow + idx) = make_uint2(h[0] | (h[1] << 16), h[2] | (h[3] << 16));
+        if constexpr (PACK) {
+#pragma unroll
+          for (int q = 0; q < 4; ++q) {
+            if (k & 1) hw[i][k0 >> 2][k >> 1][q] |= h[q] << 16;
+            else hw[i][k0 >> 2][k >> 1][q] = h[q];
+          }
+        }
+      }
+    }
+  }
+  if constexpr (PACK) {
+    uint32_t* tw = reinterpret_cast<uint32_t*>(smem);
+    __syncthreads();
+#pragma unroll
+    for (int i = 0; i < 2; ++i)
+#pragma unroll
+      for (int kq = 0; kq < 2; ++kq)
+#pragma unroll
+        for (int kp = 0; kp < 2; ++kp)
+#pragma unroll
+          for (int q = 0; q < 4; ++q) tw[(4 * tj + q) * GA_TP + 16 * i + 4 * te + 2 * kq + kp] = hw[i][kq][kp][q];
+    __syncthreads();
+#pragma unroll
+    for (int k = 0; k < 8; ++k) {
+      const int idx = t + 256 * k, j = idx >> 3, pc = idx & 7;
+      const uint32_t* src = tw + j * GA_TP + 4 * pc;
+      const size_t prow = (size_t)(j & 15) * C + c0 + (j >> 4);
+      *reinterpret_cast<uint4*>(pack + prow * E + e0 + 8 * pc) = make_uint4(src[0], src[1], src[2], src[3]);
     }
   }
 }
@@ -296,25 +325,40 @@
   return N > 0 && E % GA_E == 0 && C % 16 == 0 && (dtype == RG_H16 || dtype == RG_F32) ? 1 : 0;
 }
 
-extern "C" int rg_g0_wgrad_adam(const float* z, const void* gz0, float* p, float* m, float* v, const float* hyper,
-                                void* shadow_bf16, int N, int E, int C, int dtype, void* stream) {
-  RG_REQUIRE(z && gz0 && p && m && v && hyper, RG_EINVAL, "g0_wgrad_adam: null");
-  RG_REQUIRE(rg_g0_wgrad_adam_supported(N, E, C, dtype), RG_EUNSUPPORTED, "g0_wgrad_adam: E %% 64 == 0 and C %% 16 == 0 required");
+namespace {
+int g0_wgrad_adam_launch(const char* what, bool pack, const float* z, const void* gz0, float* p, float* m, float* v,
+                         const float* hyper, void* shadow, void* wp, int N, int E, int C, int dtype, void* stream) {
+  RG_REQUIRE(z && gz0 && p && m && v && hyper && (wp || !pack), RG_EINVAL, "%s: null", what);
+  RG_REQUIRE(rg_g0_wgrad_adam_supported(N, E, C, dtype), RG_EUNSUPPORTED, "%s: E %% 64 == 0 and C %% 16 == 0 required", what);
   RG_REQUIRE((((uintptr_t)p | (uintptr_t)m | (uintptr_t)v | (uintptr_t)z | (uintptr_t)gz0) & 15) == 0 &&
-                 (((uintptr_t)shadow_bf16) & 7) == 0, RG_EINVAL, "g0_wgrad_adam: 16-byte aligned buffers required");
+                 (((uintptr_t)shadow) & 7) == 0 && (((uintptr_t)wp) & 15) == 0, RG_EINVAL, "%s: 16-byte aligned buffers required", what);
   static int order = -1;
   if (order < 0) { const char* e = getenv("RNAGAN_G0ADAM_ORDER"); order = e ? atoi(e) : 1; }
   const int e_fastest = order != 0;
   const dim3 grid(e_fastest ? (unsigned)(E / GA_E) : (unsigned)(C / 16), e_fastest ? (unsigned)(C / 16) : (unsigned)(E / GA_E));
   hipStream_t st = rg_stream(stream);
-  if (dtype == RG_H16)
-    hipLaunchKernelGGL(g0_wgrad_adam_kernel<h16_t>, grid, dim3(256), 0, st, z, (const h16_t*)gz0, p, m, v, hyper,
-                       (uint16_t*)shadow_bf16, N, E, C, e_fastest);
-  else
-    hipLaunchKernelGGL(g0_wgrad_adam_kernel<float>, grid, dim3(256), 0, st, z, (const float*)gz0, p, m, v, hyper,
-                       (uint16_t*)shadow_bf16, N, E, C, e_fastest);
-  RG_LAUNCH_CHECK("g0_wgrad_adam");
+#define RG_G0ADAM_LAUNCH(TG, PK) \
+  hipLaunchKernelGGL((g0_wgrad_adam_kernel<TG, PK>), grid, dim3(256), 0, st, z, (const TG*)gz0, p, m, v, hyper, (uint16_t*)shadow, \
+                     (uint16_t*)wp, N, E, C, e_fastest)
+  if (dtype == RG_H16) {
+    if (pack) RG_G0ADAM_LAUNCH(h16_t, true); else RG_G0ADAM_LAUNCH(h16_t, false);
+  } else {
+    if (pack) RG_G0ADAM_LAUNCH(float, true); else RG_G0ADAM_LAUNCH(float, false);
+  }
+#undef RG_G0ADAM_LAUNCH
+  RG_LAUNCH_CHECK(what);
   return RG_OK;
+}
+}
+
+extern "C" int rg_g0_wgrad_adam(const float* z, const void* gz0, float* p, float* m, float* v, const float* hyper,
+                                void* shadow_bf16, int N, int E, int C, int dtype, void* stream) {
+  return g0_wgrad_adam_launch("g0_wgrad_adam", false, z, gz0, p, m, v, hyper, shadow_bf16, nullptr, N, E, C, dtype, stream);
+}
+
+extern "C" int rg_g0_wgrad_adam_pack(const float* z, const void* gz0, float* p, float* m, float* v, const float* hyper,
+                                     void* shadow_bf16, void* wp, int N, int E, int C, int dtype, void* stream) {
+  return g0_wgrad_adam_launch("g0_wgrad_adam_pack", true, z, gz0, p, m, v, hyper, shadow_bf16, wp, N, E, C, dtype, stream);
 }
 
 extern "C" int rg_linear_wgrad_adam(const void* gT, const void* xT, int ldn, int N, float* p, float* m, float* v,
diff --git a/rna_gan_amd/csrc/rg_internal.h b/rna_gan_amd/csrc/rg_internal.h
--- a/rna_gan_amd/csrc/rg_internal.h
+++ b/rna_gan_amd/csrc/rg_internal.h
@@ -169,7 +169,11 @@
 size_t rg_skinny_wgrad_ws_bytes(int N, int Ho, int Wo, int O, int I);
 int rg_skinny_wgrad_slabs_impl(const void* low, const float* high_nchw, int N, int Ho, int Wo, int O, int I, int dtype,
                                void* slab, size_t slab_bytes, int* nslab_out, float* bias_slab, int* bias_done_out,
-                               hipStream_t st);
+                               hipStream_t st, const float* pre_mean = nullptr, const float* pre_invstd = nullptr,
+                               const float* pre_gamma = nullptr, const float* pre_beta = nullptr, float pre_slope = 1.f);
+bool rg_skinny_wgrad_pre_ok(int N, int Ho, int Wo, int O, int dtype);
 int rg_skinny_wgrad_impl(const void* low, const float* high_nchw, float* dw, int N, int Ho, int Wo, int O, int I,
                          int dtype, int accumulate, void* ws, size_t ws_bytes, hipStream_t st, float* dbias = nullptr,
-                         int bias_accumulate = 0, int* bias_done_out = nullptr);
+                         int bias_accumulate = 0, int* bias_done_out = nullptr, const float* pre_mean = nullptr,
+                         const float* pre_invstd = nullptr, const float* pre_gamma = nullptr, const float* pre_beta = nullptr,
+                         float pre_slope = 1.f);
diff --git a/rna_gan_amd/csrc/rg_skinny.hip b/rna_gan_amd/csrc/rg_skinny.hip
--- a/rna_gan_amd/csrc/rg_skinny.hip
+++ b/rna_gan_amd/csrc/rg_skinny.hip
@@ -1013,9 +1013,10 @@
   r.v3 = *reinterpret_cast<const sk_u32x4*>(src + 6144);
 }
 
+template <bool PRE>
 __global__ __launch_bounds__(256, 2) void skinny_wgrad_rows128_kernel(const uint16_t* __restrict__ low,
                                                                       const float* __restrict__ x, float* __restrict__ slab,
-                                                                      int nunits, float* __restrict__ bias_slab) {
+                                                                      int nunits, float* __restrict__ bias_slab, LuPre pre) {
   __shared__ __attribute__((aligned(16))) uint16_t pt2[2][(SK_K + 1) * SW_PTS];
   __shared__ __attribute__((aligned(16))) uint16_t lt2[2][128 * 64];
   uint16_t* const lt = lt2[0];
@@ -1031,6 +1032,26 @@
   const int grp16 = lane >> 4, idx = lane & 15, q4 = idx >> 2, p4 = idx & 3, fh = grp16 >> 1, cb = grp16 & 1;
   const int per = (nunits + gridDim.x - 1) / gridDim.x;
   const int u0 = blockIdx.x * per, u1 = min(nunits, u0 + per);
+  float pm[8], pr[8], pb[8];
+  if (PRE) {
+#pragma unroll
+    for (int j = 0; j < 8; ++j) {
+      const int c = (t & 7) * 8 + j;
+      pm[j] = pre.mean[c]; pr[j] = pre.invstd[c] * pre.gamma[c]; pb[j] = pre.beta[c];
+    }
+  }
+  auto bn8 = [&](sk_u32x4 v) -> sk_u32x4 {
+    if (!PRE) return v;
+    uint32_t d[4] = {v.x, v.y, v.z, v.w};
+#pragma unroll
+    for (int j = 0; j < 4; ++j) {
+      const float lo = lrelu_f((h16_to_f32((uint16_t)d[j]) - pm[2 * j]) * pr[2 * j] + pb[2 * j], pre.slope);
+      const float hi = lrelu_f((h16_to_f32((uint16_t)(d[j] >> 16)) - pm[2 * j + 1]) * pr[2 * j + 1] + pb[2 * j + 1], pre.slope);
+      d[j] = sk_pack2(lo, hi);
+    }
+    sk_u32x4 o = {d[0], d[1], d[2], d[3]};
+    return o;
+  };
   if (u0 < u1) {
     fd128_zero_edges<SW_PTS>(pt2[0], t);
     fd128_zero_edges<SW_PTS>(pt2[1], t);
@@ -1046,10 +1067,10 @@
       {
         const int px = t >> 3, c = t & 7;
         uint16_t* d = ltu + px * 64 + ((c ^ (((px >> 1) & 1) << 2)) << 3);
-        *reinterpret_cast<sk_u32x4*>(d) = lcur.v0;
-        *reinterpret_cast<sk_u32x4*>(d + 32 * 64) = lcur.v1;
-        *reinterpret_cast<sk_u32x4*>(d + 64 * 64) = lcur.v2;
-        *reinterpret_cast<sk_u32x4*>(d + 96 * 64) = lcur.v3;
+        *reinterpret_cast<sk_u32x4*>(d) = bn8(lcur.v0);
+        *reinterpret_cast<sk_u32x4*>(d + 32 * 64) = bn8(lcur.v1);
+        *reinterpret_cast<sk_u32x4*>(d + 64 * 64) = bn8(lcur.v2);
+        *reinterpret_cast<sk_u32x4*>(d + 96 * 64) = bn8(lcur.v3);
       }
       __syncthreads();
       fd128_load(cur, x, min(u + 2, u1 - 1), wave, lane);
@@ -1328,12 +1349,20 @@
   return (size_t)nb * (O * SK_K + 64) * sizeof(float);
 }
 
+bool rg_skinny_wgrad_pre_ok(int N, int Ho, int Wo, int O, int dtype) {
+  return dtype == RG_H16 && O == 64 && N > 0 && Ho == R128_HO && Wo == R128_WO && sk_rows128(2 * Ho, 2 * Wo);
+}
+
 int rg_skinny_wgrad_slabs_impl(const void* low, const float* high_nchw, int N, int Ho, int Wo, int O, int I, int dtype,
                                void* slab, size_t slab_bytes, int* nslab_out, float* bias_slab, int* bias_done_out,
-                               hipStream_t st) {
+                               hipStream_t st, const float* pre_mean, const float* pre_invstd, const float* pre_gamma,
+                               const float* pre_beta, float pre_slope) {
   (void)I;
+  const LuPre pre{pre_mean, pre_invstd, pre_gamma, pre_beta, pre_slope};
   *nslab_out = 0;
   if (bias_done_out) *bias_done_out = 0;
+  RG_REQUIRE(!pre_mean || rg_skinny_wgrad_pre_ok(N, Ho, Wo, O, dtype), RG_EUNSUPPORTED,
+             "skinny_wgrad_slabs: fused BatchNorm input");
   const size_t elems = (size_t)O * SK_K;
   const long long npix = (long long)N * Ho * Wo;
   int chunk;
@@ -1343,8 +1372,12 @@
   if (sk_rows128(2 * Ho, 2 * Wo)) {
     if (nbm > 512) nbm = 512;
     RG_REQUIRE(slab && slab_bytes >= (size_t)nbm * elems * sizeof(float), RG_EWORKSPACE, "skinny_wgrad_slabs: buffer too small");
-    hipLaunchKernelGGL(skinny_wgrad_rows128_kernel, dim3(nbm), dim3(256), 0, st, (const uint16_t*)low, high_nchw, (float*)slab,
-                       nunits, bias_slab);
+    if (pre_mean)
+      hipLaunchKernelGGL(skinny_wgrad_rows128_kernel<true>, dim3(nbm), dim3(256), 0, st, (const uint16_t*)low, high_nchw,
+                         (float*)slab, nunits, bias_slab, pre);
+    else
+      hipLaunchKernelGGL(skinny_wgrad_rows128_kernel<false>, dim3(nbm), dim3(256), 0, st, (const uint16_t*)low, high_nchw,
+                         (float*)slab, nunits, bias_slab, pre);
     if (bias_done_out) *bias_done_out = bias_slab ? 1 : 0;
   } else {
     RG_REQUIRE(slab && slab_bytes >= (size_t)nbm * elems * sizeof(float), RG_EWORKSPACE, "skinny_wgrad_slabs: buffer too small");
@@ -1358,8 +1391,12 @@
 
 int rg_skinny_wgrad_impl(const void* low, const float* high_nchw, float* dw, int N, int Ho, int Wo, int O, int I,
                          int dtype, int accumulate, void* ws, size_t ws_bytes, hipStream_t st, float* dbias, int bias_accumulate,
-                         int* bias_done_out) {
+                         int* bias_done_out, const float* pre_mean, const float* pre_invstd, const float* pre_gamma,
+                         const float* pre_beta, float pre_slope) {
   (void)I;
+  const LuPre pre{pre_mean, pre_invstd, pre_gamma, pre_beta, pre_slope};
+  RG_REQUIRE(!pre_mean || rg_skinny_wgrad_pre_ok(N, Ho, Wo, O, dtype), RG_EUNSUPPORTED,
+             "skinny_wgrad: fused BatchNorm input");
   int bias_done_local = 0;
   if (!bias_done_out) bias_done_out = &bias_done_local;
   *bias_done_out = 0;
@@ -1375,8 +1412,12 @@
     if (sk_rows128(2 * Ho, 2 * Wo)) {
       if (nbm > 512) nbm = 512;
       float* bpart = (dbias && ws_bytes >= (size_t)nbm * (elems + 64) * sizeof(float)) ? (float*)ws + (size_t)nbm * elems : nullptr;
-      hipLaunchKernelGGL(skinny_wgrad_rows128_kernel, dim3(nbm), dim3(256), 0, st, (const uint16_t*)low, high_nchw, (float*)ws,
-                         nunits, bpart);
+      if (pre_mean)
+        hipLaunchKernelGGL(skinny_wgrad_rows128_kernel<true>, dim3(nbm), dim3(256), 0, st, (const uint16_t*)low, high_nchw,
+                           (float*)ws, nunits, bpart, pre);
+      else
+        hipLaunchKernelGGL(skinny_wgrad_rows128_kernel<false>, dim3(nbm), dim3(256), 0, st, (const uint16_t*)low, high_nchw,
+                           (float*)ws, nunits, bpart, pre);
       RG_LAUNCH_CHECK("skinny_wgrad(128)");
       int rc = rg_reduce_slabs((const float*)ws, dw, elems, nbm, accumulate, 0, 0, st);
       if (rc || !bpart) return rc;
diff --git a/rna_gan_amd/engine.py b/rna_gan_amd/engine.py
--- a/rna_gan_amd/engine.py
+++ b/rna_gan_amd/engine.py
@@ -478,6 +478,13 @@
             if img is not None:
                 ctx.img = img
                 return img, ctx
+        elif (l == len(G.blocks) - 1 and getattr(ops, "fuse_last_block", False) and
+              getattr(z, "_rg_slabs", None) is None):
+            r = ops.last_up_bn(z, st, bn, G.slope, G.last, G.last.bias, True, update_running, keep=True)
+            if r is not None:
+                ctx.img, mean, invstd = r
+                ctx.z.append(z); ctx.mean.append(mean); ctx.invstd.append(invstd); ctx.a.append(None)
+                return ctx.img, ctx
         a, mean, invstd = _bn_forward(ops, z, bn, G.slope, update_running, st)
         if keep:
             ctx.z.append(z); ctx.mean.append(mean); ctx.invstd.append(invstd); ctx.a.append(a)
@@ -564,7 +571,12 @@
     R = len(G.blocks)
     if gzl is None:
         gzl = ops.tanh_bwd(gimg, ctx.img)
-    ops.skinny_wgrad(ctx.a[R], gzl, G.last.dw, accumulate)
+    if ctx.a[R] is None:
+        bnR = G.blocks[R - 1][1]
+        ops.skinny_wgrad(ctx.z[R], gzl, G.last.dw, accumulate,
+                         pre=(ctx.mean[R], ctx.invstd[R], bnR.gamma, bnR.beta, G.slope))
+    else:
+        ops.skinny_wgrad(ctx.a[R], gzl, G.last.dw, accumulate)
     if gzl_parts is not None:
         ops.parts_chan_sum(gzl_parts, G.last.dbias, accumulate)
     else:
diff --git a/rna_gan_amd/graphed.py b/rna_gan_amd/graphed.py
--- a/rna_gan_amd/graphed.py
+++ b/rna_gan_amd/graphed.py
@@ -40,6 +40,7 @@
         self._out_spec = None
         self.wire_cell = None
         self._rebuilt = {}
+        self._packed = ()
 
     STABLE_NUMEL = 4096
 
@@ -89,6 +90,7 @@
                     self.static_out = self._stable(out, bufs) if len(bufs) == len(self._flat(out)) else out
                 self.graph = g
                 self._rebuilt = {mid: [cw for cw, pv in snap.items() if cw.packs_version != pv] for mid, snap in before.items()}
+                self._packed = tuple(cw for o in self.optimizers for cw in getattr(o, "packed_by_step", ()))
                 if os.environ.get("RNAGAN_GRAPH_DEBUG"):
                     print("rna_gan_amd: captured graph #%d for %s" % (len(_captured), getattr(self.fn, "__name__", "?")),
                           flush=True)
@@ -108,4 +110,7 @@
             m.mark_packs_fresh(only=self._rebuilt.get(id(m)))
         for m in self.stepped:
             m.weights_changed(by_optimizer=True)
+        if self._packed:
+            from .optim import mark_packed
+            mark_packed(self._packed)
         return self.static_out
diff --git a/rna_gan_amd/models.py b/rna_gan_amd/models.py
--- a/rna_gan_amd/models.py
+++ b/rna_gan_amd/models.py
@@ -150,6 +150,9 @@
                 continue
             if cw.packs_version != cw.version:
                 st = max(st, 2 if (cw.shadow is not None and cw.shadow_version != cw.version) else 1)
+        g0 = getattr(self._rt_net, "g0", None)
+        if st and g0 is not None and g0.packs is not None and g0.packs_version == g0.version:
+            st += 4
         return st
 
     def mark_packs_fresh(self, only=None):
diff --git a/rna_gan_amd/ops_hip.py b/rna_gan_amd/ops_hip.py
--- a/rna_gan_amd/ops_hip.py
+++ b/rna_gan_amd/ops_hip.py
@@ -126,6 +126,8 @@
         self._ws_retired = []
         self.fuse_input_post = os.environ.get("RNAGAN_INPUT_POST", "1") != "0"
         self.pack_from_shadow = os.environ.get("RNAGAN_PACK_FROM_SHADOW", "1") != "0"
+        self.fuse_g0_pack = True
+        self.fuse_last_block = True
         self.wgrad_in_step = os.environ.get("RNAGAN_WGRAD_ADAM", "1") != "0"
         self._skinny_defer = None
         self.skinny_bias = os.environ.get("RNAGAN_SKINNY_BIAS", "1") != "0"
@@ -750,10 +752,12 @@
         check(self.lib.rg_sign_pack(_ptr(a), _ptr(bits), a.numel() // 64, 64, self.dt, self.stream), "rg_sign_pack")
         return bits
 
-    def last_up_bn(self, z, partials, bn, slope: float, cw: ConvW, bias, tanh: bool, update_running=True):
+    def last_up_bn(self, z, partials, bn, slope: float, cw: ConvW, bias, tanh: bool, update_running=True, keep=False):
         N, Ho, Wo, O = z.shape
         I = cw.w.shape[1]
         if self.stat_reduce is not None or not self.lib.rg_last_up_pre_supported(Wo, O, I, self.dt):
+            return None
+        if keep and not (self.fuse_last_block and self.lib.rg_skinny_wgrad_pre_supported(N, Ho, Wo, O, I, self.dt)):
             return None
         M, C = self._mc(z)
         rm, rv, nbt = (bn.running_mean, bn.running_var, bn.nbt) if update_running else (None, None, None)
@@ -769,7 +773,7 @@
         check(self.lib.rg_last_up_pre(_ptr(z), _ptr(cw.w), _ptr(bias), _ptr(y), _ptr(mean), _ptr(invstd), _ptr(bn.gamma),
                                       _ptr(bn.beta), float(slope), N, Ho, Wo, O, I, int(tanh), self.dt, self.stream),
               "rg_last_up_pre")
-        return y
+        return (y, mean, invstd) if keep else y
 
     def last_up_bn2(self, z, partials, bn, slope: float, cw: ConvW, bias, tanh: bool, update_running=True):
         N2, Ho, Wo, O = z.shape
@@ -839,7 +843,7 @@
               "rg_gp_coef_parts_scaled")
         return loss, coef
 
-    def skinny_wgrad(self, low, high_nchw, dw, accumulate: bool, dbias=None, dbias_accumulate=False):
+    def skinny_wgrad(self, low, high_nchw, dw, accumulate: bool, dbias=None, dbias_accumulate=False, pre=None):
         N, Ho, Wo, O = low.shape
         I = high_nchw.shape[1]
         assert high_nchw.dtype == torch.float32 and high_nchw.is_contiguous() and low.is_contiguous()
@@ -868,10 +872,18 @@
             bhave = 0 if bprev is None else bprev[1]
             off = have * O * 48 * 4
             ns, bdone = ctypes.c_int(0), ctypes.c_int(0)
-            check(self.lib.rg_skinny_wgrad_slabs(_ptr(low), _ptr(high_nchw), N, Ho, Wo, O, I, self.dt, cw._slab_ws.data_ptr() + off,
-                                                 cw._slab_ws.numel() - off, ctypes.addressof(ns),
-                                                 cw._bias_ws.data_ptr() + bhave * O * 4 if want_bias else 0,
-                                                 ctypes.addressof(bdone), self.stream), "rg_skinny_wgrad_slabs")
+            if pre is not None:
+                check(self.lib.rg_skinny_wgrad_slabs_pre(_ptr(low), _ptr(high_nchw), _ptr(pre[0]), _ptr(pre[1]), _ptr(pre[2]),
+                                                         _ptr(pre[3]), float(pre[4]), N, Ho, Wo, O, I, self.dt,
+                                                         cw._slab_ws.data_ptr() + off, cw._slab_ws.numel() - off,
+                                                         ctypes.addressof(ns),
+                                                         cw._bias_ws.data_ptr() + bhave * O * 4 if want_bias else 0,
+                                                         ctypes.addressof(bdone), self.stream), "rg_skinny_wgrad_slabs_pre")
+            else:
+                check(self.lib.rg_skinny_wgrad_slabs(_ptr(low), _ptr(high_nchw), N, Ho, Wo, O, I, self.dt,
+                                                     cw._slab_ws.data_ptr() + off, cw._slab_ws.numel() - off, ctypes.addressof(ns),
+                                                     cw._bias_ws.data_ptr() + bhave * O * 4 if want_bias else 0,
+                                                     ctypes.addressof(bdone), self.stream), "rg_skinny_wgrad_slabs")
             if ns.value > 0:
                 cw.pending_slabs = (cw._slab_ws, have + int(ns.value), RG_F32)
                 if want_bias and bdone.value:
@@ -884,6 +896,12 @@
                 raise RuntimeError("rna_gan_amd: deferred image-side weight gradient: the second contribution has no slab form")
         ws = self._ws(nb)
         bdone = ctypes.c_int(0)
+        if pre is not None:
+            check(self.lib.rg_skinny_wgrad_bias_pre(_ptr(low), _ptr(high_nchw), _ptr(dw), _ptr(dbias), _ptr(pre[0]), _ptr(pre[1]),
+                                                    _ptr(pre[2]), _ptr(pre[3]), float(pre[4]), N, Ho, Wo, O, I, self.dt,
+                                                    int(accumulate), int(dbias_accumulate), _ptr(ws), ws.numel(),
+                                                    ctypes.addressof(bdone), self.stream), "rg_skinny_wgrad_bias_pre")
+            return bool(bdone.value)
         check(self.lib.rg_skinny_wgrad_bias(_ptr(low), _ptr(high_nchw), _ptr(dw), _ptr(dbias), N, Ho, Wo, O, I, self.dt,
                                             int(accumulate), int(dbias_accumulate), _ptr(ws), ws.numel(), ctypes.addressof(bdone),
                                             self.stream), "rg_skinny_wgrad_bias")
diff --git a/rna_gan_amd/optim.py b/rna_gan_amd/optim.py
--- a/rna_gan_amd/optim.py
+++ b/rna_gan_amd/optim.py
@@ -6,6 +6,11 @@
 
 from . import _abi
 from ._abi import check
+
+
+def mark_packed(cws):
+    for cw in cws:
+        cw.packs_version = cw.version
 
 
 class Adam(torch.optim.Adam):
@@ -24,6 +29,7 @@
         self.buf_gen = 0
         self.grad_wire = None
         self._ema = None
+        self.packed_by_step = ()
 
     def bind(self, module, fuse_linear_wgrad=False):
         mine = {id(p) for g in self.param_groups for p in g["params"]}
@@ -144,7 +150,7 @@
         ginv = 1.0 / float(getattr(mops, "loss_scale", 1.0)) if mops is not None else 1.0
         stream = torch.cuda.current_stream(flat.data.device).cuda_stream
         amp = getattr(mops, "amp", None) if mops is not None else None
-        launches, probes = [], []
+        launches, probes, packed = [], [], []
         if amp is None:
             check(lib.rg_adam_hyper_dev2(self._step_dev.data_ptr(), float(g["lr"]), float(g["betas"][0]),
                                          float(g["betas"][1]), float(g["eps"]), float(g.get("weight_decay", 0.0)), ginv,
@@ -169,10 +175,19 @@
                 raise RuntimeError("rna_gan_amd.optim.Adam: the deferred G.0 weight gradient expects that tensor at the head "
                                    "of the flat buffer")
             E, C = g0.w.shape[0], g0.w.shape[1]
-            launches.append(lambda z=z, gy=gy, E=E, C=C, dt=dt: check(lib.rg_g0_wgrad_adam(
-                z.data_ptr(), gy.data_ptr(), flat.data.data_ptr(), self._m.data_ptr(), self._v.data_ptr(),
-                self._hyper.data_ptr(), 0 if shadow is None else shadow.data_ptr(), z.shape[0], E, C, dt, stream),
-                "rg_g0_wgrad_adam"))
+            wp = g0.packs[0] if (g0.packs is not None and g0.shadow is not None and shadow is not None and
+                                 getattr(mops, "fuse_g0_pack", False) and mops.pack_from_shadow) else None
+            if wp is not None:
+                packed.append(g0)
+                launches.append(lambda z=z, gy=gy, E=E, C=C, dt=dt, wp=wp: check(lib.rg_g0_wgrad_adam_pack(
+                    z.data_ptr(), gy.data_ptr(), flat.data.data_ptr(), self._m.data_ptr(), self._v.data_ptr(),
+                    self._hyper.data_ptr(), shadow.data_ptr(), wp.data_ptr(), z.shape[0], E, C, dt, stream),
+                    "rg_g0_wgrad_adam_pack"))
+            else:
+                launches.append(lambda z=z, gy=gy, E=E, C=C, dt=dt: check(lib.rg_g0_wgrad_adam(
+                    z.data_ptr(), gy.data_ptr(), flat.data.data_ptr(), self._m.data_ptr(), self._v.data_ptr(),
+                    self._hyper.data_ptr(), 0 if shadow is None else shadow.data_ptr(), z.shape[0], E, C, dt, stream),
+                    "rg_g0_wgrad_adam"))
             probes += [seg(z), seg(gy)]
             lo = n0
         segs = []
@@ -287,4 +302,6 @@
         if not torch.cuda.is_current_stream_capturing():
             self._host_steps += 1
         self._module.weights_changed(by_optimizer=True)
+        self.packed_by_step = tuple(packed)
+        mark_packed(packed)
         return None
```

New measurement: 5995 imgs/sec. Within noise of the previous version (-0.4%).
